# vt-asaplab/vPIN

Hardware: AMD Instinct MI355X
Metric: R1CS constraints/sec, whole Spartan SNARK (sat proof + SPARK evaluation proof; vPIN point-mult + point-add instances) (higher is better)
Workload: dtype u256 (integers mod q and mod p = 2^255-19, 32-bit limbs); 1 GPU; vPIN LeNet trace (layers L1..L7): 12 SNARKs per step; inputs=resident in HBM, parallelism=one trace per rank x 1 rank(s), no collective; 4 stream(s) per rank, table_slot_bytes=128

## Files before the change

include/vpin_hip.h:

```cpp
#ifndef VPIN_HIP_H
#define VPIN_HIP_H
#include <stddef.h>
#include <stdint.h>

#ifdef __cplusplus
extern "C" {
#endif

#define VPIN_OK 0
#define VPIN_EINVAL (-1)
#define VPIN_ENODEV (-2)
#define VPIN_ENOMEM (-3)
#define VPIN_EHIP (-4)
#define VPIN_ESHAPE (-5)
#define VPIN_EVERIFY (-6)

typedef struct vpin_ctx vpin_ctx;
typedef struct vpin_table vpin_table;

const char* vpin_strerror(int code);
const char* vpin_last_error(void);
int vpin_crash_line_set(const char* line, size_t n);
int vpin_abi_version(void);

int vpin_ctx_create(int device, vpin_ctx** out);
int vpin_ctx_create_prio(int device, int priority, vpin_ctx** out);
int vpin_ctx_create_cumask(int device, const uint32_t* cu_mask, uint32_t n_words, vpin_ctx** out);
int vpin_ctx_set_cumask_after_phase1(vpin_ctx* ctx, const uint32_t* cu_mask, uint32_t n_words);
void vpin_ctx_destroy(vpin_ctx* ctx);
void* vpin_ctx_stream(vpin_ctx* ctx);
int vpin_ctx_set_progress_flag(vpin_ctx* ctx, int* flag);
int vpin_ctx_set_shared_device(vpin_ctx* ctx, int on);
unsigned long long vpin_ctx_strip_rows_taken(vpin_ctx* ctx);
unsigned long long vpin_ctx_pip_row_chunks(vpin_ctx* ctx);
int vpin_ctx_pool_stats(vpin_ctx* ctx, size_t out[3]);
int vpin_driver_alloc_stats(unsigned long long out[2]);
int vpin_ctx_pool_trim(vpin_ctx* ctx);
int vpin_ctx_set_low_memory(vpin_ctx* ctx, int on);
int vpin_ctx_set_expected_proofs(vpin_ctx* ctx, int n);
int vpin_ctx_device_props(vpin_ctx* ctx, int* num_cus, int* clock_khz);
int vpin_ctx_mem_info(vpin_ctx* ctx, size_t* free_bytes, size_t* total_bytes);
int vpin_ctx_sync(vpin_ctx* ctx);

int vpin_host_register(void* p, size_t bytes);
int vpin_host_unregister(void* p);

int vpin_table_upload(vpin_ctx* ctx, const uint8_t* mont32, size_t len, vpin_table** out);
int vpin_table_alloc(vpin_ctx* ctx, size_t len, vpin_table** out);
int vpin_table_wrap(vpin_ctx* ctx, void* device_ptr, size_t len, vpin_table** out);
int vpin_table_clone(vpin_ctx* ctx, const vpin_table* src, vpin_table** out);
void vpin_table_free(vpin_ctx* ctx, vpin_table* t);
size_t vpin_table_len(const vpin_table* t);
void* vpin_table_device_ptr(const vpin_table* t);
int vpin_table_read(vpin_ctx* ctx, const vpin_table* t, size_t off, size_t n, uint8_t* out);
int vpin_table_write(vpin_ctx* ctx, vpin_table* t, size_t off, size_t n, const uint8_t* src);

int vpin_sc_cubic_round(vpin_ctx* ctx, const vpin_table* tau, const vpin_table* Az,
                        const vpin_table* Bz, const vpin_table* Cz, uint8_t out_e0_e2_e3[96]);
int vpin_sc_quad_round(vpin_ctx* ctx, const vpin_table* A, const vpin_table* B,
                       uint8_t out_e0_e2[64]);
int vpin_sc_bind(vpin_ctx* ctx, vpin_table* const* tables, int k, const uint8_t r[32]);
int vpin_sc_cubic_bind_round(vpin_ctx* ctx, vpin_table* tau, vpin_table* Az, vpin_table* Bz,
                             vpin_table* Cz, const uint8_t r[32], uint8_t out_e0_e2_e3[96]);
int vpin_sc_quad_bind_round(vpin_ctx* ctx, vpin_table* A, vpin_table* B, const uint8_t r[32],
                            uint8_t out_e0_e2[64]);

int vpin_eq_table(vpin_ctx* ctx, const uint8_t* r, int ell, vpin_table** out);

int vpin_eq_suffix_tables(vpin_ctx* ctx, const uint8_t* tau, int ell, vpin_table** out);
int vpin_sc_cubic3_round(vpin_ctx* ctx, const vpin_table* pyramid, int ell, int level, vpin_table* Az,
                         vpin_table* Bz, vpin_table* Cz, uint8_t out_S0_S2_S3[96]);
int vpin_sc_cubic3_bind_round(vpin_ctx* ctx, const vpin_table* pyramid, int ell, int level, vpin_table* Az,
                              vpin_table* Bz, vpin_table* Cz, const uint8_t r[32], uint8_t out_S0_S2_S3[96]);
int vpin_sc_cubic3_lead_round(vpin_ctx* ctx, const vpin_table* pyramid, int ell, int level, vpin_table* Az,
                              vpin_table* Bz, vpin_table* Cz, const uint8_t* r, uint8_t out[96]);
int vpin_spark_batched_round(vpin_ctx* ctx, vpin_table* forest, size_t n, int ncirc, int level, size_t len,
                             const vpin_table* E, size_t e_off, const uint8_t* r, int lead, const vpin_table* derefs,
                             const vpin_table* vals, vpin_table* scratch, int first_fold, uint8_t* out);

typedef struct vpin_gens vpin_gens;
int vpin_gens_create(vpin_ctx* ctx, const uint8_t* gens_xyzt, size_t nb, vpin_gens** out);
int vpin_gens_map_stream(vpin_ctx* ctx, const uint8_t* stream64, size_t nb, uint8_t* out_xyzt);
int vpin_gens_shared(vpin_ctx* ctx, const char* label, const uint8_t* gens_xyzt, size_t nb, size_t budget_gb,
                     const vpin_gens** out);
void vpin_gens_shared_clear(void);
size_t vpin_gens_shared_bytes(int device);
void vpin_gens_free(vpin_ctx* ctx, vpin_gens* g);
size_t vpin_gens_count(const vpin_gens* g);
int vpin_gens_layout(const vpin_gens* g, size_t out[6]);
size_t vpin_gens_entry_bytes(void);
int vpin_hyrax_commit(vpin_ctx* ctx, const vpin_gens* g, const vpin_table* Z, const uint8_t* blinds,
                      size_t L, size_t blind_base, uint8_t* out_compressed );
int vpin_hyrax_commit_rows(vpin_ctx* ctx, const vpin_gens* g, const vpin_table* Z, size_t L, size_t row0, size_t nrows,
                           const uint8_t* blinds, size_t blind_base, uint8_t* out_compressed);
int vpin_hyrax_commit_pippenger(vpin_ctx* ctx, const vpin_gens* g, const vpin_table* Z, const uint8_t* blinds, size_t L,
                                size_t blind_base, int c_bits, uint8_t* out_compressed);
int vpin_hyrax_commit_pair(vpin_ctx* ctx, const vpin_gens* g, const vpin_table* Za, const vpin_table* Zb,
                           const uint8_t* blinds_a, const uint8_t* blinds_b, size_t L, size_t blind_base,
                           uint8_t* out_a, uint8_t* out_b, uint8_t* out_sum);
int vpin_gens_msm(vpin_ctx* ctx, const vpin_gens* g, const uint8_t* scalars_mont, size_t rows, size_t ncols,
                  uint8_t* out_compressed , uint8_t* out_xyzt );

int vpin_msm(vpin_ctx* ctx, const uint8_t* scalars_mont, const uint8_t* points_compressed, size_t n, uint8_t* out_compressed,
             uint8_t* out_xyzt);
int vpin_msm_bucket(vpin_ctx* ctx, const uint8_t* scalars_mont, const uint8_t* points_compressed, size_t n, uint8_t* out_compressed,
                    uint8_t* out_xyzt);
int vpin_points_add(vpin_ctx* ctx, const uint8_t* a_compressed, const uint8_t* b_compressed, size_t n, uint8_t* out_compressed);

size_t vpin_gens_msm_parts_count(size_t ncols);
int vpin_gens_msm_parts(vpin_ctx* ctx, const vpin_gens* g, const uint8_t* scalars_mont, size_t rows, size_t ncols,
                        uint8_t* parts_xyzt);

int vpin_poly_bound(vpin_ctx* ctx, const vpin_table* Z, const uint8_t* Lvec, size_t L_size, uint8_t* out_LZ);
int vpin_poly_slices_bound(vpin_ctx* ctx, const vpin_table* Z, int nbits, int used, const uint8_t* r, size_t r_len,
                           const uint8_t* ch, uint8_t* evals_out, uint8_t* LZ_out);
int vpin_poly_slices_bound_u32(vpin_ctx* ctx, const uint32_t* slices_u32, int n32, const vpin_table* Zfq, int nbits, int used,
                               const uint8_t* r, size_t r_len, const uint8_t* ch, uint8_t* evals_out, uint8_t* LZ_out);

typedef struct {
  size_t num_cons, num_vars, num_inputs;
  size_t nnz[3];
  const uint32_t* row[3];
  const uint32_t* col[3];
  const uint8_t* val[3];
} vpin_r1cs;
typedef struct vpin_r1cs_dev vpin_r1cs_dev;
int vpin_r1cs_upload(vpin_ctx* ctx, const vpin_r1cs* inst, vpin_r1cs_dev** out);
void vpin_r1cs_free(vpin_ctx* ctx, vpin_r1cs_dev* d);
void vpin_r1cs_dims(const vpin_r1cs_dev* d, size_t* num_cons, size_t* num_vars, size_t* num_inputs);
int vpin_r1cs_build_z(vpin_ctx* ctx, const vpin_r1cs_dev* d, const vpin_table* vars, const uint8_t* inputs,
                      vpin_table** out_z);
int vpin_r1cs_multiply_vec(vpin_ctx* ctx, const vpin_r1cs_dev* d, const vpin_table* z, vpin_table** Az,
                           vpin_table** Bz, vpin_table** Cz);
int vpin_r1cs_eval_table(vpin_ctx* ctx, const vpin_r1cs_dev* d, const vpin_table* evals_rx, const uint8_t r_abc[96],
                         vpin_table** out);
int vpin_r1cs_evaluate(vpin_ctx* ctx, const vpin_r1cs_dev* d, const vpin_table* evals_rx, const vpin_table* evals_ry,
                       uint8_t out[96]);

int vpin_sat_prove(vpin_ctx* ctx, const vpin_r1cs* inst, const uint8_t* vars_para, const uint8_t* vars_input,
                   const uint8_t* vars, const uint8_t* inputs, const uint8_t seed_commit64[64],
                   const uint8_t seed_proof64[64], uint8_t* proof_out, size_t proof_cap, size_t* proof_len,
                   uint8_t* comm_para_out, uint8_t* comm_input_out, uint8_t inst_evals_out[96],
                   uint8_t* rx_out, uint8_t* ry_out);
int vpin_sat_prove_resident(vpin_ctx* ctx, const vpin_r1cs_dev* inst, const vpin_table* vars_para,
                            const vpin_table* vars_input, const vpin_table* vars, const uint8_t* inputs,
                            const uint8_t seed_commit64[64], const uint8_t seed_proof64[64], uint8_t* proof_out,
                            size_t proof_cap, size_t* proof_len, uint8_t* comm_para_out, uint8_t* comm_input_out,
                            uint8_t inst_evals_out[96], uint8_t* rx_out, uint8_t* ry_out);
size_t vpin_sat_proof_max_bytes(size_t num_cons, size_t num_vars);
int vpin_dense_mlpoly_commit_sum(vpin_ctx* ctx, const vpin_table* vars, const uint8_t seed_commit64[64], uint8_t* out_compressed);
int vpin_sat_prepare(vpin_ctx* ctx, size_t num_vars);
int vpin_spark_prepare(vpin_ctx* ctx, size_t num_cons, size_t num_vars, size_t max_nnz);

void vpin_sat_last_timings(double out[8]);


typedef struct vpin_spark_decomm vpin_spark_decomm;

#define VPIN_ECOMM (-7)
typedef struct vpin_comm vpin_comm;
typedef int (*vpin_allgather_fn)(void* user, const void* send, void* recv, size_t bytes_per_rank);
int vpin_comm_create_shm(const char* name, int rank, int world, size_t slot_bytes, vpin_comm** out);
int vpin_comm_create_local(int world, size_t slot_bytes, vpin_comm** out_handles );
int vpin_comm_create_callbacks(int rank, int world, vpin_allgather_fn fn, void* user, vpin_comm** out);
void vpin_comm_destroy(vpin_comm* cm);
int vpin_comm_rank(const vpin_comm* cm);
int vpin_comm_world(const vpin_comm* cm);
int vpin_comm_allgather(vpin_comm* cm, const void* send, void* recv, size_t bytes);
int vpin_comm_enable_rccl(vpin_comm* cm, vpin_ctx* ctx);
int vpin_comm_allgather_dev(vpin_comm* cm, vpin_ctx* ctx, const void* d_send, void* d_recv, size_t bytes);
int vpin_comm_set_serialize(vpin_comm* cm, int on);
typedef struct {
// ... 234 lines not shown
```

vpin_amd/capi.py:

```python
import ctypes as C
import os
import re

import numpy as np

HERE = os.path.dirname(os.path.abspath(__file__))
ROOT = os.path.dirname(HERE)
HEADER = os.path.join(ROOT, "include", "vpin_hip.h")

KERNEL_CLASSES = {
    0: "sc_cubic", 1: "sc_quad", 2: "sc_bind", 3: "sc_cubic_fused", 4: "sc_quad_fused", 5: "eq", 6: "msm", 7: "sc_tail",
    8: "spark_round", 9: "spark_build", 10: "spark_round_big", 11: "msm_rows", 12: "spark_tail",
}
K_COUNT = 16


class VpinError(RuntimeError):
    def __init__(self, code, where):
        self.code = code
        L = lib()
        msg = L.vpin_strerror(code).decode()
        last = L.vpin_last_error().decode()
        super().__init__(f"{where}: {msg} ({code})" + (f" [{last}]" if last else ""))

# ... 586 lines not shown
            _chk(lib().vpin_ctx_create_cumask(device, words.ctypes.data_as(C.c_void_p), len(words), C.byref(self.h)), "vpin_ctx_create_cumask")
            return
        _chk(lib().vpin_ctx_create_prio(device, priority, C.byref(self.h)), "vpin_ctx_create_prio")

    @staticmethod
    def _mask_words(cu_mask):
        cus = sorted(set(int(x) for x in cu_mask))
        words = np.zeros((cus[-1] // 32) + 1, dtype=np.uint32)
        for x in cus:
            words[x // 32] |= np.uint32(1 << (x % 32))
        return words

    def set_cumask_after_phase1(self, cu_mask):
        if cu_mask is None:
            _chk(lib().vpin_ctx_set_cumask_after_phase1(self.h, None, 0), "vpin_ctx_set_cumask_after_phase1")
            return
        words = self._mask_words(cu_mask)
        _chk(lib().vpin_ctx_set_cumask_after_phase1(self.h, words.ctypes.data_as(C.c_void_p), len(words)), "vpin_ctx_set_cumask_after_phase1")

    def close(self):
        if self.h:
            lib().vpin_ctx_destroy(self.h)
            self.h = None

    def __enter__(self):
        return self

    def __exit__(self, *a):
        self.close()

    @property
    def stream(self):
        return lib().vpin_ctx_stream(self.h)

    def sync(self):
        _chk(lib().vpin_ctx_sync(self.h), "vpin_ctx_sync")

    def device_props(self):
        cus, khz = C.c_int(), C.c_int()
        L = lib()
        L.vpin_ctx_device_props.argtypes = [C.c_void_p, C.POINTER(C.c_int), C.POINTER(C.c_int)]
        _chk(L.vpin_ctx_device_props(self.h, C.byref(cus), C.byref(khz)), "vpin_ctx_device_props")
        return cus.value, khz.value * 1e3

    def device_total_bytes(self):
        f, t = C.c_size_t(), C.c_size_t()
        L = lib()
        L.vpin_ctx_mem_info.argtypes = [C.c_void_p, C.POINTER(C.c_size_t), C.POINTER(C.c_size_t)]
        _chk(L.vpin_ctx_mem_info(self.h, C.byref(f), C.byref(t)), "vpin_ctx_mem_info")
        return t.value

    def pool_stats(self):
        L = lib()
        L.vpin_ctx_pool_stats.argtypes = [C.c_void_p, C.POINTER(C.c_size_t * 3)]
        out = (C.c_size_t * 3)()
        _chk(L.vpin_ctx_pool_stats(self.h, C.byref(out)), "vpin_ctx_pool_stats")
        return int(out[0]), int(out[1]), int(out[2])

    @staticmethod
    def crash_line_set(line_bytes):
        L = lib()
        L.vpin_crash_line_set.argtypes = [C.c_char_p, C.c_size_t]
        _chk(L.vpin_crash_line_set(line_bytes if line_bytes else None, len(line_bytes)), "vpin_crash_line_set")

    @staticmethod
    def driver_alloc_stats():
        L = lib()
        L.vpin_driver_alloc_stats.argtypes = [C.POINTER(C.c_ulonglong * 2)]
        out = (C.c_ulonglong * 2)()
        _chk(L.vpin_driver_alloc_stats(C.byref(out)), "vpin_driver_alloc_stats")
        return int(out[0]), int(out[1])

    def pool_trim(self):
        L = lib()
        L.vpin_ctx_pool_trim.argtypes = [C.c_void_p]
        _chk(L.vpin_ctx_pool_trim(self.h), "vpin_ctx_pool_trim")

    def pip_row_chunks(self):
        L = lib()
        L.vpin_ctx_pip_row_chunks.argtypes = [C.c_void_p]
        L.vpin_ctx_pip_row_chunks.restype = C.c_ulonglong
        return int(L.vpin_ctx_pip_row_chunks(self.h))

    def strip_rows_taken(self):
        L = lib()
        L.vpin_ctx_strip_rows_taken.argtypes = [C.c_void_p]
        L.vpin_ctx_strip_rows_taken.restype = C.c_ulonglong
        return int(L.vpin_ctx_strip_rows_taken(self.h))

    def set_shared_device(self, on=True):
        _chk(lib().vpin_ctx_set_shared_device(self.h, 1 if on else 0), "vpin_ctx_set_shared_device")

    def set_low_memory(self, on=True):
        L = lib()
        L.vpin_ctx_set_low_memory.argtypes = [C.c_void_p, C.c_int]
        _chk(L.vpin_ctx_set_low_memory(self.h, 1 if on else 0), "vpin_ctx_set_low_memory")

    def set_expected_proofs(self, n):
        L = lib()
        L.vpin_ctx_set_expected_proofs.argtypes = [C.c_void_p, C.c_int]
        _chk(L.vpin_ctx_set_expected_proofs(self.h, int(n)), "vpin_ctx_set_expected_proofs")

    def gens_map_stream(self, stream):
        L = lib()
        L.vpin_gens_map_stream.argtypes = [C.c_void_p, C.c_void_p, C.c_size_t, C.c_void_p]
        buf = np.frombuffer(bytes(stream), dtype=np.uint8).copy()
        n = buf.size // 64
        out = np.zeros((n, 128), dtype=np.uint8)
        _chk(L.vpin_gens_map_stream(self.h, buf.ctypes.data_as(C.c_void_p), n, out.ctypes.data_as(C.c_void_p)), "vpin_gens_map_stream")
        return out

    def upload(self, arr):
        a = np.ascontiguousarray(arr)
        n = a.nbytes // 32
        h = C.c_void_p()
        _chk(lib().vpin_table_upload(self.h, a.ctypes.data_as(C.c_void_p), n, C.byref(h)), "vpin_table_upload")
        return Table(self, h)

    def alloc(self, n):
        h = C.c_void_p()
        _chk(lib().vpin_table_alloc(self.h, n, C.byref(h)), "vpin_table_alloc")
        return Table(self, h)

    def wrap(self, device_ptr, n):
        h = C.c_void_p()
        _chk(lib().vpin_table_wrap(self.h, C.c_void_p(device_ptr), n, C.byref(h)), "vpin_table_wrap")
        return Table(self, h)

    def eq_table(self, r):
        r = np.ascontiguousarray(r, dtype=np.uint64).reshape(-1, 4)
        h = C.c_void_p()
        _chk(lib().vpin_eq_table(self.h, r.ctypes.data_as(C.c_void_p), r.shape[0], C.byref(h)), "vpin_eq_table")
        return Table(self, h)

    def sc_cubic_round(self, tau, A, B, Cc):
        out = np.zeros((3, 4), dtype=np.uint64)
        _chk(lib().vpin_sc_cubic_round(self.h, tau.h, A.h, B.h, Cc.h, out.ctypes.data_as(C.c_void_p)),
             "vpin_sc_cubic_round")
        return out

    def sc_quad_round(self, A, B):
        out = np.zeros((2, 4), dtype=np.uint64)
        _chk(lib().vpin_sc_quad_round(self.h, A.h, B.h, out.ctypes.data_as(C.c_void_p)), "vpin_sc_quad_round")
        return out

    def sc_bind(self, tables, r):
        r = np.ascontiguousarray(r, dtype=np.uint64).reshape(4)
        arr = (C.c_void_p * len(tables))(*[t.h for t in tables])
        _chk(lib().vpin_sc_bind(self.h, arr, len(tables), r.ctypes.data_as(C.c_void_p)), "vpin_sc_bind")

    def sc_cubic_bind_round(self, tau, A, B, Cc, r):
        r = np.ascontiguousarray(r, dtype=np.uint64).reshape(4)
        out = np.zeros((3, 4), dtype=np.uint64)
        _chk(lib().vpin_sc_cubic_bind_round(self.h, tau.h, A.h, B.h, Cc.h, r.ctypes.data_as(C.c_void_p),
                                            out.ctypes.data_as(C.c_void_p)), "vpin_sc_cubic_bind_round")
        return out

    def sc_quad_bind_round(self, A, B, r):
        r = np.ascontiguousarray(r, dtype=np.uint64).reshape(4)
        out = np.zeros((2, 4), dtype=np.uint64)
        _chk(lib().vpin_sc_quad_bind_round(self.h, A.h, B.h, r.ctypes.data_as(C.c_void_p),
                                           out.ctypes.data_as(C.c_void_p)), "vpin_sc_quad_bind_round")
        return out

    def gens_create(self, xyzt):
        a = np.ascontiguousarray(xyzt, dtype=np.uint8).reshape(-1, 128)
        h = C.c_void_p()
        _chk(lib().vpin_gens_create(self.h, a.ctypes.data_as(C.c_void_p), a.shape[0], C.byref(h)), "vpin_gens_create")
        return Gens(self, h)

    def gens_shared(self, label, xyzt, budget_gb=0):
        a = np.ascontiguousarray(xyzt, dtype=np.uint8).reshape(-1, 128)
        h = C.c_void_p()
        _chk(lib().vpin_gens_shared(self.h, label.encode(), a.ctypes.data_as(C.c_void_p), a.shape[0], budget_gb, C.byref(h)),
             "vpin_gens_shared")
        g = Gens(self, h)
        g.free = lambda: None
        return g

    def gens_msm_parts(self, gens, scalars, rows, ncols):
        L = lib()
        L.vpin_gens_msm_parts_count.restype = C.c_size_t
        L.vpin_gens_msm_parts_count.argtypes = [C.c_size_t]
        s = np.ascontiguousarray(scalars, dtype=np.uint64).reshape(rows * ncols, 4)
        np_ = L.vpin_gens_msm_parts_count(ncols)
        out = np.zeros((rows, np_, 128), dtype=np.uint8)
        L.vpin_gens_msm_parts.argtypes = [C.c_void_p, C.c_void_p, C.c_void_p, C.c_size_t, C.c_size_t, C.c_void_p]
        _chk(L.vpin_gens_msm_parts(self.h, gens.h, s.ctypes.data_as(C.c_void_p), rows, ncols, out.ctypes.data_as(C.c_void_p)),
             "vpin_gens_msm_parts")
        return out

    def hyrax_commit(self, gens, Z, blinds, blind_base):
        b = np.ascontiguousarray(blinds, dtype=np.uint64).reshape(-1, 4)
        Ls = b.shape[0]
        out = np.zeros((Ls, 32), dtype=np.uint8)
        _chk(lib().vpin_hyrax_commit(self.h, gens.h, Z.h, b.ctypes.data_as(C.c_void_p), Ls, blind_base,
                                     out.ctypes.data_as(C.c_void_p)), "vpin_hyrax_commit")
        return out

    def hyrax_commit_pippenger(self, gens, Z, blinds, blind_base, Ls=None, c_bits=0):
        b = None if blinds is None else np.ascontiguousarray(blinds, dtype=np.uint64).reshape(-1, 4)
        Ls = b.shape[0] if b is not None else int(Ls)
        out = np.zeros((Ls, 32), dtype=np.uint8)
        _chk(lib().vpin_hyrax_commit_pippenger(self.h, gens.h, Z.h, b.ctypes.data_as(C.c_void_p) if b is not None else None, Ls,
                                               blind_base, c_bits, out.ctypes.data_as(C.c_void_p)), "vpin_hyrax_commit_pippenger")
        return out

    def hyrax_commit_pair(self, gens, Za, Zb, blinds_a, blinds_b, blind_base):
        ba = np.ascontiguousarray(blinds_a, dtype=np.uint64).reshape(-1, 4)
        bb = np.ascontiguousarray(blinds_b, dtype=np.uint64).reshape(-1, 4)
        Ls = ba.shape[0]
        outs = [np.zeros((Ls, 32), dtype=np.uint8) for _ in range(3)]
        _chk(lib().vpin_hyrax_commit_pair(self.h, gens.h, Za.h, Zb.h, ba.ctypes.data_as(C.c_void_p),
                                          bb.ctypes.data_as(C.c_void_p), Ls, blind_base,
                                          *[o.ctypes.data_as(C.c_void_p) for o in outs]), "vpin_hyrax_commit_pair")
        return outs

    def gens_msm(self, gens, scalars, rows, ncols, want_xyzt=False):
        s = np.ascontiguousarray(scalars, dtype=np.uint64).reshape(rows * ncols, 4)
        out = np.zeros((rows, 32), dtype=np.uint8)
        ox = np.zeros((rows, 128), dtype=np.uint8) if want_xyzt else None
        _chk(lib().vpin_gens_msm(self.h, gens.h, s.ctypes.data_as(C.c_void_p), rows, ncols,
                                 out.ctypes.data_as(C.c_void_p),
                                 ox.ctypes.data_as(C.c_void_p) if want_xyzt else None), "vpin_gens_msm")
        return (out, ox) if want_xyzt else out

    def msm(self, scalars, points_compressed, want_xyzt=False):
        s = np.ascontiguousarray(scalars, dtype=np.uint64).reshape(-1, 4)
        pts = np.ascontiguousarray(points_compressed, dtype=np.uint8).reshape(-1, 32)
        assert s.shape[0] == pts.shape[0]
        out, xyzt = np.zeros(32, np.uint8), np.zeros(128, np.uint8)
        L = lib()
        L.vpin_msm.argtypes = [C.c_void_p, C.c_void_p, C.c_void_p, C.c_size_t, C.c_void_p, C.c_void_p]
        p = lambda a: a.ctypes.data_as(C.c_void_p)
        _chk(L.vpin_msm(self.h, p(s), p(pts), s.shape[0], p(out), p(xyzt) if want_xyzt else None), "vpin_msm")
        return (out, xyzt) if want_xyzt else out

    def msm_bucket(self, scalars, points_compressed, want_xyzt=False):
        s = np.ascontiguousarray(scalars, dtype=np.uint64).reshape(-1, 4)
        pts = np.ascontiguousarray(points_compressed, dtype=np.uint8).reshape(-1, 32)
        assert s.shape[0] == pts.shape[0]
        out, xyzt = np.zeros(32, np.uint8), np.zeros(128, np.uint8)
        L = lib()
        L.vpin_msm_bucket.argtypes = [C.c_void_p, C.c_void_p, C.c_void_p, C.c_size_t, C.c_void_p, C.c_void_p]
        p = lambda a: a.ctypes.data_as(C.c_void_p)
        _chk(L.vpin_msm_bucket(self.h, p(s), p(pts), s.shape[0], p(out), p(xyzt) if want_xyzt else None), "vpin_msm_bucket")
        return (out, xyzt) if want_xyzt else out

    def dense_mlpoly_commit_sum(self, t_vars, seed_commit):
        L = lib()
        L.vpin_dense_mlpoly_commit_sum.argtypes = [C.c_void_p, C.c_void_p, C.c_void_p, C.c_void_p]
        nv = len(t_vars)
        Ls = 1 << ((nv.bit_length() - 1) // 2)
        out = np.zeros((Ls, 32), dtype=np.uint8)
        sc = np.frombuffer(bytes(seed_commit), dtype=np.uint8).copy()
        _chk(L.vpin_dense_mlpoly_commit_sum(self.h, t_vars.h, sc.ctypes.data_as(C.c_void_p), out.ctypes.data_as(C.c_void_p)),
             "vpin_dense_mlpoly_commit_sum")
        return out

    def points_add(self, a, b):
        a = np.ascontiguousarray(a, dtype=np.uint8).reshape(-1, 32)
        b = np.ascontiguousarray(b, dtype=np.uint8).reshape(-1, 32)
        out = np.zeros_like(a)
        L = lib()
        L.vpin_points_add.argtypes = [C.c_void_p, C.c_void_p, C.c_void_p, C.c_size_t, C.c_void_p]
        p = lambda x: x.ctypes.data_as(C.c_void_p)
        _chk(L.vpin_points_add(self.h, p(a), p(b), a.shape[0], p(out)), "vpin_points_add")
        return out

    def poly_bound(self, Z, Lvec):
        lv = np.ascontiguousarray(Lvec, dtype=np.uint64).reshape(-1, 4)
        out = np.zeros((len(Z) // lv.shape[0], 4), dtype=np.uint64)
        _chk(lib().vpin_poly_bound(self.h, Z.h, lv.ctypes.data_as(C.c_void_p), lv.shape[0],
                                   out.ctypes.data_as(C.c_void_p)), "vpin_poly_bound")
        return out

    def poly_slices_bound(self, Z, nbits, used, r, ch=None):
        rr = np.ascontiguousarray(r, dtype=np.uint64).reshape(-1, 4)
        ell = rr.shape[0] + nbits
        ev = np.zeros((used, 4), dtype=np.uint64)
# ... 442 lines not shown
```

vpin_amd/csrc/capi.hip:

```cpp
#include <chrono>
#include <csignal>
#include <execinfo.h>
#include <fcntl.h>
#include <unistd.h>
#include <cstdio>
#include <cstdlib>
#include <cstring>
#include <thread>

#include "ctx.h"

namespace vpin {

static thread_local std::string g_last_error;

void set_last_error(const char* what, hipError_t e) {
  g_last_error = std::string(what) + ": " + hipGetErrorString(e);
}

void set_last_error_text(const char* text) { g_last_error = text; }

static hipEvent_t get_event(vpin_ctx* c) {
  if (!c->free_events.empty()) {
    hipEvent_t e = c->free_events.back();
// ... 273 lines not shown
    c->cu_masked = true;
  } else {
    e = hipStreamCreateWithPriority(&c->stream, hipStreamNonBlocking, prio);
  }
  if (e != hipSuccess) { set_last_error("hipStreamCreate", e); delete c; return VPIN_EHIP; }
  c->stream_main = c->stream;
  c->cus_main = c->num_cus;
  c->partials_cap = (size_t)18 * 4096 * 3;
  if (hipMalloc(&c->d_partials, c->partials_cap * sizeof(fq)) != hipSuccess ||
      hipMalloc(&c->d_out, 8 * sizeof(fq)) != hipSuccess ||
      hipHostMalloc(&c->h_out, 8 * sizeof(fq), hipHostMallocDefault) != hipSuccess) {
    vpin_ctx_destroy(c);
    return VPIN_ENOMEM;
  }
  ctx_register(c);
  *out = c;
  return VPIN_OK;
}

void vpin_ctx_destroy(vpin_ctx* c) {
  if (!c) return;
  (void)hipSetDevice(c->device);
  if (c->stream) (void)hipStreamSynchronize(c->stream);
  ctx_leave_alt(c);
  if (c->prover_cache_free) c->prover_cache_free(c);
  if (c->spark_cache_free) c->spark_cache_free(c);
  if (c->verify_cache_free) c->verify_cache_free(c);
  if (c->h_spark) (void)hipHostFree(c->h_spark);
  if (c->d_spark_cnt) (void)hipFree(c->d_spark_cnt);
  if (c->d_add_count) (void)hipFree(c->d_add_count);
  ctx_unregister(c);
  ctx_wait_unpinned(c);
  dev_pool_release(c);
  if (!c->pool_sizes.empty()) {
    fprintf(stderr, "vpin_ctx_destroy: %zu device block(s) still referenced by live handles are released with the context; "
                    "free tables / instances / decommitments before the context\n", c->pool_sizes.size());
    for (auto& kv : c->pool_sizes) (void)hipFree(kv.first);
    c->pool_sizes.clear();
  }
  for (auto& r : c->recs) { (void)hipEventDestroy(r.start); (void)hipEventDestroy(r.stop); }
  for (auto e : c->free_events) (void)hipEventDestroy(e);
  if (c->d_partials) (void)hipFree(c->d_partials);
  if (c->d_out) (void)hipFree(c->d_out);
  if (c->h_out) (void)hipHostFree(c->h_out);
  if (c->h_bullet) (void)hipHostFree(c->h_bullet);
  if (c->stream_alt) { (void)hipStreamSynchronize(c->stream_alt); (void)hipStreamDestroy(c->stream_alt); }
  if (c->stream_switch_ev) (void)hipEventDestroy(c->stream_switch_ev);
  if (c->stream_main) (void)hipStreamDestroy(c->stream_main);
  delete c;
}

void* vpin_ctx_stream(vpin_ctx* c) { return c ? (void*)c->stream : nullptr; }

int vpin_ctx_set_cumask_after_phase1(vpin_ctx* c, const uint32_t* cu_mask, uint32_t n_words) {
  if (!c || c->cu_masked || c->stream != c->stream_main) return VPIN_EINVAL;
  (void)hipSetDevice(c->device);
  if (c->stream_alt) {
    VPIN_HIP_TRY(hipStreamSynchronize(c->stream_alt));
    (void)hipStreamDestroy(c->stream_alt);
    c->stream_alt = nullptr;
    c->cus_alt = 0;
  }
  if (!cu_mask || n_words == 0) return VPIN_OK;
  int enabled = 0;
  for (uint32_t w = 0; w < n_words; w++) {
    uint32_t bits = cu_mask[w];
    if ((w + 1) * 32 > (uint32_t)c->cus_main) bits &= (w * 32 >= (uint32_t)c->cus_main) ? 0u : ((1u << (c->cus_main - w * 32)) - 1u);
    enabled += __builtin_popcount(bits);
  }
  if (enabled == 0) return VPIN_EINVAL;
  if (!c->stream_switch_ev) VPIN_HIP_TRY(hipEventCreateWithFlags(&c->stream_switch_ev, hipEventDisableTiming));
  VPIN_HIP_TRY(hipExtStreamCreateWithCUMask(&c->stream_alt, n_words, cu_mask));
  c->cus_alt = enabled;
  return VPIN_OK;
}

int vpin_ctx_set_progress_flag(vpin_ctx* c, int* flag) {
  if (!c) return VPIN_EINVAL;
  c->progress_flag = flag;
  return VPIN_OK;
}

unsigned long long vpin_ctx_strip_rows_taken(vpin_ctx* c) { return c ? c->strip_rows_taken : 0ull; }
unsigned long long vpin_ctx_pip_row_chunks(vpin_ctx* c) { return c ? c->pip_row_chunks : 0ull; }

int vpin_host_register(void* p, size_t bytes) {
  if (!p || !bytes) return VPIN_EINVAL;
  VPIN_HIP_TRY(hipHostRegister(p, bytes, hipHostRegisterDefault));
  return VPIN_OK;
}
int vpin_host_unregister(void* p) {
  if (!p) return VPIN_EINVAL;
  VPIN_HIP_TRY(hipHostUnregister(p));
  return VPIN_OK;
}

int vpin_ctx_pool_trim(vpin_ctx* c) {
  if (!c) return VPIN_EINVAL;
  (void)hipSetDevice(c->device);
  dev_pool_release(c);
  return VPIN_OK;
}

int vpin_ctx_pool_stats(vpin_ctx* c, size_t out[3]) {
  if (!c || !out) return VPIN_EINVAL;
  std::lock_guard<std::mutex> g(c->pool_mu);
  size_t total = 0, cached = 0;
  for (auto& kv : c->pool_sizes) total += kv.second;
  for (auto& kv : c->pool_free_lists) cached += kv.first * kv.second.size();
  out[0] = total; out[1] = cached; out[2] = c->pool_sizes.size();
  return VPIN_OK;
}

namespace {
char g_crash_buf[8192];
volatile size_t g_crash_len = 0;
struct sigaction g_crash_old[5];
const int g_crash_sigs[5] = {SIGSEGV, SIGBUS, SIGABRT, SIGFPE, SIGTERM};
void crash_handler(int) {
  const size_t n = g_crash_len;
  size_t off = 0;
  while (off < n) {
    const ssize_t w = write(1, g_crash_buf + off, n - off);
    if (w <= 0) break;
    off += (size_t)w;
  }
  _exit(0);
}
}

namespace {
int g_segv_fd = 2;
void segv_trace_handler(int sig) {
  void* frames[64];
  const int n = backtrace(frames, 64);
  const char msg[] = "[vpin] fatal signal, call stack of the faulting thread:\n";
  (void)!write(g_segv_fd, msg, sizeof msg - 1);
  backtrace_symbols_fd(frames, n, g_segv_fd);
  signal(sig, SIG_DFL);
  raise(sig);
}
struct SegvTraceInit {
  SegvTraceInit() {
    const char* e = getenv("VPIN_SEGV_TRACE");
    if (!e) return;
    if (e[0] == '/' || e[0] == '.' || strchr(e, '/')) {
      const int fd = open(e, O_WRONLY | O_CREAT | O_APPEND, 0644);
      if (fd >= 0) g_segv_fd = fd;
    }
    struct sigaction sa;
    memset(&sa, 0, sizeof sa);
    sa.sa_handler = segv_trace_handler;
    sigemptyset(&sa.sa_mask);
    for (int sg : {SIGSEGV, SIGBUS, SIGABRT}) (void)sigaction(sg, &sa, nullptr);
  }
} g_segv_trace_init;
}

int vpin_crash_line_set(const char* line, size_t n) {
  if (n > sizeof g_crash_buf || (n && !line)) return VPIN_EINVAL;
  const bool was_armed = g_crash_len != 0;
  if (n == 0) {
    if (was_armed)
      for (int i = 0; i < 5; i++) (void)sigaction(g_crash_sigs[i], &g_crash_old[i], nullptr);
    g_crash_len = 0;
    return VPIN_OK;
// ... 232 lines not shown
```

vpin_amd/csrc/ctx.h:

```cpp
#pragma once
#include <hip/hip_runtime.h>

#include <atomic>
#include <chrono>
#include <cstdio>
#include <cstdlib>
#include <map>
#include <mutex>
#include <string>
#include <unordered_map>
#include <vector>

#include "../../include/vpin_hip.h"
#include "fq_dev.h"

namespace vpin {

void set_last_error(const char* what, hipError_t e);

#define VPIN_HIP_TRY(expr)                         \
  do {                                             \
    hipError_t e_ = (expr);                        \
    if (e_ != hipSuccess) {                        \
      ::vpin::set_last_error(#expr, e_);           \
      return VPIN_EHIP;                            \
    }                                              \
  } while (0)

struct ProfRec {
  int kclass;
  double bytes;
  hipEvent_t start, stop;
  int also = -1;
  double units = 0.0;
};

}

struct vpin_ctx;

struct vpin_table {
  vpin::fq* d = nullptr;
  size_t len = 0;
  size_t cap = 0;
  bool owned = true;
  vpin_ctx* owner = nullptr;
};

struct vpin_gens;

struct vpin_ctx {
  int device = 0;
  hipStream_t stream = nullptr;
  int num_cus = 256;
  bool cu_masked = false;
  hipStream_t stream_main = nullptr, stream_alt = nullptr;
  hipEvent_t stream_switch_ev = nullptr;
  int cus_main = 256, cus_alt = 0;
  vpin::fq* d_partials = nullptr;
  size_t partials_cap = 0;
  vpin::fq* d_out = nullptr;
  vpin::fq* h_out = nullptr;
  bool prof = false;
  bool prof_count_adds = false;
  unsigned long long* d_add_count = nullptr;
  std::vector<vpin::ProfRec> recs;
  std::vector<hipEvent_t> free_events;
  vpin_kstat stats[VPIN_K_COUNT] = {};
  std::mutex pool_mu;
  std::atomic<int> pins{0};
  std::map<size_t, std::vector<void*>> pool_free_lists;
  std::unordered_map<void*, size_t> pool_sizes;
  void* prover_cache = nullptr;
  void (*prover_cache_free)(vpin_ctx*) = nullptr;
  void* spark_cache = nullptr;
  void (*spark_cache_free)(vpin_ctx*) = nullptr;
  void* verify_cache = nullptr;
  void (*verify_cache_free)(vpin_ctx*) = nullptr;
  vpin::fq* h_spark = nullptr;
  uint32_t* d_spark_cnt = nullptr;
  uint32_t spark_seq = 0;
  int round_split = 0, round_split_grid = 0, round_split_ncirc = 0;
  int round_group_ndotp = 0;
  uint32_t tail_seq = 0;
  std::atomic<int> tail_rounds{0};
  vpin::fq tail_sums[3 * 18];
  vpin::fq tail_final[6 * 18];
  unsigned long long pip_row_chunks = 0;
  unsigned long long strip_rows_taken = 0;
  bool low_memory = false;
  bool shared_device = false;
  int expected_proofs = 0;
  double gens_scalars_per_proof = 0.0;
  void* h_bullet = nullptr;
  uint32_t bullet_seq = 0;
  std::atomic<vpin_comm*> comm_pub{nullptr};
  vpin_comm* comm = nullptr;
  volatile int* progress_flag = nullptr;
};

namespace vpin {

struct ProfScope {
  vpin_ctx* ctx;
  int rec = -1;
  ProfScope(vpin_ctx* c, int kclass, double bytes, int also = -1, double units = 0.0);
  ~ProfScope();
};

void ctx_enter_alt(vpin_ctx* c);
void ctx_leave_alt(vpin_ctx* c);
struct AltStreamGuard {
  vpin_ctx* c;
  explicit AltStreamGuard(vpin_ctx* ctx) : c(ctx) {}
  ~AltStreamGuard() { ctx_leave_alt(c); }
};

int dev_alloc(vpin_ctx* c, size_t bytes, void** out);
hipError_t driver_malloc(void** p, size_t bytes);
void note_driver_alloc(size_t bytes);
void dev_free(vpin_ctx* c, void* p);
int live_ctx_count();
double host_cpu_quota();
void dev_free_owned(vpin_ctx* owner, vpin_ctx* fallback, void* p);
void dev_pool_release(vpin_ctx* c);
void dev_release_block(vpin_ctx* c, void* p);

struct DevBuf {
  vpin_ctx* c;
  void* p = nullptr;
  explicit DevBuf(vpin_ctx* ctx) : c(ctx) {}
  ~DevBuf() { if (p) dev_free(c, p); }
  int alloc(size_t bytes) { return dev_alloc(c, bytes, &p); }
  void release() { if (p) { dev_free(c, p); p = nullptr; } }
};

int table_alloc_uninit(vpin_ctx* c, size_t len, vpin_table** out);

struct CommitPairState;
int commit_pair_begin(vpin_ctx* c, const vpin_gens* g, const vpin_table* Za, const vpin_table* Zb, size_t L,
                      CommitPairState** out, size_t row0 = 0, size_t nrows = (size_t)-1, size_t row_step = 1);
int commit_pair_finish(vpin_ctx* c, const vpin_gens* g, CommitPairState* st, const uint8_t* blinds_a, const uint8_t* blinds_b,
                       size_t blind_base, uint8_t* out_a, uint8_t* out_b, uint8_t* out_sum);

int sc_round_launch(vpin_ctx* c, int K, vpin_table* const* tabs, const uint8_t* r);
int sc_round_wait(vpin_ctx* c, int K, uint8_t* out);
int sc_final_claims(vpin_ctx* c, vpin_table* const* tables, int k, const uint8_t r[32], uint8_t* out);
int sc_cubic3_launch(vpin_ctx* c, vpin_table* const* t, const vpin_table* pyramid, int ell, int level, const uint8_t* r,
                     bool lead = false);

int r1cs_multiply_vec_strided(vpin_ctx* c, const vpin_r1cs_dev* d, const vpin_table* z, size_t r0, size_t step, vpin_table** Az,
                              vpin_table** Bz, vpin_table** Cz);
int table_take_strided(vpin_ctx* c, const vpin_table* src, size_t r0, size_t step, vpin_table** out);
int r1cs_eval_table_strided(vpin_ctx* c, const vpin_r1cs_dev* d, const vpin_table* evals_rx, const uint8_t r_abc[96], size_t r0,
                            size_t step, vpin_table** out);

int poly_bound_dist(vpin_ctx* c, const vpin_table* Z, const uint8_t* Lvec, size_t L_size, uint8_t* out_LZ, const fq* z_rows = nullptr);

int slices_bound(vpin_ctx* c, const uint32_t* Z32, int n32, const fq* Z, size_t N, int S, size_t Rs, const uint8_t* Ltop, size_t T,
                 const uint8_t* Rv, fq* d_LZs, uint8_t* ev_out);
int slices_combine(vpin_ctx* c, const fq* d_LZs, int S, size_t Rs, const uint8_t* coef, uint8_t* out_LZ);

inline bool is_pow2(size_t x) { return x && !(x & (x - 1)); }

int gens_msm_parts_dev(vpin_ctx* c, const vpin_gens* g, const fq* d_scalars, size_t rows, size_t ncols, uint8_t* parts_xyzt);
int hyrax_commit_derefs_hot(vpin_ctx* c, const vpin_gens* g, const vpin_table* Z, size_t L, size_t N, const uint32_t* const col_idx[3],
                            const uint32_t hot[3], const fq* e_ry, uint8_t* out_compressed, size_t row0 = 0, size_t nrows = (size_t)-1,
                            size_t row_step = 1, const fq* z_rows = nullptr);
int hyrax_commit_rows_strided(vpin_ctx* c, const vpin_gens* g, const vpin_table* Z, size_t L, size_t row0, size_t nrows, size_t row_step,
                              uint8_t* out_compressed, const fq* z_rows = nullptr);
size_t gens_msm_parts_scratch_bytes(size_t rows, size_t ncols);
int gens_msm_parts_launch(vpin_ctx* c, const vpin_gens* g, const fq* d_scalars, size_t rows, size_t ncols, void* scratch,
                          uint8_t* parts_xyzt, bool host_mapped = false);

struct ge_niels;
struct ge_ext;
int pip_rows(vpin_ctx* c, const ge_niels* d_gn, const fq* dZ, size_t rows, size_t stride, size_t ncols, const fq* d_extra, int n_extra,
             int cbits, ge_ext* d_points, unsigned long long* d_adds);
int pip_default_bits(size_t n);

struct BulletState;
int bullet_begin(vpin_ctx* c, const uint8_t* x_mont, const uint8_t* a_mont, size_t R, BulletState** out);
int bullet_round_begin(vpin_ctx* c, const vpin_gens* g, BulletState* st, size_t n, uint8_t* parts_xyzt, uint8_t cLR[64]);
int bullet_round_end(vpin_ctx* c);
uint8_t* bullet_pinned(vpin_ctx* c);
int bullet_fold(vpin_ctx* c, BulletState* st, size_t n, const uint8_t u[32], const uint8_t u_inv[32]);
int bullet_finish(vpin_ctx* c, const vpin_gens* g, BulletState* st, uint8_t xhat_ahat[64], uint8_t* parts_xyzt);
void bullet_free(vpin_ctx* c, BulletState* st);
bool bullet_fused(const BulletState* st);
int bullet_step(vpin_ctx* c, const vpin_gens* g, BulletState* st, size_t n, const uint8_t* u_prev, const uint8_t* u_inv_prev,
                uint8_t cLR[64]);
size_t bullet_part_ptrs(vpin_ctx* c, const BulletState* st, size_t n, int row, const uint8_t** out);
int bullet_finish_fused(vpin_ctx* c, const vpin_gens* g, BulletState* st, const uint8_t u[32], const uint8_t u_inv[32],
                        uint8_t xhat_ahat[64]);
int bullet_step_launch(vpin_ctx* c, const vpin_gens* g, const fq* a_prev, const fq* b_prev, fq* a_next, fq* b_next, fq* sj, size_t n,
                       size_t R, bool fold, bool finish, const uint8_t* u, const uint8_t* u_inv, uint8_t* parts_pinned,
                       uint32_t* up_pinned, uint32_t seq, void* dev_parts);

struct TraceLap {
  vpin_ctx* c;
  const char* who;
  bool on;
  std::chrono::steady_clock::time_point t;
  TraceLap(vpin_ctx* ctx, const char* w) : c(ctx), who(w), on(getenv("VPIN_CLI_TRACE") != nullptr), t(std::chrono::steady_clock::now()) {}
  void operator()(const char* what) {
    if (!on) return;
    if (c) (void)hipStreamSynchronize(c->stream);
    auto n = std::chrono::steady_clock::now();
    fprintf(stderr, "[%s] %-22s %9.1f ms\n", who, what, std::chrono::duration<double, std::milli>(n - t).count());
    t = n;
  }
};

}
```

vpin_amd/csrc/ge_tree_dev.h:

```cpp
#pragma once
#include "fp10_dev.h"

namespace vpin {

__device__ __forceinline__ ge_ext ge_load(const ge_ext* p) {
  ge_ext e;
  e.X = fp_load(&p->X); e.Y = fp_load(&p->Y); e.Z = fp_load(&p->Z); e.T = fp_load(&p->T);
  return e;
}
__device__ __forceinline__ void ge_store(ge_ext* o, const ge_ext& a) {
  fp_store(&o->X, a.X); fp_store(&o->Y, a.Y); fp_store(&o->Z, a.Z); fp_store(&o->T, a.T);
}
__device__ __forceinline__ void ge_store_identity(ge_ext* o) { ge_store(o, ge_identity()); }
__device__ __forceinline__ ge_niels ge_load(const ge_niels* p) {
  ge_niels e;
  e.ypx = fp_load(&p->ypx); e.ymx = fp_load(&p->ymx); e.xy2d = fp_load(&p->xy2d);
  return e;
}
__device__ __forceinline__ void ge_store(ge_niels* o, const ge_niels& a) {
  fp_store(&o->ypx, a.ypx); fp_store(&o->ymx, a.ymx); fp_store(&o->xy2d, a.xy2d);
}
__device__ __forceinline__ ge_cached ge_load(const ge_cached* p) {
  ge_cached e;
  e.YpX = fp_load(&p->YpX); e.YmX = fp_load(&p->YmX); e.Z = fp_load(&p->Z); e.T2d = fp_load(&p->T2d);
  return e;
}
__device__ __forceinline__ void ge_store(ge_cached* o, const ge_cached& a) {
  fp_store(&o->YpX, a.YpX); fp_store(&o->YmX, a.YmX); fp_store(&o->Z, a.Z); fp_store(&o->T2d, a.T2d);
}
__device__ __forceinline__ ge_ext ge_load(const fp* xyzt) { return ge_load(reinterpret_cast<const ge_ext*>(xyzt)); }
__device__ __forceinline__ void ge_store(fp* xyzt, const ge_ext& a) { ge_store(reinterpret_cast<ge_ext*>(xyzt), a); }
__device__ __forceinline__ void ge_store_frozen(fp* xyzt, const ge_ext& a) {
  fp_store(xyzt, fp_freeze(a.X)); fp_store(xyzt + 1, fp_freeze(a.Y)); fp_store(xyzt + 2, fp_freeze(a.Z)); fp_store(xyzt + 3, fp_freeze(a.T));
}
__device__ __forceinline__ void ge_store_result(fp* out32, fp* out_xyzt, const ge_ext& r) {
  fp_store(out32, ge_compress(r));
  ge_store_frozen(out_xyzt, r);
}

__device__ __forceinline__ void ge10_store_strided(uint32_t* __restrict__ p, size_t stride, const ge10& a) {
#pragma unroll
  for (int l = 0; l < 10; l++) {
    p[(size_t)l * stride] = a.X.v[l]; p[(size_t)(10 + l) * stride] = a.Y.v[l];
    p[(size_t)(20 + l) * stride] = a.Z.v[l]; p[(size_t)(30 + l) * stride] = a.T.v[l];
  }
}
__device__ __forceinline__ ge10 ge10_load_strided(const uint32_t* __restrict__ p, size_t stride) {
  ge10 a;
#pragma unroll
  for (int l = 0; l < 10; l++) {
    a.X.v[l] = p[(size_t)l * stride]; a.Y.v[l] = p[(size_t)(10 + l) * stride];
    a.Z.v[l] = p[(size_t)(20 + l) * stride]; a.T.v[l] = p[(size_t)(30 + l) * stride];
  }
  return a;
}

__device__ __forceinline__ uint16_t fq_signed_window(fq& s, uint32_t& carry, uint32_t cw, bool top) {
  const uint32_t mask = (1u << cw) - 1u, half = 1u << (cw - 1);
  uint32_t v = (s.v[0] & mask) + carry;
#pragma unroll
  for (int i = 0; i < 7; i++) s.v[i] = __builtin_amdgcn_alignbit(s.v[i + 1], s.v[i], cw);
  s.v[7] >>= cw;
  const bool neg = !top && v > half;
  if (neg) v = (mask + 1u) - v;
  carry = neg ? 1u : 0u;
  return (uint16_t)(v | (neg && v ? 0x8000u : 0u));
}
template <class Width>
__device__ __forceinline__ ge10 ge10_horner_windows(const ge_ext* wsum, int W, Width width) {
  ge10 acc = ge10_from_ext(ge_load(wsum + W - 1));
#pragma unroll 1
  for (int w = W - 2; w >= 0; w--) {
#pragma unroll 1
    for (int k = 0, cw = width(w); k < cw; k++) acc = ge10_double(acc);
    acc = ge10_add_ge10(acc, ge10_from_ext(ge_load(wsum + w)));
  }
  return acc;
}

__device__ __forceinline__ fp fp_shfl_from(const fp& a, int src) {
  fp r;
#pragma unroll
  for (int i = 0; i < 8; i++) r.v[i] = __shfl(a.v[i], src, 64);
  return r;
}
__device__ __forceinline__ fp fp_pick(bool c, const fp& a, const fp& b) {
  fp r;
#pragma unroll
  for (int i = 0; i < 8; i++) r.v[i] = c ? a.v[i] : b.v[i];
  return r;
}
__device__ __forceinline__ void ge_tree_quad(ge_ext* sh, int n, int split = 0) {
  const int role = threadIdx.x & 3, qbase = (threadIdx.x & 63) & ~3;
  const fp* shf = reinterpret_cast<const fp*>(sh);
  fp* shw = reinterpret_cast<fp*>(sh);
  for (int s = n / 2; s >= 1; s >>= 1) {
    if (s == split) continue;
    const int items = s < split ? 2 * s : s;
    for (int w = threadIdx.x >> 2; w < items; w += (int)(blockDim.x >> 2)) {
      const int i = w < s ? w : split + (w - s);
      const int f0 = role < 2 ? 1 : (role == 2 ? 3 : 2);
      const fp p0 = shf[4 * i + f0], q0 = shf[4 * (i + s) + f0];
      fp u = p0, v = q0;
      if (role < 2) {
        const fp p1 = shf[4 * i], q1 = shf[4 * (i + s)];
        u = fp_pick(role == 0, fp_sub(p0, p1), fp_add(p0, p1));
        v = fp_pick(role == 0, fp_sub(q0, q1), fp_add(q0, q1));
      }
      fp m = fp_mul(u, v);
      m = fp_mul(m, fp_pick(role == 2, FP_D2(), fp_one()));
      m = fp_pick(role == 3, fp_add(m, m), m);
      const fp a = fp_shfl_from(m, qbase), b = fp_shfl_from(m, qbase + 1), c = fp_shfl_from(m, qbase + 2),
               d = fp_shfl_from(m, qbase + 3);
      const fp E = fp_sub(b, a), H = fp_add(b, a), F = fp_sub(d, c), G = fp_add(d, c);
      u = fp_pick(role == 0 || role == 3, E, fp_pick(role == 1, G, F));
      v = fp_pick(role == 0, F, fp_pick(role == 2, G, H));
      shw[4 * i + role] = fp_mul(u, v);
    }
    __syncthreads();
  }
}

}
```

vpin_amd/csrc/msm.hip:

```cpp
#include <algorithm>
#include <atomic>
#include <cstdlib>
#include <condition_variable>
#include <cstring>
#include <memory>
#include <mutex>
#include <string>
#include <vector>

#include "ctx.h"
#include "fp_dev.h"
#include "fp10_dev.h"
#include "ge_tree_dev.h"
#include "mailbox_dev.h"

#ifndef VPIN_NIELS_SLOT
#define VPIN_NIELS_SLOT 96
#endif
static_assert(VPIN_NIELS_SLOT == 96 || VPIN_NIELS_SLOT == 128, "table entry size");

struct vpin_gens {
  vpin::fp* table = nullptr;
  vpin::fp* table_hi = nullptr;
  int s32 = VPIN_NIELS_SLOT / 32;
  size_t nb = 0;
  size_t nbt = 0;
  size_t split = 0;
  int c = 12, W = 22, E = 2048;
  int c_hi = 8, W_hi = 32, E_hi = 128;
};

namespace vpin {

struct TableView {
  const fp* t;
  const fp* t_hi;
  size_t split, nbt;
  int c, W, E, c_hi, W_hi, E_hi;
  size_t sum0;
  int s32;
};

struct TableSeg {
  const fp* t;
  size_t j, nb;
  int c, W, E, s32;
  __device__ __forceinline__ const ge_niels* entry(int w, uint32_t d) const {
    return reinterpret_cast<const ge_niels*>(t + (((size_t)w * nb + j) * (size_t)E + d) * (size_t)s32);
  }
};
__device__ __forceinline__ TableSeg table_seg(const TableView& tv, size_t j) {
  if (j < tv.split) return TableSeg{tv.t, j, tv.split, tv.c, tv.W, tv.E, tv.s32};
  return TableSeg{tv.t_hi, j - tv.split, tv.nbt - tv.split, tv.c_hi, tv.W_hi, tv.E_hi, tv.s32};
}


__global__ __launch_bounds__(256) void gens_sum_kernel(fp* __restrict__ xyzt, size_t nb) {
  const int k = blockIdx.x;
  const size_t lo = k ? ((size_t)1 << (k - 1)) : 0, hi = (size_t)1 << k;
  ge_ext acc = ge_identity();
  for (size_t j = lo + threadIdx.x; j < hi && j < nb; j += 256) {
    acc = ge_add(acc, ge_load(xyzt + 4 * j));
  }
  __shared__ ge_ext sh[256];
  sh[threadIdx.x] = acc;
  __syncthreads();
  for (int st = 128; st >= 1; st >>= 1) {
    if ((int)threadIdx.x < st) {
      acc = ge_add(acc, sh[threadIdx.x + st]);
      sh[threadIdx.x] = acc;
    }
    __syncthreads();
  }
  if (threadIdx.x == 0) ge_store(xyzt + 4 * (nb + k), acc);
}
__global__ void gens_sum_scan_kernel(fp* __restrict__ xyzt, size_t nb, int nsum) {
  if (threadIdx.x || blockIdx.x) return;
  ge_ext acc = ge_load(xyzt + 4 * nb);
  for (int k = 1; k < nsum; k++) {
    fp* q = xyzt + 4 * (nb + k);
    acc = ge_add(acc, ge_load(q));
    ge_store(q, acc);
  }
}

__global__ __launch_bounds__(64) void gens_shift_kernel(const fp* __restrict__ xyzt, size_t nb, int W, int c,
                                                        ge_ext* __restrict__ shifts) {
  size_t j = (size_t)blockIdx.x * blockDim.x + threadIdx.x;
  if (j >= nb) return;
  ge_ext p = ge_load(xyzt + 4 * j);
  for (int w = 0; w < W; w++) {
    ge_store(shifts + j * W + w, p);
    for (int k = 0; k < c; k++) p = ge_double(p);
  }
}

__global__ __launch_bounds__(64) void gens_table_kernel(const ge_ext* __restrict__ shifts, size_t nb, int W, int E,
                                                        fp* __restrict__ table, int s32, fp* __restrict__ prefix) {
  size_t idx = (size_t)blockIdx.x * blockDim.x + threadIdx.x;
  if (idx >= nb * (size_t)W) return;
  size_t j = idx / W;
  int w = (int)(idx % W);
  const ge_ext p = ge_load(shifts + j * W + w);
  ge_cached pc = ge_to_cached(p);
  fp* out = table + (((size_t)w * nb + j) * E) * (size_t)s32;
  fp* pre = prefix + ((size_t)w * nb + j) * E;
  ge_ext q = p;
  fp run = fp_one();
  for (int k = 0; k < E; k++) {
    fp_store(out + (size_t)k * s32, q.X); fp_store(out + (size_t)k * s32 + 1, q.Y); fp_store(out + (size_t)k * s32 + 2, q.Z);
    run = fp_mul(run, q.Z);
    fp_store(pre + k, run);
    if (k + 1 < E) q = ge_add_cached(q, pc);
  }
  fp acc = fp_invert(run);
  const fp d2 = FP_D2();
  for (int k = E - 1; k >= 0; k--) {
    fp X = fp_load(out + (size_t)k * s32), Y = fp_load(out + (size_t)k * s32 + 1), Z = fp_load(out + (size_t)k * s32 + 2);
    fp zinv = (k > 0) ? fp_mul(acc, fp_load(pre + k - 1)) : acc;
    acc = fp_mul(acc, Z);
    fp x = fp_mul(X, zinv), y = fp_mul(Y, zinv);
    fp_store(out + (size_t)k * s32, fp_add(y, x));
    fp_store(out + (size_t)k * s32 + 1, fp_sub(y, x));
    fp_store(out + (size_t)k * s32 + 2, fp_mul(fp_mul(x, y), d2));
  }
}


__device__ __forceinline__ bool fq_fold_sign(fq& s) {
  if (s.v[7] < 0x08000000u) return false;
  fq d;
  unsigned bw = 0;
#pragma unroll
  for (int i = 0; i < 8; i++) d.v[i] = __builtin_subc(fq_modulus_limb(i), s.v[i], bw, &bw);
  s = d;
  return true;
}
// ... 290 lines not shown
  for (size_t r = r0; r < r1; r++) n += flag[r] ? 1u : 0u;
  base[threadIdx.x] = n;
  __syncthreads();
  if (threadIdx.x == 0) {
    uint32_t run = 0;
    for (int t = 0; t < 1024; t++) { const uint32_t v = base[t]; base[t] = run; run += v; }
    *count = run;
  }
  __syncthreads();
  uint32_t o = base[threadIdx.x];
  for (size_t r = r0; r < r1; r++)
    if (flag[r]) list[o++] = (uint32_t)r;
}

__global__ __launch_bounds__(256) void strip_trim_kernel(const uint32_t* __restrict__ list, uint32_t* __restrict__ count, uint32_t n_use,
                                                          uint32_t n_all, uint8_t* __restrict__ flag) {
  const uint32_t li = n_use + blockIdx.x * 256 + threadIdx.x;
  if (li < n_all) flag[list[li]] = 0;
  if (blockIdx.x == 0 && threadIdx.x == 0) *count = n_use;
}

__global__ __launch_bounds__(kMsmBlock, 3) void msm_strip_kernel(const fq* __restrict__ Z, size_t stride, size_t ncols, TableView tv, HotRows hr,
                                                                  const uint32_t* __restrict__ list, const uint32_t* __restrict__ list_count,
                                                                  int S, size_t row_base, size_t row_step, int z_compact,
                                                                  ge_ext* __restrict__ parts, uint32_t* __restrict__ sync, int lag) {
  const uint32_t n = *list_count;
  const uint32_t s = blockIdx.x % (uint32_t)S, grp = blockIdx.x / (uint32_t)S;
  if (grp * kMsmBlock >= n) return;
  const uint32_t li = grp * kMsmBlock + threadIdx.x;
  const bool live = li < n;
  const uint32_t i = list[live ? li : n - 1];
  const size_t row = row_base + (size_t)i * row_step;
  const fq* zr = Z + (z_compact ? (size_t)i : row) * stride;
  const uint32_t* idx = nullptr;
  uint32_t hot = 0xffffffffu;
  if (hr.rows_per_vec && row >= hr.row0 && row < hr.row0 + 3 * hr.rows_per_vec) {
    const size_t m = (row - hr.row0) / hr.rows_per_vec;
    if (hr.hot[m] != 0xffffffffu) { hot = hr.hot[m]; idx = hr.idx[m] + (row - hr.row0 - m * hr.rows_per_vec) * ncols; }
  }
  const size_t per = (ncols + (size_t)S - 1) / (size_t)S, j0 = (size_t)s * per, j1 = j0 + per < ncols ? j0 + per : ncols;
  ge10 acc = ge10_identity();
  const uint32_t groups = (n + kMsmBlock - 1) / kMsmBlock;
  uint32_t* my_sync = sync ? sync + (size_t)s * (per + 1) : nullptr;
  __shared__ int sh_nosync;
  if (threadIdx.x == 0) sh_nosync = 0;
  __syncthreads();
  for (size_t j = j0; j < j1; j++) {
    if (my_sync && j - j0 >= (size_t)lag) {
      if (threadIdx.x == 0 && !sh_nosync) {
        long spin = 0;
        while (__hip_atomic_load(my_sync + (j - j0 - (size_t)lag), __ATOMIC_RELAXED, __HIP_MEMORY_SCOPE_AGENT) < groups)
          if (++spin > (1L << 16)) { sh_nosync = 1; break; }
      }
      __syncthreads();
    }
    fq v = fq_load(zr + j);
    const bool act = live && !fq_is_zero(v) && !(idx && idx[j] == hot);
    if (__builtin_amdgcn_ballot_w64(act) != 0) {
      fq sc = fq_from_mont(v);
      if (!act) sc = fq_zero();
      table_mul_acc10(acc, sc, tv, j);
    }
    if (my_sync) {
      __syncthreads();
      if (threadIdx.x == 0) __hip_atomic_fetch_add(my_sync + (j - j0), 1u, __ATOMIC_RELAXED, __HIP_MEMORY_SCOPE_AGENT);
    }
  }
  if (live) {
    const ge_ext av = ge10_to_ext(acc);
    ge_store(parts + (size_t)li * (size_t)S + s, av);
  }
}

__global__ __launch_bounds__(64) void strip_combine_kernel(const ge_ext* __restrict__ parts, const uint32_t* __restrict__ list,
                                                            const uint32_t* __restrict__ list_count, int S, ge_ext* __restrict__ out) {
  const uint32_t li = blockIdx.x * 64 + threadIdx.x;
  if (li >= *list_count) return;
  ge_ext* o = out + list[li];
  ge_ext a = ge_load(o);
  for (int s = 0; s < S; s++) a = ge_add(a, ge_load(parts + (size_t)li * (size_t)S + s));
  ge_store(o, a);
}

__device__ __forceinline__ uint32_t count_digits(fq s, const TableView& tv, size_t j) {
  (void)fq_fold_sign(s);
  const TableSeg sg = table_seg(tv, j);
  uint32_t carry = 0, n = 0;
  const uint32_t full = 1u << sg.c, half = 1u << (sg.c - 1);
  for (int w = 0; w < sg.W; w++) {
    uint32_t v = scalar_digit(s, w, sg.c) + carry;
    const bool neg = v > half;
    const uint32_t mag = neg ? full - v : v;
    carry = neg ? 1u : 0u;
    n += mag != 0;
  }
  return n;
}
__global__ __launch_bounds__(kMsmBlock) void msm_count_adds_kernel(const fq* __restrict__ Z, size_t stride, size_t ncols,
                                                                   const fq* __restrict__ extra, int n_extra, size_t extra_base0,
                                                                   TableView tv, unsigned long long* __restrict__ count,
                                                                   HotRows hr = HotRows{}, size_t row_base = 0, size_t row_step = 1,
                                                                   int z_compact = 0) {
  const size_t row = row_base + (size_t)blockIdx.x * row_step;
  const fq* zr = Z + (z_compact ? (size_t)blockIdx.x : row) * stride;
  const uint32_t* hidx = nullptr;
  uint32_t hot = 0xffffffffu;
  if (hr.rows_per_vec && row >= hr.row0 && row < hr.row0 + 3 * hr.rows_per_vec) {
    const size_t m = (row - hr.row0) / hr.rows_per_vec;
    if (hr.hot[m] != 0xffffffffu) { hot = hr.hot[m]; hidx = hr.idx[m] + (row - hr.row0 - m * hr.rows_per_vec) * ncols; }
  }
  uint32_t n = 0;
  bool constant = false;
  if (ncols >= 256 && (ncols & (ncols - 1)) == 0 && ((size_t)1 << (tv.nbt - tv.sum0 - 1)) >= ncols) {
    const fq first = fq_load(zr);
    int same = 1;
    for (size_t j = threadIdx.x; j < ncols; j += kMsmBlock) same &= fq_eq(first, fq_load(zr + j)) ? 1 : 0;
    constant = __syncthreads_and(same) != 0;
    if (constant && threadIdx.x == 0 && !fq_is_zero(first))
      n += count_digits(fq_from_mont(first), tv, tv.sum0 + (size_t)(63 - __builtin_clzll((unsigned long long)ncols)));
  }
  if (!constant)
    for (size_t j = threadIdx.x; j < ncols; j += kMsmBlock) {
      const fq s = fq_load(zr + j);
      if (!fq_is_zero(s) && !(hidx && hidx[j] == hot)) n += count_digits(fq_from_mont(s), tv, j);
    }
  for (int e = threadIdx.x; e < n_extra; e += kMsmBlock) {
    const fq x = fq_load(extra + row * (size_t)n_extra + e);
    if (!fq_is_zero(x)) n += count_digits(fq_from_mont(x), tv, extra_base0 + e);
  }
  __shared__ uint32_t sh[kMsmBlock];
  sh[threadIdx.x] = n;
  __syncthreads();
  for (int st = kMsmBlock / 2; st >= 1; st >>= 1) {
    if ((int)threadIdx.x < st) sh[threadIdx.x] += sh[threadIdx.x + st];
    __syncthreads();
  }
  if (threadIdx.x == 0 && sh[0]) atomicAdd(count, (unsigned long long)sh[0]);
}

constexpr int kWideScalars = 32;
template <int Q>
__global__ __launch_bounds__(kMsmBlock) void msm_wide_kernel(const fq* __restrict__ S, size_t ncols, TableView tv,
                                                             fp* __restrict__ parts_xyzt) {
  const size_t row = blockIdx.y;
  const int grp = threadIdx.x & 7;
  ge_ext acc = ge_identity();
#pragma unroll 1
  for (int q = 0; q < Q; q++) {
    const size_t j = ((size_t)blockIdx.x * Q + q) * kWideScalars + (threadIdx.x >> 3);
    if (j < ncols) {
      fq s = fq_load(S + row * ncols + j);
      if (!fq_is_zero(s)) {
        const TableSeg sg = table_seg(tv, j);
        const int wpg = (sg.W + 7) / 8;
        int w0 = grp * wpg, w1 = (w0 + wpg < sg.W) ? w0 + wpg : sg.W;
        if (w0 < w1) table_mul_acc_range(acc, fq_from_mont(s), sg, w0, w1);
      }
    }
  }
  __shared__ ge_ext sh[kMsmBlock];
  sh[threadIdx.x] = acc;
  __syncthreads();
  ge_tree_quad(sh, kMsmBlock);
  if (threadIdx.x == 0) {
    acc = sh[0];
    ge_store_frozen(parts_xyzt + 4 * (row * gridDim.x + blockIdx.x), acc);
  }
}


struct BulletStep {
  const fq* a_prev; const fq* b_prev;
  fq* a_next; fq* b_next;
  fq* sj;
  size_t n, R;
  int fold, finish, nmsm;
  fq u, u_inv;
  fp* parts;
  uint32_t* up;
  uint32_t seq;
};

__global__ __launch_bounds__(kMsmBlock) void bullet_step_kernel(BulletStep a, TableView tv) {
  const size_t n = a.n;
  const int nip = (int)gridDim.x - a.nmsm;
  if ((int)blockIdx.x < nip) {
    const int ib = (int)blockIdx.x;
    const size_t i = (size_t)ib * kMsmBlock + threadIdx.x;
    fq pl = fq_zero(), pr = fq_zero();
    if (a.finish) {
      if (ib == 0 && threadIdx.x == 0) {
        pl = fq_add(fq_mul(fq_load(a.a_prev), a.u), fq_mul(a.u_inv, fq_load(a.a_prev + 1)));
        pr = fq_add(fq_mul(fq_load(a.b_prev), a.u_inv), fq_mul(a.u, fq_load(a.b_prev + 1)));
      }
    } else if (i < n) {
      fq a0, a1, b0, b1;
      if (a.fold) {
        a0 = fq_add(fq_mul(fq_load(a.a_prev + i), a.u), fq_mul(a.u_inv, fq_load(a.a_prev + 2 * n + i)));
        a1 = fq_add(fq_mul(fq_load(a.a_prev + n + i), a.u), fq_mul(a.u_inv, fq_load(a.a_prev + 3 * n + i)));
        b0 = fq_add(fq_mul(fq_load(a.b_prev + i), a.u_inv), fq_mul(a.u, fq_load(a.b_prev + 2 * n + i)));
        b1 = fq_add(fq_mul(fq_load(a.b_prev + n + i), a.u_inv), fq_mul(a.u, fq_load(a.b_prev + 3 * n + i)));
      } else {
        a0 = fq_load(a.a_prev + i); a1 = fq_load(a.a_prev + n + i);
        b0 = fq_load(a.b_prev + i); b1 = fq_load(a.b_prev + n + i);
      }
      fq_store(a.a_next + i, a0); fq_store(a.a_next + n + i, a1);
      fq_store(a.b_next + i, b0); fq_store(a.b_next + n + i, b1);
      pl = fq_mul(a0, b1);
      pr = fq_mul(a1, b0);
    }
    __shared__ fq shp[kMsmBlock / 64][2];
// ... 113 lines not shown
  ge_ext acc = ge_load(p);
  for (int k = 1; k < chunks; k++) acc = ge_add(acc, ge_load(p + k));
  ge_store(out + i, acc);
}

__global__ __launch_bounds__(64) void ge_add_rows_kernel(const ge_ext* __restrict__ a, const ge_ext* __restrict__ b, size_t n,
                                                         ge_ext* __restrict__ out) {
  size_t i = (size_t)blockIdx.x * blockDim.x + threadIdx.x;
  if (i >= n) return;
  ge_store(out + i, ge_add(ge_load(a + i), ge_load(b + i)));
}

__global__ __launch_bounds__(256) void pip_gens_kernel(TableView tv, size_t n, size_t blind_base, int n_extra, ge_niels* __restrict__ out) {
  const size_t i = (size_t)blockIdx.x * 256 + threadIdx.x;
  if (i >= n + (size_t)n_extra) return;
  const TableSeg sg = table_seg(tv, i < n ? i : blind_base);
  ge_store(out + i, ge_load(sg.entry(0, 0)));
}

__global__ __launch_bounds__(64) void ge_compress_kernel(const ge_ext* __restrict__ pts, size_t n, fp* __restrict__ out32,
                                                         fp* __restrict__ out_xyzt) {
  size_t i = (size_t)blockIdx.x * blockDim.x + threadIdx.x;
  if (i >= n) return;
  const ge_ext p = ge_load(pts + i);
  if (out32) fp_store(out32 + i, ge_compress(p));
  if (out_xyzt) ge_store_frozen(out_xyzt + 4 * i, p);
}

}

namespace vpin {

__device__ __forceinline__ fp FP_ONE_MINUS_D_SQ() { return fp_const(0x945fc176u, 0xe27c09c1u, 0xcd5e350fu, 0x2c81a138u, 0xbe70dfe4u, 0x9994abddu, 0xb2b3e0d7u, 0x029072a8u); }
__device__ __forceinline__ fp FP_D_MINUS_ONE_SQ() { return fp_const(0x44ed4d20u, 0x31ad5aaau, 0xb01e1999u, 0xd29e4a2cu, 0x529b4eebu, 0x4cdcd32fu, 0xf66c2241u, 0x5968b37au); }
__device__ __forceinline__ fp FP_SQRT_AD_MINUS_ONE() { return fp_const(0x497b2e1bu, 0x7e97f6a0u, 0x1b7854bdu, 0xaf9d8e0cu, 0x31f5d1fdu, 0x0f3cfcc9u, 0x2b8348acu, 0x376931bfu); }

__device__ __forceinline__ fp fp_sqrt_ratio_m1(const fp& u, const fp& v, bool* was_square) {
  const fp v3 = fp_mul(fp_sqr(v), v), v7 = fp_mul(fp_sqr(v3), v);
  fp r = fp_mul(fp_mul(u, v3), fp_pow_p58(fp_mul(u, v7)));
  const fp check = fp_mul(v, fp_sqr(r));
  const fp nu = fp_neg(u), nu_i = fp_mul(nu, FP_SQRT_M1());
  const bool correct = fp_eq(check, u), flipped = fp_eq(check, nu), flipped_i = fp_eq(check, nu_i);
  r = fp_select(flipped || flipped_i, fp_mul(r, FP_SQRT_M1()), r);
  *was_square = correct || flipped;
  return fp_abs(r);
}

__device__ __noinline__ ge_ext ge_elligator(const fp& t) {
  const fp one = fp_one(), m1 = fp_neg(one), d = FP_D();
  const fp r = fp_mul(FP_SQRT_M1(), fp_sqr(t));
  const fp u = fp_mul(fp_add(r, one), FP_ONE_MINUS_D_SQ());
  const fp v = fp_mul(fp_sub(m1, fp_mul(r, d)), fp_add(r, d));
  bool sq;
  fp s = fp_sqrt_ratio_m1(u, v, &sq);
  const fp sp = fp_neg(fp_abs(fp_mul(s, t)));
  s = fp_select(sq, s, sp);
  const fp c = fp_select(sq, m1, r);
  const fp N = fp_sub(fp_mul(fp_mul(c, fp_sub(r, one)), FP_D_MINUS_ONE_SQ()), v);
  const fp ss = fp_sqr(s);
  const fp w0 = fp_mul(fp_add(s, s), v), w1 = fp_mul(N, FP_SQRT_AD_MINUS_ONE()), w2 = fp_sub(one, ss), w3 = fp_add(one, ss);
  ge_ext p;
  p.X = fp_mul(w0, w3); p.Y = fp_mul(w2, w1); p.Z = fp_mul(w1, w3); p.T = fp_mul(w0, w2);
  return p;
}

__global__ __launch_bounds__(64) void gens_derive_kernel(const uint32_t* __restrict__ stream, size_t nb, fp* __restrict__ xyzt) {
  const size_t i = (size_t)blockIdx.x * 64 + threadIdx.x;
  if (i >= nb) return;
  fp t0, t1;
#pragma unroll
  for (int k = 0; k < 8; k++) { t0.v[k] = stream[16 * i + k]; t1.v[k] = stream[16 * i + 8 + k]; }
  t0.v[7] &= 0x7fffffffu;
  t1.v[7] &= 0x7fffffffu;
  const ge_ext p = ge_add(ge_elligator(t0), ge_elligator(t1));
  ge_store_frozen(xyzt + 4 * i, p);
}

}

using namespace vpin;

extern "C" {

static int gens_build_once(vpin_ctx* c, const uint8_t* gens_xyzt, size_t nb, size_t budget, int cmax, vpin_gens** out);

static int gens_build(vpin_ctx* c, const uint8_t* gens_xyzt, size_t nb, size_t budget, vpin_gens** out) {
  (void)hipSetDevice(c->device);
  size_t free_b = 0, total_b = 0;
  const hipError_t e_info = c->expected_proofs > 0 ? hipErrorUnknown : hipMemGetInfo(&free_b, &total_b);
  if (e_info == hipSuccess && free_b) {
    static const double frac = [] { const char* e = getenv("VPIN_GENS_FREE_FRACTION"); double v = e ? atof(e) : 0.0; return v > 0.0 && v < 1.0 ? v : 1.0 / 3.0; }();
    const size_t cap = (size_t)((double)free_b * frac);
    if (budget > cap) budget = cap;
  }
  const size_t floor_b = (size_t)1 << 28;
  if (budget < floor_b) budget = floor_b;
  static const int env_cmax = [] { const char* e = getenv("VPIN_GENS_CMAX"); int v = e ? atoi(e) : 12; return v < 8 ? 8 : v > 14 ? 14 : v; }();
  int cmax = env_cmax;
  if (c->expected_proofs > 0 && c->gens_scalars_per_proof > 0.0) {
    const double S = c->gens_scalars_per_proof * (double)c->expected_proofs, n_lo = (double)std::min<size_t>(nb, 16386);
    double best = 0.0;
    for (int cc = 8; cc <= 12; cc++) {
      const double W = (double)((254 + cc - 1) / cc), cost = n_lo * W * (double)(1u << (cc - 1)) * 4.0 + S * W;
      if (cc == 8 || cost < best) { best = cost; cmax = cc; }
    }
  }
  for (;;) {
    int rc = gens_build_once(c, gens_xyzt, nb, budget, cmax, out);
    if (rc != VPIN_ENOMEM || budget <= floor_b) return rc;
    (void)hipGetLastError();
    budget /= 2;
    if (budget < floor_b) budget = floor_b;
  }
}

static size_t table_slot_bytes() {
  const char* e = getenv("VPIN_TABLE_SLOT");
  const int v = e ? atoi(e) : VPIN_NIELS_SLOT;
  return v == 128 ? 128 : v == 96 ? 96 : (size_t)VPIN_NIELS_SLOT;
}

static int gens_build_once(vpin_ctx* c, const uint8_t* gens_xyzt, size_t nb, size_t budget, int cmax, vpin_gens** out) {
  if (!c || !gens_xyzt || !out || nb == 0) return VPIN_EINVAL;
  const size_t slot = table_slot_bytes();
  (void)hipSetDevice(c->device);
  vpin_gens* g = new (std::nothrow) vpin_gens();
  if (!g) return VPIN_ENOMEM;
  g->nb = nb;
  g->s32 = (int)(slot / 32);
  int nsum = 1;
  while (((size_t)2 << (nsum - 1)) <= nb) nsum++;
  const size_t nbt = nb + (size_t)nsum;
  g->nbt = nbt;
  constexpr size_t kSplitBases = 16386;
  auto fit = [&](size_t n, size_t bud, int cmax, int* c_, int* W_, int* E_) {
    int cc = cmax;
    for (; cc > 6; cc--)
      if (n * (size_t)((254 + cc - 1) / cc) * ((size_t)1 << (cc - 1)) * slot <= bud) break;
    *c_ = cc;
    *W_ = (254 + cc - 1) / cc;
    *E_ = 1 << (cc - 1);
  };
  g->split = nbt;
  fit(nb, budget, cmax, &g->c, &g->W, &g->E);
  if (nb > kSplitBases) {
    int c2, W2, E2;
    fit(kSplitBases, budget, cmax, &c2, &W2, &E2);
    const size_t lo_bytes = kSplitBases * (size_t)W2 * E2 * slot;
    if (c2 > g->c && lo_bytes < budget) {
      g->split = kSplitBases;
      g->c = c2; g->W = W2; g->E = E2;
      fit(nbt - kSplitBases, budget - lo_bytes, g->c, &g->c_hi, &g->W_hi, &g->E_hi);
    }
  }
  const size_t n_hi = nbt - g->split;
  const size_t entries = g->split * (size_t)g->W * g->E, entries_hi = n_hi * (size_t)g->W_hi * g->E_hi;
  const size_t max_entries = entries > entries_hi ? entries : entries_hi;
  const size_t max_shifts = std::max(g->split * (size_t)g->W, n_hi * (size_t)g->W_hi);
  TraceLap lap(c, "gens_build");
  DevBuf raw(c), b_shifts(c), b_prefix(c);
  if (raw.alloc(nbt * 128) != VPIN_OK || b_shifts.alloc(max_shifts * sizeof(ge_ext)) != VPIN_OK ||
      b_prefix.alloc(max_entries * sizeof(fp)) != VPIN_OK || driver_malloc((void**)&g->table, entries * slot) != hipSuccess ||
      (n_hi && driver_malloc((void**)&g->table_hi, entries_hi * slot) != hipSuccess)) {
    if (g->table) (void)hipFree(g->table);
    if (g->table_hi) (void)hipFree(g->table_hi);
    delete g;
    return VPIN_ENOMEM;
  }
  ge_ext* shifts = (ge_ext*)b_shifts.p;
  fp* prefix = (fp*)b_prefix.p;
  lap("hipMalloc");
  hipError_t e = hipMemcpyAsync(raw.p, gens_xyzt, nb * 128, hipMemcpyHostToDevice, c->stream);
  if (e == hipSuccess) {
    hipLaunchKernelGGL(gens_sum_kernel, dim3((unsigned)nsum), dim3(256), 0, c->stream, (fp*)raw.p, nb);
    hipLaunchKernelGGL(gens_sum_scan_kernel, dim3(1), dim3(64), 0, c->stream, (fp*)raw.p, nb, nsum);
    hipLaunchKernelGGL(gens_shift_kernel, dim3((unsigned)((g->split + 63) / 64)), dim3(64), 0, c->stream, (const fp*)raw.p, g->split,
                       g->W, g->c, shifts);
    hipLaunchKernelGGL(gens_table_kernel, dim3((unsigned)((g->split * g->W + 63) / 64)), dim3(64), 0, c->stream, shifts, g->split, g->W,
                       g->E, g->table, g->s32, prefix);
    if (n_hi) {
      hipLaunchKernelGGL(gens_shift_kernel, dim3((unsigned)((n_hi + 63) / 64)), dim3(64), 0, c->stream,
                         (const fp*)raw.p + 4 * g->split, n_hi, g->W_hi, g->c_hi, shifts);
      hipLaunchKernelGGL(gens_table_kernel, dim3((unsigned)((n_hi * g->W_hi + 63) / 64)), dim3(64), 0, c->stream, shifts, n_hi,
                         g->W_hi, g->E_hi, g->table_hi, g->s32, prefix);
    }
    e = hipGetLastError();
  }
  if (e == hipSuccess) e = hipStreamSynchronize(c->stream);
  lap("table kernels");
  if (e == hipSuccess && c->expected_proofs == 0 && !getenv("VPIN_GENS_TMP_KEEP") && b_prefix.p) {
    void* pp = b_prefix.p;
    b_prefix.p = nullptr;
    dev_release_block(c, pp);
  }
  if (e != hipSuccess) {
    set_last_error("vpin_gens_create", e);
    (void)hipFree(g->table);
    if (g->table_hi) (void)hipFree(g->table_hi);
    delete g;
    return VPIN_EHIP;
  }
  *out = g;
  return VPIN_OK;
}

static size_t default_budget() {
  static const size_t budget = [] {
    const char* e = getenv("VPIN_GENS_BUDGET_GB");
    size_t gb = e ? (size_t)atoi(e) : 24;
    return (gb ? gb : 24) << 30;
  }();
  return budget;
}

int vpin_gens_create(vpin_ctx* c, const uint8_t* gens_xyzt, size_t nb, vpin_gens** out) {
  return gens_build(c, gens_xyzt, nb, default_budget(), out);
}

int vpin_gens_map_stream(vpin_ctx* c, const uint8_t* stream64, size_t nb, uint8_t* out_xyzt) {
  if (!c || !stream64 || !out_xyzt || nb == 0) return VPIN_EINVAL;
  (void)hipSetDevice(c->device);
  DevBuf bs(c), bo(c);
  if (bs.alloc(nb * 64) || bo.alloc(nb * 128)) return VPIN_ENOMEM;
  VPIN_HIP_TRY(hipMemcpyAsync(bs.p, stream64, nb * 64, hipMemcpyHostToDevice, c->stream));
  hipLaunchKernelGGL(gens_derive_kernel, dim3((unsigned)((nb + 63) / 64)), dim3(64), 0, c->stream, (const uint32_t*)bs.p, nb, (fp*)bo.p);
  VPIN_HIP_TRY(hipGetLastError());
  VPIN_HIP_TRY(hipMemcpyAsync(out_xyzt, bo.p, nb * 128, hipMemcpyDeviceToHost, c->stream));
  VPIN_HIP_TRY(hipStreamSynchronize(c->stream));
  return VPIN_OK;
}

namespace {
struct RegEntry { int device; std::string label; vpin_gens* g; };
struct Building { int device; std::string label; size_t nb; };
std::mutex g_reg_mu;
std::condition_variable g_reg_cv;
std::vector<RegEntry> g_reg;
std::vector<Building> g_building;
}

int vpin_gens_shared(vpin_ctx* c, const char* label, const uint8_t* gens_xyzt, size_t nb, size_t budget_gb,
                     const vpin_gens** out) {
  if (!c || !label || !out || nb == 0) return VPIN_EINVAL;
  auto lookup = [&]() -> const vpin_gens* {
    const vpin_gens* best = nullptr;
    for (auto& e : g_reg)
      if (e.device == c->device && e.label == label && e.g->nb >= nb && (!best || e.g->nb < best->nb)) best = e.g;
    return best;
  };
  {
    std::unique_lock<std::mutex> lock(g_reg_mu);
    for (;;) {
      if (const vpin_gens* best = lookup()) { *out = best; return VPIN_OK; }
      bool covered = false;
      for (auto& b : g_building) covered = covered || (b.device == c->device && b.label == label && b.nb >= nb);
      if (!covered) break;
      g_reg_cv.wait(lock);
    }
    if (!gens_xyzt) return VPIN_EINVAL;
    static std::atomic<bool> said{false};
    for (auto& e : g_reg)
      if (e.device == c->device && e.label == label && !said.exchange(true))
        fprintf(stderr, "vpin_gens_shared: a table of \"%s\" for %zu generators is built beside the one for %zu (both stay allocated): "
                        "call vpin_spark_prepare / vpin_sat_prepare with the largest shape first\n", label, nb, e.g->nb);
    g_building.push_back(Building{c->device, label, nb});
  }
  vpin_gens* g = nullptr;
  const int rc = gens_build(c, gens_xyzt, nb, budget_gb ? (budget_gb << 30) : default_budget(), &g);
  std::lock_guard<std::mutex> lock(g_reg_mu);
  for (size_t i = 0; i < g_building.size(); i++)
    if (g_building[i].device == c->device && g_building[i].label == label && g_building[i].nb == nb) { g_building.erase(g_building.begin() + (long)i); break; }
  if (!rc) {
    g_reg.push_back(RegEntry{c->device, label, g});
    *out = g;
  }
  g_reg_cv.notify_all();
  return rc;
}

size_t vpin_gens_shared_bytes(int device) {
  std::lock_guard<std::mutex> lock(g_reg_mu);
  size_t total = 0;
  for (auto& e : g_reg)
    if (e.device == device)
      total += (size_t)32 * (size_t)e.g->s32 * ((size_t)e.g->W * e.g->split * (size_t)e.g->E +
                                     (e.g->split < e.g->nbt ? (size_t)e.g->W_hi * (e.g->nbt - e.g->split) * (size_t)e.g->E_hi : 0));
  return total;
}

void vpin_gens_shared_clear(void) {
  std::lock_guard<std::mutex> lock(g_reg_mu);
  for (auto& e : g_reg) {
    (void)hipSetDevice(e.device);
    (void)hipDeviceSynchronize();
    if (e.g->table) (void)hipFree(e.g->table);
    if (e.g->table_hi) (void)hipFree(e.g->table_hi);
    delete e.g;
  }
  g_reg.clear();
}

void vpin_gens_free(vpin_ctx* c, vpin_gens* g) {
  if (!g) return;
  if (c) { (void)hipSetDevice(c->device); (void)hipStreamSynchronize(c->stream); }
  if (g->table) (void)hipFree(g->table);
  if (g->table_hi) (void)hipFree(g->table_hi);
  delete g;
}

size_t vpin_gens_count(const vpin_gens* g) { return g ? g->nb : 0; }
int vpin_gens_layout(const vpin_gens* g, size_t out[6]) {
  if (!g || !out) return VPIN_EINVAL;
  out[0] = (size_t)g->c; out[1] = (size_t)g->W; out[2] = g->split;
  out[3] = g->split < g->nbt ? (size_t)g->c_hi : 0; out[4] = g->split < g->nbt ? (size_t)g->W_hi : 0; out[5] = g->nbt;
  return VPIN_OK;
}
size_t vpin_gens_entry_bytes(void) { return table_slot_bytes(); }

static inline TableView view(const vpin_gens* g) {
  return TableView{g->table, g->table_hi, g->split, g->nbt, g->c, g->W, g->E, g->c_hi, g->W_hi, g->E_hi, g->nb, g->s32};
}

static int pip_mode() {
  const char* e = getenv("VPIN_MSM_PIPPENGER");
  const int v = e ? atoi(e) : 0;
  return v <= 0 ? 0 : (v >= 9 && v <= 12 ? v : -1);
}

static int msm_rows_pip(vpin_ctx* c, const vpin_gens* g, const fq* dZ, size_t rows, size_t stride, size_t ncols, const fq* d_extra,
                        int n_extra, size_t extra_base0, int cbits, ge_ext* d_points) {
  DevBuf dgn(c);
  if (dgn.alloc((ncols + 1) * sizeof(ge_niels))) return VPIN_ENOMEM;
  hipLaunchKernelGGL(pip_gens_kernel, dim3((unsigned)((ncols + 1 + 255) / 256)), dim3(256), 0, c->stream, view(g), ncols, extra_base0,
                     n_extra, (ge_niels*)dgn.p);
  return pip_rows(c, (const ge_niels*)dgn.p, dZ, rows, stride, ncols, d_extra, n_extra, cbits, d_points,
                  c->prof_count_adds ? c->d_add_count : nullptr);
}

static unsigned msm_lds_pad(const vpin_ctx* c) {
  static const int env_pad = [] { const char* e = getenv("VPIN_MSM_LDS_PAD"); return e ? atoi(e) : -1; }();
  return env_pad >= 0 ? (unsigned)env_pad : (c->shared_device ? kSharedPad : 0u);
}

static int msm_rows(vpin_ctx* c, const vpin_gens* g, const fq* dZ, size_t rows, size_t stride, size_t ncols,
                    const fq* d_extra, int n_extra, size_t extra_base0, ge_ext* d_points) {
  if (const int pm = pip_mode())
    if (n_extra <= 1 && ncols + (size_t)n_extra <= 32768)
      return msm_rows_pip(c, g, dZ, rows, stride, ncols, d_extra, n_extra, extra_base0, pm < 0 ? 0 : pm, d_points);
  double nz_est = (double)rows * ((double)ncols + n_extra);
  size_t total = ncols + (size_t)n_extra;
  int chunks = 1;
  if (rows < 128) {
    size_t want = (total + kMsmBlock - 1) / kMsmBlock * 4;
    chunks = (int)(want < 1 ? 1 : want > 64 ? 64 : want);
  } else if (rows >= 768 && total > (size_t)kSeg) {
    static const int env_chunks = [] { const char* e = getenv("VPIN_MSM_ROW_CHUNKS"); return e ? atoi(e) : 0; }();
    chunks = env_chunks > 0 ? env_chunks : (int)std::min<size_t>(8, (total + kSeg - 1) / kSeg);
  } else if (rows < 768 && total >= 2 * (size_t)kMsmBlock) {
    size_t want = (768 + rows - 1) / rows, most = total / kMsmBlock;
    chunks = (int)(want < most ? want : most);
    if (chunks < 1) chunks = 1;
  }
  DevBuf parts(c);
  ge_ext* dst = d_points;
  if (chunks > 1) {
    if (parts.alloc(rows * (size_t)chunks * sizeof(ge_ext))) return VPIN_ENOMEM;
    dst = (ge_ext*)parts.p;
  }
  if (c->prof_count_adds && c->d_add_count && rows >= 128)
    hipLaunchKernelGGL(msm_count_adds_kernel, dim3((unsigned)rows), dim3(kMsmBlock), 0, c->stream, dZ, stride, ncols, d_extra,
                       n_extra, extra_base0, view(g), c->d_add_count);
  {
    ProfScope ps(c, VPIN_K_MSM, 32.0 * nz_est, rows >= 128 ? VPIN_K_MSM_ROWS : -1);
    hipLaunchKernelGGL(msm_rows_kernel, dim3((unsigned)rows, (unsigned)chunks), dim3(kMsmBlock), msm_lds_pad(c), c->stream, dZ, stride, ncols,
                       d_extra, n_extra, extra_base0, view(g), dst);
  }
  if (chunks > 1)
    hipLaunchKernelGGL(ge_sum_chunks_kernel, dim3((unsigned)((rows + 63) / 64)), dim3(64), 0, c->stream, (const ge_ext*)dst,
                       rows, chunks, d_points);
  VPIN_HIP_TRY(hipGetLastError());
  return VPIN_OK;
}

static int compress_to_host(vpin_ctx* c, const ge_ext* d_pts, size_t n, uint8_t* out0, uint8_t* out1 = nullptr, uint8_t* out2 = nullptr) {
  uint8_t* const outs[3] = {out0, out1, out2};
  const size_t k = out2 ? 3 : out1 ? 2 : 1, per = n / k * 32;
  DevBuf dout(c);
  if (dout.alloc(n * 32)) return VPIN_ENOMEM;
  hipLaunchKernelGGL(ge_compress_kernel, dim3((unsigned)((n + 63) / 64)), dim3(64), 0, c->stream, d_pts, n, (fp*)dout.p, (fp*)nullptr);
  VPIN_HIP_TRY(hipGetLastError());
  for (size_t i = 0; i < k; i++) VPIN_HIP_TRY(hipMemcpyAsync(outs[i], (uint8_t*)dout.p + i * per, per, hipMemcpyDeviceToHost, c->stream));
  VPIN_HIP_TRY(hipStreamSynchronize(c->stream));
  return VPIN_OK;
}

static int commit_rows(vpin_ctx* c, const vpin_gens* g, const fq* z, size_t rows, size_t stride, size_t R, const uint8_t* blinds,
                       size_t blind_base, bool buckets, int c_bits, uint8_t* out_compressed) {
  (void)hipSetDevice(c->device);
  const int n_extra = blinds ? 1 : 0;
  DevBuf dbl(c), dpts(c);
  if ((blinds && dbl.alloc(rows * 32)) || dpts.alloc(rows * sizeof(ge_ext))) return VPIN_ENOMEM;
  if (blinds) VPIN_HIP_TRY(hipMemcpyAsync(dbl.p, blinds, rows * 32, hipMemcpyHostToDevice, c->stream));
  const int rc = buckets ? msm_rows_pip(c, g, z, rows, stride, R, (const fq*)dbl.p, n_extra, blind_base, c_bits, (ge_ext*)dpts.p)
                         : msm_rows(c, g, z, rows, stride, R, (const fq*)dbl.p, n_extra, blind_base, (ge_ext*)dpts.p);
  if (rc) return rc;
  return compress_to_host(c, (const ge_ext*)dpts.p, rows, out_compressed);
}

int vpin_hyrax_commit(vpin_ctx* c, const vpin_gens* g, const vpin_table* Z, const uint8_t* blinds, size_t L,
                      size_t blind_base, uint8_t* out_compressed) {
  if (!c || !g || !Z || !Z->d || !blinds || !out_compressed || L == 0) return VPIN_EINVAL;
  if (Z->len % L != 0) return VPIN_ESHAPE;
  const size_t R = Z->len / L;
  if (R > g->nb || blind_base >= g->nb) return VPIN_ESHAPE;
  return commit_rows(c, g, Z->d, L, R, R, blinds, blind_base, false, 0, out_compressed);
}

int vpin_hyrax_commit_pippenger(vpin_ctx* c, const vpin_gens* g, const vpin_table* Z, const uint8_t* blinds, size_t L,
                                size_t blind_base, int c_bits, uint8_t* out_compressed) {
  if (!c || !g || !Z || !Z->d || !out_compressed || L == 0) return VPIN_EINVAL;
  if (Z->len % L != 0) return VPIN_ESHAPE;
  const size_t R = Z->len / L;
  if (R > g->nb || (blinds && blind_base >= g->nb)) return VPIN_ESHAPE;
  return commit_rows(c, g, Z->d, L, R, R, blinds, blind_base, true, c_bits, out_compressed);
}

int vpin_hyrax_commit_rows(vpin_ctx* c, const vpin_gens* g, const vpin_table* Z, size_t L, size_t row0, size_t nrows,
                           const uint8_t* blinds, size_t blind_base, uint8_t* out_compressed) {
  if (!c || !g || !Z || !Z->d || !out_compressed || L == 0 || nrows == 0) return VPIN_EINVAL;
  if (Z->len % L != 0 || row0 + nrows > L) return VPIN_ESHAPE;
  const size_t R = Z->len / L;
  if (R > g->nb || (blinds && blind_base >= g->nb)) return VPIN_ESHAPE;
  return commit_rows(c, g, Z->d + row0 * R, nrows, R, R, blinds, blind_base, false, 0, out_compressed);
}

}

namespace vpin {

struct StripShape { size_t groups; int strips; uint32_t rows_used; };
static StripShape strip_shape(size_t R, uint32_t eligible, size_t slots, bool cu_masked, size_t min_list) {
  const size_t G = ((size_t)eligible + kMsmBlock - 1) / kMsmBlock;
  size_t bestG = 0;
  int bestS = 0;
  for (int cand = 8; cand <= 64 && (size_t)cand * 128 <= R; cand += 8)
    if (G * (size_t)cand <= slots) { bestG = G; bestS = cand; }
  if (cu_masked)
    for (int cand = 8; cand <= 64 && (size_t)cand * 128 <= R; cand += 8) {
      const size_t g2 = std::min(G, slots / (size_t)cand);
      if (g2 * kMsmBlock >= min_list && g2 * (size_t)cand > bestG * (size_t)bestS) { bestG = g2; bestS = cand; }
    }
  if (const char* eshape = getenv("VPIN_MSM_STRIP_SHAPE")) {
    int eg = 0, esn = 0;
    if (sscanf(eshape, "%d,%d", &eg, &esn) == 2 && eg > 0 && esn > 0 && esn % 8 == 0 && (size_t)esn <= R / 8) {
      if (std::min(G, (size_t)eg) * (size_t)esn <= slots) { bestG = std::min(G, (size_t)eg); bestS = esn; }
      else if (getenv("VPIN_MSM_STRIP_TRACE")) fprintf(stderr, "[strip] VPIN_MSM_STRIP_SHAPE=%d,%d refused: %zu workgroups on %zu slots\n", eg, esn, std::min(G, (size_t)eg) * (size_t)esn, slots);
    }
  }
  return StripShape{bestG, bestS, bestG ? (uint32_t)std::min<size_t>(eligible, bestG * kMsmBlock) : 0u};
}

int hyrax_commit_derefs_hot(vpin_ctx* c, const vpin_gens* g, const vpin_table* Z, size_t L, size_t N, const uint32_t* const col_idx[3],
                            const uint32_t hot[3], const fq* e_ry, uint8_t* out_compressed, size_t row0, size_t nrows, size_t row_step,
                            const fq* z_rows) {
  if (!c || !g || !Z || (!Z->d && !z_rows) || !col_idx || !hot || !e_ry || !out_compressed || L == 0 || Z->len % L) return VPIN_EINVAL;
  const size_t R = Z->len / L;
  if (R > g->nb || N % R || Z->len < 6 * N) return VPIN_ESHAPE;
  const fq* zbase = z_rows ? z_rows : (const fq*)Z->d;
  const int z_compact = z_rows ? 1 : 0;
  if (nrows == (size_t)-1) { row0 = 0; nrows = L; row_step = 1; }
  if (row_step == 0 || (nrows && row0 + (nrows - 1) * row_step >= L)) return VPIN_ESHAPE;
  if (nrows == 0) return VPIN_OK;
  if (pip_mode()) return hyrax_commit_rows_strided(c, g, Z, L, row0, nrows, row_step, out_compressed, z_rows);
  (void)hipSetDevice(c->device);
  DevBuf dpts(c), dT(c);
  if (dpts.alloc(nrows * sizeof(ge_ext))) return VPIN_ENOMEM;
  HotRows hr{};
  hr.row0 = 3 * (N / R);
  hr.rows_per_vec = N / R;
  uint32_t distinct[3];
  int nd = 0;
  for (int m = 0; m < 3; m++) {
    hr.idx[m] = col_idx[m];
    hr.hot[m] = hot[m];
    if (hot[m] == 0xffffffffu) continue;
    bool seen = false;
    for (int k = 0; k < nd; k++) seen = seen || distinct[k] == hot[m];
    if (!seen) distinct[nd++] = hot[m];
  }
  if (nd && dT.alloc((size_t)nd * R * sizeof(ge_cached))) return VPIN_ENOMEM;
  for (int k = 0; k < nd; k++) {
    ge_cached* Tk = (ge_cached*)dT.p + (size_t)k * R;
    hipLaunchKernelGGL(scalar_times_bases_kernel, dim3((unsigned)((R + 63) / 64)), dim3(64), 0, c->stream, e_ry + distinct[k], R, view(g), Tk);
    for (int m = 0; m < 3; m++)
      if (hot[m] == distinct[k]) hr.T[m] = Tk;
  }
  if (c->prof_count_adds && c->d_add_count)
    hipLaunchKernelGGL(msm_count_adds_kernel, dim3((unsigned)nrows), dim3(kMsmBlock), 0, c->stream, zbase, R, R, (const fq*)nullptr, 0,
                       (size_t)0, view(g), c->d_add_count, hr, row0, row_step, z_compact);
  static const int env_chunks = [] { const char* e = getenv("VPIN_MSM_HOT_CHUNKS"); return e ? atoi(e) : 0; }();
  const int chunks = env_chunks > 0 ? env_chunks : (int)std::max<size_t>(1, std::min<size_t>(8, R / kSeg));
  DevBuf dparts(c);
  if (chunks > 1 && dparts.alloc(nrows * (size_t)chunks * sizeof(ge_ext))) return VPIN_ENOMEM;
  const char* es = getenv("VPIN_MSM_STRIP");
  const char* em = getenv("VPIN_MSM_STRIP_MIN");
  const int env_strip = es ? atoi(es) : -1;
  const size_t min_rows = em ? (size_t)atol(em) : 8192, min_list = em ? (size_t)1 : 4096, min_R = em ? (size_t)64 : 4096;
  int S = env_strip > 0 ? env_strip : 16;
  DevBuf dflag(c), dlist(c), dsparts(c), dsync(c);
  uint32_t n_strip = 0;
  bool uniform_shape = false;
  if (env_strip != 0 && (env_strip > 0 || (!c->shared_device && c->comm == nullptr)) && nrows >= min_rows && R >= min_R && R <= g->split &&
      S % 8 == 0 && (size_t)S <= R / 8) {
    if (dflag.alloc(nrows) || dlist.alloc((nrows + 1) * sizeof(uint32_t))) return VPIN_ENOMEM;
    uint32_t* d_list = (uint32_t*)dlist.p;
    uint32_t* d_count = d_list + nrows;
    hipLaunchKernelGGL(strip_classify_kernel, dim3((unsigned)nrows), dim3(kMsmBlock), 0, c->stream, zbase, R, R, hr, row0, row_step, z_compact,
                       (uint8_t*)dflag.p);
    hipLaunchKernelGGL(strip_list_kernel, dim3(1), dim3(1024), 0, c->stream, (const uint8_t*)dflag.p, nrows, d_list, d_count);
    VPIN_HIP_TRY(hipMemcpyAsync(&n_strip, d_count, sizeof n_strip, hipMemcpyDeviceToHost, c->stream));
    VPIN_HIP_TRY(hipStreamSynchronize(c->stream));
    if (n_strip < min_list) n_strip = 0;
    if (n_strip && env_strip < 0) {
      const size_t slots = (size_t)c->num_cus * (c->shared_device ? 1 : 3);
      const StripShape shape = strip_shape(R, n_strip, slots, c->cu_masked, min_list);
      if (shape.rows_used && shape.rows_used < n_strip)
        hipLaunchKernelGGL(strip_trim_kernel, dim3((n_strip - shape.rows_used + 255) / 256), dim3(256), 0, c->stream, (const uint32_t*)d_list,
                           d_count, shape.rows_used, n_strip, (uint8_t*)dflag.p);
      if (getenv("VPIN_MSM_STRIP_TRACE")) fprintf(stderr, "[strip] %zu rows: %u eligible, %u taken as %zu groups x %d strips on %zu slots\n", nrows, n_strip, shape.rows_used, shape.groups, shape.strips, slots);
      n_strip = shape.rows_used;
      if (n_strip) {
        S = shape.strips;
        uniform_shape = true;
      }
    }
    if (n_strip && dsparts.alloc((size_t)n_strip * (size_t)S * sizeof(ge_ext))) return VPIN_ENOMEM;
  }
  const uint8_t* d_flag = n_strip ? (const uint8_t*)dflag.p : nullptr;
  {
    ProfScope ps(c, VPIN_K_MSM, 32.0 * (double)(nrows * R), VPIN_K_MSM_ROWS);
    const unsigned pad = msm_lds_pad(c);
    if (n_strip) {
      c->strip_rows_taken += n_strip;
      const unsigned groups = (unsigned)((n_strip + kMsmBlock - 1) / kMsmBlock);
      const size_t per = (R + (size_t)S - 1) / (size_t)S;
      const char* el = getenv("VPIN_MSM_STRIP_LAG");
      const int lag = el ? atoi(el) : 1;
      uint32_t* d_sync = nullptr;
      if (lag > 0 && uniform_shape) {
        if (dsync.alloc((size_t)S * (per + 1) * sizeof(uint32_t))) return VPIN_ENOMEM;
        d_sync = (uint32_t*)dsync.p;
        VPIN_HIP_TRY(hipMemsetAsync(d_sync, 0, (size_t)S * (per + 1) * sizeof(uint32_t), c->stream));
      }
      hipLaunchKernelGGL(msm_strip_kernel, dim3(groups * (unsigned)S), dim3(kMsmBlock), pad, c->stream, zbase, R, R, view(g), hr,
                         (const uint32_t*)dlist.p, (const uint32_t*)dlist.p + nrows, S, row0, row_step, z_compact, (ge_ext*)dsparts.p,
                         d_sync, lag);
    }
    hipLaunchKernelGGL(msm_rows_hot_kernel, dim3((unsigned)nrows, (unsigned)chunks), dim3(kMsmBlock), pad, c->stream, zbase, R, R,
                       view(g), hr, chunks > 1 ? (ge_ext*)dparts.p : (ge_ext*)dpts.p, row0, row_step, z_compact, d_flag);
    if (chunks > 1)
      hipLaunchKernelGGL(ge_sum_chunks_kernel, dim3((unsigned)((nrows + 63) / 64)), dim3(64), 0, c->stream, (const ge_ext*)dparts.p, nrows,
                         chunks, (ge_ext*)dpts.p);
    if (n_strip)
      hipLaunchKernelGGL(strip_combine_kernel, dim3((n_strip + 63) / 64), dim3(64), 0, c->stream, (const ge_ext*)dsparts.p,
                         (const uint32_t*)dlist.p, (const uint32_t*)dlist.p + nrows, S, (ge_ext*)dpts.p);
  }
  return compress_to_host(c, (const ge_ext*)dpts.p, nrows, out_compressed);
}

int hyrax_commit_rows_strided(vpin_ctx* c, const vpin_gens* g, const vpin_table* Z, size_t L, size_t row0, size_t nrows, size_t row_step,
                              uint8_t* out_compressed, const fq* z_rows) {
  if (!c || !g || !Z || (!Z->d && !z_rows) || !out_compressed || L == 0 || row_step == 0) return VPIN_EINVAL;
  if (nrows == 0) return VPIN_OK;
  if (Z->len % L != 0 || row0 + (nrows - 1) * row_step >= L) return VPIN_ESHAPE;
  const size_t R = Z->len / L;
  if (R > g->nb) return VPIN_ESHAPE;
  if (z_rows) return commit_rows(c, g, z_rows, nrows, R, R, nullptr, 0, false, 0, out_compressed);
  return commit_rows(c, g, Z->d + row0 * R, nrows, row_step * R, R, nullptr, 0, false, 0, out_compressed);
}

}

extern "C" {

int vpin_hyrax_commit_pair(vpin_ctx* c, const vpin_gens* g, const vpin_table* Za, const vpin_table* Zb,
                           const uint8_t* blinds_a, const uint8_t* blinds_b, size_t L, size_t blind_base,
                           uint8_t* out_a, uint8_t* out_b, uint8_t* out_sum) {
  if (!c || !g || !Za || !Zb || !blinds_a || !blinds_b || !out_a || !out_b || !out_sum || L == 0) return VPIN_EINVAL;
  if (Za->len != Zb->len || Za->len % L != 0) return VPIN_ESHAPE;
  size_t R = Za->len / L;
  if (R > g->nb || blind_base >= g->nb) return VPIN_ESHAPE;
  (void)hipSetDevice(c->device);
  DevBuf dbl(c), dpts(c);
  if (dbl.alloc(2 * L * 32) || dpts.alloc(3 * L * sizeof(ge_ext))) return VPIN_ENOMEM;
  VPIN_HIP_TRY(hipMemcpyAsync(dbl.p, blinds_a, L * 32, hipMemcpyHostToDevice, c->stream));
  VPIN_HIP_TRY(hipMemcpyAsync((uint8_t*)dbl.p + L * 32, blinds_b, L * 32, hipMemcpyHostToDevice, c->stream));
  ge_ext* pts = (ge_ext*)dpts.p;
  int rc = msm_rows(c, g, Za->d, L, R, R, (const fq*)dbl.p, 1, blind_base, pts);
  if (rc) return rc;
  rc = msm_rows(c, g, Zb->d, L, R, R, (const fq*)dbl.p + L, 1, blind_base, pts + L);
  if (rc) return rc;
  hipLaunchKernelGGL(ge_add_rows_kernel, dim3((unsigned)((L + 63) / 64)), dim3(64), 0, c->stream, pts, pts + L, L, pts + 2 * L);
  return compress_to_host(c, pts, 3 * L, out_a, out_b, out_sum);
}

constexpr size_t kMaxParts = 128;
static inline int wide_q(size_t ncols) { return ncols >= 8192 ? 4 : 1; }
static inline size_t raw_parts(size_t ncols) { const size_t per = (size_t)kWideScalars * wide_q(ncols); return (ncols + per - 1) / per; }
size_t vpin_gens_msm_parts_count(size_t ncols) { size_t n = raw_parts(ncols); return n < kMaxParts ? n : kMaxParts; }

int vpin_gens_msm_parts(vpin_ctx* c, const vpin_gens* g, const uint8_t* scalars_mont, size_t rows, size_t ncols,
                        uint8_t* parts_xyzt) {
  if (!c || !g || !scalars_mont || !parts_xyzt || rows == 0 || ncols == 0) return VPIN_EINVAL;
  if (ncols > g->nb) return VPIN_ESHAPE;
  (void)hipSetDevice(c->device);
  DevBuf ds(c);
  if (ds.alloc(rows * ncols * 32)) return VPIN_ENOMEM;
  VPIN_HIP_TRY(hipMemcpyAsync(ds.p, scalars_mont, rows * ncols * 32, hipMemcpyHostToDevice, c->stream));
  return vpin::gens_msm_parts_dev(c, g, (const fq*)ds.p, rows, ncols, parts_xyzt);
}

}

namespace vpin {
struct CommitPairState {
  DevBuf pts;
  size_t L = 0;
  explicit CommitPairState(vpin_ctx* c) : pts(c) {}
};

int commit_pair_begin(vpin_ctx* c, const vpin_gens* g, const vpin_table* Za, const vpin_table* Zb, size_t L_all,
                      CommitPairState** out, size_t row0, size_t nrows, size_t row_step) {
  if (!c || !g || !Za || !Zb || !out || L_all == 0) return VPIN_EINVAL;
  if (Za->len != Zb->len || Za->len % L_all != 0) return VPIN_ESHAPE;
  size_t R = Za->len / L_all;
  if (R > g->nb) return VPIN_ESHAPE;
  if (nrows == (size_t)-1) { row0 = 0; nrows = L_all; row_step = 1; }
  if (nrows == 0 || row_step == 0 || row0 + (nrows - 1) * row_step >= L_all) return VPIN_ESHAPE;
  const size_t L = nrows;
  (void)hipSetDevice(c->device);
  CommitPairState* st = new (std::nothrow) CommitPairState(c);
  if (!st) return VPIN_ENOMEM;
  st->L = L;
  if (st->pts.alloc(5 * L * sizeof(ge_ext))) { delete st; return VPIN_ENOMEM; }
  ge_ext* pts = (ge_ext*)st->pts.p;
  int rc = msm_rows(c, g, Za->d + row0 * R, L, row_step * R, R, nullptr, 0, 0, pts);
  if (!rc) rc = msm_rows(c, g, Zb->d + row0 * R, L, row_step * R, R, nullptr, 0, 0, pts + L);
  if (rc) { delete st; return rc; }
  *out = st;
  return VPIN_OK;
}

int commit_pair_finish(vpin_ctx* c, const vpin_gens* g, CommitPairState* st, const uint8_t* blinds_a, const uint8_t* blinds_b,
                       size_t blind_base, uint8_t* out_a, uint8_t* out_b, uint8_t* out_sum) {
  if (!st) return VPIN_EINVAL;
  std::unique_ptr<CommitPairState> guard(st);
  if (!c || !g || !blinds_a || !blinds_b || !out_a || !out_b || !out_sum) return VPIN_EINVAL;
  if (blind_base >= g->nb) return VPIN_ESHAPE;
  const size_t L = st->L;
  DevBuf dbl(c);
  if (dbl.alloc(2 * L * 32)) return VPIN_ENOMEM;
  VPIN_HIP_TRY(hipMemcpyAsync(dbl.p, blinds_a, L * 32, hipMemcpyHostToDevice, c->stream));
  VPIN_HIP_TRY(hipMemcpyAsync((uint8_t*)dbl.p + L * 32, blinds_b, L * 32, hipMemcpyHostToDevice, c->stream));
  ge_ext* pts = (ge_ext*)st->pts.p;
  hipLaunchKernelGGL(single_base_mul_kernel, dim3((unsigned)((2 * L + 7) / 8)), dim3(64), 0, c->stream, (const fq*)dbl.p, 2 * L,
                     view(g), blind_base, pts + 2 * L);
// ... 106 lines not shown
```

vpin_amd/csrc/prover.cpp:

```cpp
#include "host/prover_common.h"

namespace {

using namespace vpin_host;
using namespace vpin_prover;


struct SatGens {
  size_t ell = 0, L = 0, R = 0, nb = 0;
  std::vector<Point> g;
  FixedBase fb[5];
  const vpin_gens* dev = nullptr;
  PcGens pc;
  Mcg gens_1, gens_3, gens_4;
};

struct ProverCache {
  std::map<size_t, std::unique_ptr<SatGens>> by_nv;
};

static void cache_free(vpin_ctx* c) {
  auto* pc = static_cast<ProverCache*>(c->prover_cache);
  if (!pc) return;
  delete pc;
  c->prover_cache = nullptr;
}

static int get_gens(vpin_ctx* c, size_t num_vars, SatGens** out) {
  if (!c->prover_cache) { c->prover_cache = new ProverCache(); c->prover_cache_free = cache_free; }
  auto* pc = static_cast<ProverCache*>(c->prover_cache);
  auto it = pc->by_nv.find(num_vars);
  if (it != pc->by_nv.end()) { *out = it->second.get(); return VPIN_OK; }
  std::unique_ptr<SatGens> sg(new SatGens());
  sg->ell = log2z(num_vars);
  size_t left = sg->ell / 2;
  sg->L = (size_t)1 << left;
  sg->R = (size_t)1 << (sg->ell - left);
  sg->nb = sg->R + 2 < 5 ? 5 : sg->R + 2;
  vpin::TraceLap lap(nullptr, "sat gens");
  derive_gens(sg->g, sg->nb, "gens_r1cs_sat", c);
  lap("derive_gens (host)");
#pragma omp parallel for schedule(dynamic, 1) num_threads(host_threads())
  for (int i = 0; i < 7; i++) {
    if (i < 5) sg->fb[i] = FixedBase(sg->g[i]);
    else if (i == 5) sg->pc.fb_gR = FixedBase(sg->g[sg->R]);
    else sg->pc.fb_h = FixedBase(sg->g[sg->R + 1]);
  }
  sg->pc.ell = sg->ell; sg->pc.L = sg->L; sg->pc.R = sg->R;
  sg->pc.bind_views();
  sg->gens_1 = sg->pc.gens_1;
  sg->gens_3 = Mcg{3, {&sg->fb[0], &sg->fb[1], &sg->fb[2], nullptr}, &sg->fb[3]};
  sg->gens_4 = Mcg{4, {&sg->fb[0], &sg->fb[1], &sg->fb[2], &sg->fb[3]}, &sg->fb[4]};
  int rc = vpin_gens_shared(c, "gens_r1cs_sat", nullptr, sg->nb, 0, &sg->dev);
  if (rc == VPIN_EINVAL) {
    std::vector<uint8_t> xyzt(128 * sg->nb);
    for (size_t i = 0; i < sg->nb; i++) sg->g[i].to_xyzt(xyzt.data() + 128 * i);
    c->gens_scalars_per_proof = (double)num_vars;
    rc = vpin_gens_shared(c, "gens_r1cs_sat", xyzt.data(), sg->nb, 0, &sg->dev);
  }
  if (rc) return rc;
  lap("fixed bases + table");
  sg->pc.dev = sg->dev;
  *out = sg.get();
  pc->by_nv[num_vars] = std::move(sg);
  return VPIN_OK;
}


struct ZkSc { std::vector<CG> comm_polys, comm_evals; std::vector<DotProof> proofs; };

static void write_zksc(Writer& w, const ZkSc& p) {
  w.u64(p.comm_polys.size()); for (auto& c : p.comm_polys) w.point(c);
  w.u64(p.comm_evals.size()); for (auto& c : p.comm_evals) w.point(c);
  w.u64(p.proofs.size());
  for (auto& d : p.proofs) {
    w.point(d.delta); w.point(d.beta);
    w.u64(d.z.size()); for (auto& s : d.z) w.scalar(s);
    w.scalar(d.z_delta); w.scalar(d.z_beta);
  }
}

static int zk_sumcheck(vpin_ctx* c, int K, vpin_table** tabs, const Fq& claim, const Fq& blind_claim, int rounds,
                       const Mcg& g1, const Mcg& gn, Transcript& tr, Transcript& tape, ZkSc& pf, std::vector<Fq>& r_out,
                       Fq* final_claims, Fq& blind_last, const std::vector<Fq>* tau = nullptr,
                       const vpin_table* pyramid = nullptr, int lw = 0) {
  const int nc = (K == 4) ? 4 : 3;
  const bool factored = (K == 4 && tau != nullptr && pyramid != nullptr);
  const int ntab = factored ? 3 : K;
  vpin_comm* cm = lw > 0 ? c->comm : nullptr;
  const int world = cm ? cm->world : 1;
  const int loc_rounds = rounds - lw;
  if (lw > 0 && (!cm || (1 << lw) != world || loc_rounds < 1)) return VPIN_EINVAL;
  Fq c_rank = Fq::one();
  std::vector<Fq> eq_lo;
  if (cm && factored) {
    eq_lo.resize(world);
    host_eq(tau->data() + loc_rounds, (size_t)lw, eq_lo.data());
    c_rank = eq_lo[cm->rank];
  }
  std::vector<std::vector<Fq>> htab;
  Fq s_eq = Fq::one();
  const Fq f_one = Fq::one(), f_two = Fq::from_u64(2), f_three = Fq::from_u64(3), f_five = Fq::from_u64(5);
  std::vector<Fq> blinds_poly = tape.challenge_vector("blinds_poly", rounds);
  std::vector<Fq> blinds_evals = tape.challenge_vector("blinds_evals", rounds);
  struct RoundRand { Fq d[4], r_delta, r_beta; };
  std::vector<RoundRand> rr(rounds);
  for (int j = 0; j < rounds; j++) {
    for (int i = 0; i < nc; i++) rr[j].d[i] = tape.challenge_scalar("d_vec");
    rr[j].r_delta = tape.challenge_scalar("r_delta");
    rr[j].r_beta = tape.challenge_scalar("r_beta");
  }
  std::vector<CG> delta(rounds);
  std::vector<Point> P_bp(rounds), P_be(rounds), P_rb(rounds);
#pragma omp parallel for schedule(dynamic, 1) num_threads(host_threads())
  for (int j = 0; j < rounds; j++) {
    delta[j] = compress(commit(rr[j].d, nc, rr[j].r_delta, gn));
    P_bp[j] = gn.h->mul(blinds_poly[j]);
    P_be[j] = g1.h->mul(blinds_evals[j]);
    P_rb[j] = g1.h->mul(rr[j].r_beta);
  }
  Fq claim_pr = claim;
  CG comm_claim = compress(commit1(claim_pr, blind_claim, g1));
  r_out.clear();
  bool lead = factored;
  std::vector<Fq> tau_inv;
  if (factored) {
    tau_inv.assign(tau->begin(), tau->begin() + rounds);
    for (auto& x : tau_inv) lead = lead && !x.is_zero();
    if (lead) fq_batch_invert(tau_inv.data(), tau_inv.size());
  }
  Fq cn = claim;
  int rc = factored ? vpin::sc_cubic3_launch(c, tabs, pyramid, loc_rounds, 1, nullptr, lead) : vpin::sc_round_launch(c, K, tabs, nullptr);
  if (rc) return rc;
  auto host_round = [&](int j, bool lead_now, Fq e[3]) {
    const size_t len = htab[0].size(), half = len / 2;
    e[0] = e[1] = e[2] = Fq::zero();
    if (factored) {
      std::vector<Fq> E(half);
      host_eq(tau->data() + j + 1, (size_t)(rounds - j - 1), E.data());
      for (size_t i = 0; i < half; i++) {
        const Fq a0 = htab[0][i], a1 = htab[0][i + half], b0 = htab[1][i], b1 = htab[1][i + half], c0 = htab[2][i], c1 = htab[2][i + half];
// ... 630 lines not shown
```

vpin_amd/csrc/spark.cpp:

```cpp
#include <cstdio>

#include "host/prover_common.h"
#include "gadget_dev.h"
#include "spark_dev.h"

namespace {

using namespace vpin_host;
using namespace vpin_prover;

static bool spark_trace() { static const bool on = getenv("VPIN_SPARK_TRACE") != nullptr; return on; }
struct TraceSpan {
  const char* name; Clock::time_point t0;
  explicit TraceSpan(const char* n) : name(n), t0(Clock::now()) {}
  ~TraceSpan() { if (spark_trace()) fprintf(stderr, "[spark] %-28s %8.3f ms\n", name, secs(t0, Clock::now()) * 1e3); }
};


struct SparkGens {
  std::vector<Point> g;
  std::map<size_t, std::unique_ptr<PcGens>> views;
};

static void spark_cache_free(vpin_ctx* c) {
  auto* sg = static_cast<SparkGens*>(c->spark_cache);
  if (!sg) return;
  delete sg;
  c->spark_cache = nullptr;
}

static size_t spark_budget_gb(vpin_ctx* c) {
  if (c->expected_proofs > 0) return (size_t)24;
  static const size_t gb = [c] {
    const char* e = getenv("VPIN_SPARK_GENS_BUDGET_GB");
    if (e && atoi(e) > 0) return (size_t)atoi(e);
    size_t free_b = 0, total_b = 0;
    (void)hipSetDevice(c->device);
    if (hipMemGetInfo(&free_b, &total_b) != hipSuccess) return (size_t)24;
    return free_b >= ((size_t)200 << 30) ? (size_t)80 : (size_t)24;
  }();
  return gb;
}

static int get_view(vpin_ctx* c, size_t ell, const PcGens** out) {
  if (!c->spark_cache) { c->spark_cache = new SparkGens(); c->spark_cache_free = spark_cache_free; }
  auto* sg = static_cast<SparkGens*>(c->spark_cache);
  auto it = sg->views.find(ell);
  if (it == sg->views.end()) {
    const size_t left = ell / 2, R = (size_t)1 << (ell - left), nb = R + 2;
    vpin::TraceLap lap(nullptr, "spark get_view");
    if (sg->g.size() < nb) derive_gens(sg->g, nb, "gens_r1cs_eval", c);
    lap("derive_gens (host)");
    std::unique_ptr<PcGens> v(new PcGens());
    v->ell = ell; v->L = (size_t)1 << left; v->R = R;
    int rc = vpin_gens_shared(c, "gens_r1cs_eval", nullptr, nb, 0, &v->dev);
    if (rc == VPIN_EINVAL) {
      std::vector<uint8_t> xyzt(128 * nb);
#pragma omp parallel for schedule(static) num_threads(host_threads())
      for (long i = 0; i < (long)nb; i++) sg->g[i].to_xyzt(xyzt.data() + 128 * (size_t)i);
      c->gens_scalars_per_proof = (double)((size_t)1 << ell) * 0.375;
      rc = vpin_gens_shared(c, "gens_r1cs_eval", xyzt.data(), nb, spark_budget_gb(c), &v->dev);
    }
    if (rc) return rc;
    lap("device table");
#pragma omp parallel for schedule(static, 1) num_threads(2)
    for (int k = 0; k < 2; k++) {
      if (k == 0) v->fb_gR = FixedBase(sg->g[R]);
      else v->fb_h = FixedBase(sg->g[R + 1]);
    }
    lap("fixed bases (host)");
    v->bind_views();
    it = sg->views.emplace(ell, std::move(v)).first;
  }
  *out = it->second.get();
  return VPIN_OK;
}

struct Shape { size_t nx, ny, N, M, v_ops, v_mem, v_derefs; };

static size_t next_pow2(size_t n) { size_t p = 1; while (p < n) p <<= 1; return p; }

static Shape shape_of(size_t num_cons, size_t num_vars, const size_t nnz[3]) {
  Shape s;
  s.nx = log2z(num_cons);
  s.ny = log2z(2 * num_vars);
  s.N = 1;
  for (int m = 0; m < 3; m++) s.N = std::max(s.N, next_pow2(nnz[m]));
  s.M = (size_t)1 << std::max(s.nx, s.ny);
  s.v_ops = log2z(s.N) + 4;
  s.v_mem = std::max(s.nx, s.ny) + 1;
  s.v_derefs = log2z(s.N) + 3;
  return s;
}

static int commit_noblind(vpin_ctx* c, const PcGens* pc, const vpin_table* Z, std::vector<CG>& out) {
  std::vector<uint8_t> zeros(pc->L * 32, 0);
  out.resize(pc->L);
  return vpin_hyrax_commit(c, pc->dev, Z, zeros.data(), pc->L, pc->R + 1, out[0].b);
}

static void append_polycomm(Transcript& tr, const char* label, const std::vector<CG>& C) {
  tr.append_message(label, "poly_commitment_begin");
  for (auto& p : C) tr.append_point("poly_commitment_share", p.b);
  tr.append_message(label, "poly_commitment_end");
}

static void w_scalars(Writer& w, const Fq* v, size_t n) { w.u64(n); for (size_t i = 0; i < n; i++) w.scalar(v[i]); }

static int polyeval_prove_plain(vpin_ctx* c, const PcGens& pc, const vpin_table* Z, const std::vector<Fq>& r, const Fq& Zr,
                                Transcript& tr, Transcript& tape, DpLog& out, const vpin::fq* z_rows = nullptr,
                                const std::vector<Fq>* lz_pre = nullptr, const std::vector<Fq>* rv_pre = nullptr) {
  if (r.size() != pc.ell || (!(lz_pre && rv_pre) && (!Z || Z->len != ((size_t)1 << pc.ell)))) return VPIN_ESHAPE;
  tr.append_protocol_name("polynomial evaluation proof");
  const size_t left = pc.ell / 2, right = pc.ell - left;
  if (lz_pre && rv_pre) {
    if (lz_pre->size() != pc.R || rv_pre->size() != pc.R) return VPIN_ESHAPE;
    TraceSpan ts("  dplog");
    return dplog_prove(c, pc, tr, tape, *lz_pre, Fq::zero(), *rv_pre, Zr, Fq::zero(), out);
  }
  std::vector<Fq> Lv(pc.L), Rv(pc.R), LZ(pc.R);
  host_eq(r.data(), left, Lv.data());
  host_eq(r.data() + left, right, Rv.data());
  int rc;
  {
    TraceSpan ts("  poly_bound");
    if (c->comm && c->comm->world > 1) rc = vpin::poly_bound_dist(c, Z, B(Lv.data()), pc.L, B(LZ.data()), z_rows);
    else rc = vpin_poly_bound(c, Z, B(Lv.data()), pc.L, B(LZ.data()));
  }
  if (rc) return rc;
  if ((rc = vpin::comm_mark(c, "hash_poly_bound"))) return rc;
  TraceSpan ts("  dplog");
  return dplog_prove(c, pc, tr, tape, LZ, Fq::zero(), Rv, Zr, Fq::zero(), out);
}

struct SlicePass {
  vpin::DevBuf lzs;
  std::vector<Fq> Rv;
  int used = 0, nbits = 0;
  bool on = false;
  explicit SlicePass(vpin_ctx* c) : lzs(c) {}
  static bool fits(const PcGens& pc, int nbits, const std::vector<Fq>& rand) {
    const bool off = getenv("VPIN_HASH_TWO_PASS") != nullptr;
    return !off && pc.ell / 2 >= (size_t)nbits && rand.size() + (size_t)nbits == pc.ell;
  }
  int run(vpin_ctx* c, const PcGens& pc, const uint32_t* table32, int n32, const vpin::fq* table, int nbits_, int used_,
          const std::vector<Fq>& rand, Fq* ev) {
    nbits = nbits_; used = used_;
    const size_t left = pc.ell / 2, T = pc.L >> nbits, N = (size_t)1 << rand.size();
    std::vector<Fq> Ltop(T);
    host_eq(rand.data(), left - (size_t)nbits, Ltop.data());
    Rv.resize(pc.R);
    host_eq(rand.data() + (left - (size_t)nbits), pc.ell - left, Rv.data());
    if (lzs.alloc((size_t)used * pc.R * 32)) return VPIN_ENOMEM;
    int rc = vpin::slices_bound(c, table32, n32, table, N, used, pc.R, B(Ltop.data()), T, B(Rv.data()), (vpin::fq*)lzs.p, B(ev));
    on = rc == VPIN_OK;
    return rc;
  }
  int combine(vpin_ctx* c, const PcGens& pc, const std::vector<Fq>& ch, std::vector<Fq>& LZ) {
    std::vector<Fq> coef((size_t)1 << nbits);
    host_eq(ch.data(), (size_t)nbits, coef.data());
    LZ.resize(pc.R);
    return vpin::slices_combine(c, (const vpin::fq*)lzs.p, used, pc.R, B(coef.data()), B(LZ.data()));
  }
};

struct DistPlan {
  vpin_comm* cm = nullptr;
  int rank = 0, world = 1;
  int owner_ops[12], owner_dotp[6], owner_mem[4];
  std::vector<std::vector<int>> ops_of, dotp_of, mem_of;
  int max_ops_inst = 0, max_mem_inst = 0;
  int lw = 0;
};

static void make_plan(int world, int owner_ops[12], int owner_dotp[6], int owner_mem[4]) {
  std::vector<long> load(world, 0);
  auto least = [&](const std::vector<long>& key2) {
    int best = 0;
    for (int r = 1; r < world; r++)
      if (load[r] < load[best] || (load[r] == load[best] && key2[r] < key2[best])) best = r;
// ... 848 lines not shown
  return 8 * 6 + 8 + 32 * ((size_t)1 << (s.v_ops / 2)) + 8 + 32 * ((size_t)1 << (s.v_mem / 2));
}

size_t vpin_snark_proof_max_bytes(const vpin_r1cs* inst) {
  if (!inst) return 0;
  Shape s = shape_of(inst->num_cons, inst->num_vars, inst->nnz);
  const size_t lgN = log2z(s.N), lgM = log2z(s.M);
  size_t b = vpin_sat_proof_max_bytes(inst->num_cons, inst->num_vars) + 96;
  b += 8 + 32 * ((size_t)1 << (s.v_derefs / 2)) + 64 * 32;
  b += lgN * (lgN * 104 + 64 + 24 * 32 + 64) + 18 * 32 + 64;
  b += lgM * (lgM * 104 + 64 + 8 * 32 + 64) + 64;
  b += 3 * (16 + 64 * 40 + 128 + 64) + 40 * 32 + 1024;
  return b;
}

int vpin_spark_prepare(vpin_ctx* c, size_t num_cons, size_t num_vars, size_t max_nnz) {
  if (!c || !vpin::is_pow2(num_cons) || !vpin::is_pow2(num_vars) || max_nnz == 0) return VPIN_EINVAL;
  (void)hipSetDevice(c->device);
  const size_t nnz[3] = {max_nnz, max_nnz, max_nnz};
  const Shape s = shape_of(num_cons, num_vars, nnz);
  const PcGens* g = nullptr;
  int rc = get_view(c, std::max(s.v_ops, s.v_mem), &g);
  if (!rc) {
    auto* sg = static_cast<SparkGens*>(c->spark_cache);
    std::vector<size_t> idx;
    for (size_t ell : {s.v_ops, s.v_mem, s.v_derefs}) {
      const size_t R = (size_t)1 << (ell - ell / 2);
      if (R + 1 < sg->g.size()) { idx.push_back(R); idx.push_back(R + 1); }
    }
#pragma omp parallel for schedule(dynamic, 1) num_threads(host_threads())
    for (long k = 0; k < (long)idx.size(); k++) { FixedBase warm(sg->g[idx[(size_t)k]]); (void)warm; }
  }
  if (!rc) rc = get_view(c, s.v_ops, &g);
  if (!rc) rc = get_view(c, s.v_mem, &g);
  if (!rc) rc = get_view(c, s.v_derefs, &g);
  return rc;
}

int vpin_spark_gens_view(vpin_ctx* c, size_t ell, const vpin_gens** out, size_t* L, size_t* R) {
  if (!c || !out || !L || !R || ell < 2 || ell > 40) return VPIN_EINVAL;
  (void)hipSetDevice(c->device);
  const PcGens* g = nullptr;
  int rc = get_view(c, ell, &g);
  if (rc) return rc;
  *out = g->dev; *L = g->L; *R = g->R;
  return VPIN_OK;
}

int vpin_dist_plan(int world, int owner_ops[12], int owner_dotp[6], int owner_mem[4]) {
  if (world < 1 || world > 12 || !owner_ops || !owner_dotp || !owner_mem) return VPIN_EINVAL;
  make_plan(world, owner_ops, owner_dotp, owner_mem);
  return VPIN_OK;
}

void vpin_spark_decomm_hot_cols(const vpin_spark_decomm* d, uint32_t out[3]) {
  for (int m = 0; m < 3; m++) out[m] = d ? d->hot_col[m] : 0xffffffffu;
}

void vpin_spark_decomm_free(vpin_ctx* c, vpin_spark_decomm* d) {
  if (!d) return;
  if (c) {
    (void)hipSetDevice(c->device);
    if (d->idx) vpin::dev_free(c, d->idx);
    if (d->vals) vpin::dev_free(c, d->vals);
    if (d->comb_ops) vpin_table_free(c, d->comb_ops);
    if (d->comb_mem) vpin_table_free(c, d->comb_mem);
  }
  delete d;
}

static int encode_commit(vpin_ctx* c, const Shape& s, std::unique_ptr<vpin_spark_decomm>& d, vpin::TraceLap& lap, size_t num_cons,
                         size_t num_vars, size_t num_inputs, vpin_spark_decomm** out, uint8_t* comm_out, size_t comm_cap,
                         size_t* comm_len, Clock::time_point t0) {
  auto fail = [&](int rc) { vpin_spark_decomm_free(c, d.release()); return rc; };
  int rc;
  const PcGens *g_ops = nullptr, *g_mem = nullptr;
  if ((rc = get_view(c, std::max(s.v_ops, s.v_mem), &g_ops)) || (rc = get_view(c, s.v_ops, &g_ops)) ||
      (rc = get_view(c, s.v_mem, &g_mem)))
    return fail(rc);
  lap("generators (views)");
  std::vector<CG> c_ops, c_mem;
  if ((rc = vpin::spark_comb_tables(c, d.get()))) return fail(rc);
  lap("comb tables");
  if ((rc = commit_noblind(c, g_ops, d->comb_ops, c_ops))) return fail(rc);
  lap("commit ops");
  if ((rc = commit_noblind(c, g_mem, d->comb_mem, c_mem))) return fail(rc);
  lap("commit mem");
  vpin::spark_comb_release(c, d.get(), false);
  lap("comb release");
  if ((rc = vpin::spark_find_hot_cols(c, d.get()))) return fail(rc);
  lap("hot columns");
  Writer w;
  w.u64(num_cons); w.u64(num_vars); w.u64(num_inputs);
  w.u64(3); w.u64(s.N); w.u64(s.M);
  w.u64(c_ops.size()); for (auto& p : c_ops) w.point(p);
  w.u64(c_mem.size()); for (auto& p : c_mem) w.point(p);
  if (w.buf.size() > comm_cap) return fail(VPIN_ESHAPE);
  memcpy(comm_out, w.buf.data(), w.buf.size());
  *comm_len = w.buf.size();
  *out = d.release();
  g_spark_timings[0] = secs(t0, Clock::now());
  return VPIN_OK;
}

int vpin_spark_encode(vpin_ctx* c, const vpin_r1cs* inst, vpin_spark_decomm** out, uint8_t* comm_out, size_t comm_cap,
                      size_t* comm_len) {
  if (!c || !inst || !out || !comm_out || !comm_len) return VPIN_EINVAL;
  if (!vpin::is_pow2(inst->num_cons) || !vpin::is_pow2(inst->num_vars) || inst->num_inputs >= inst->num_vars) return VPIN_ESHAPE;
  auto t0 = Clock::now();
  (void)hipSetDevice(c->device);
  const Shape s = shape_of(inst->num_cons, inst->num_vars, inst->nnz);
  const size_t N = s.N, M = s.M;
  if (N < 4 || M < 4 || M > ((size_t)1 << 32) || N > ((size_t)1 << 31)) return VPIN_ESHAPE;
  if (comm_cap < vpin_spark_comm_bytes(inst)) return VPIN_ESHAPE;
  for (int m = 0; m < 3; m++)
    if (inst->nnz[m] && (!inst->row[m] || !inst->col[m] || !inst->val[m])) return VPIN_EINVAL;
  std::unique_ptr<vpin_spark_decomm> d(new vpin_spark_decomm());
  d->num_cons = inst->num_cons; d->num_vars = inst->num_vars; d->num_inputs = inst->num_inputs;
  d->nx = s.nx; d->ny = s.ny; d->N = N; d->M = M;
  auto fail = [&](int rc) { vpin_spark_decomm_free(c, d.release()); return rc; };

  vpin::TraceLap lap(c, "spark_encode");
  int rc;
  if ((rc = vpin::dev_alloc(c, (12 * N + 2 * M) * 4, (void**)&d->idx))) return fail(rc);
  vpin::DevBuf b_bad(c);
  if (b_bad.alloc(4)) return fail(VPIN_ENOMEM);
  if (hipMemsetAsync(b_bad.p, 0, 4, c->stream) != hipSuccess) return fail(VPIN_EHIP);
  for (int side = 0; side < 2; side++) {
    uint32_t* addr = d->idx + (size_t)side * 6 * N;
    if (hipMemsetAsync(addr, 0, 3 * N * 4, c->stream) != hipSuccess) return fail(VPIN_EHIP);
    for (int m = 0; m < 3; m++) {
      const uint32_t* src = side ? inst->col[m] : inst->row[m];
      if (inst->nnz[m] && hipMemcpyAsync(addr + (size_t)m * N, src, inst->nnz[m] * 4, hipMemcpyHostToDevice, c->stream) != hipSuccess)
        return fail(VPIN_EHIP);
      if ((rc = vpin::spark_check_bounds(c, addr + (size_t)m * N, inst->nnz[m], (uint32_t)(side ? 2 * inst->num_vars : inst->num_cons),
                                         (uint32_t*)b_bad.p)))
        return fail(rc);
    }
    if ((rc = vpin::spark_trace_timestamps(c, addr, 3 * N, M, addr + 3 * N, d->idx + 12 * N + (size_t)side * M))) return fail(rc);
  }
  uint32_t bad = 0;
  if (hipMemcpyAsync(&bad, b_bad.p, 4, hipMemcpyDeviceToHost, c->stream) != hipSuccess || hipStreamSynchronize(c->stream) != hipSuccess)
    return fail(VPIN_EHIP);
  if (bad) return fail(VPIN_ESHAPE);
  b_bad.release();
  lap("device idx + timestamps");
  if ((rc = vpin::dev_alloc(c, 3 * N * 32, (void**)&d->vals))) return fail(rc);
  if (hipMemsetAsync(d->vals, 0, 3 * N * 32, c->stream) != hipSuccess) return fail(VPIN_EHIP);
  for (int m = 0; m < 3; m++)
    if (inst->nnz[m] && hipMemcpyAsync(d->vals + (size_t)m * N, inst->val[m], inst->nnz[m] * 32, hipMemcpyHostToDevice,
                                       c->stream) != hipSuccess)
      return fail(VPIN_EHIP);
  if (hipStreamSynchronize(c->stream) != hipSuccess) return fail(VPIN_EHIP);
  lap("upload + comb tables");

  return encode_commit(c, s, d, lap, inst->num_cons, inst->num_vars, inst->num_inputs, out, comm_out, comm_cap, comm_len, t0);
}

int vpin_spark_encode_dev(vpin_ctx* c, const vpin_dev_instance* g, vpin_spark_decomm** out, uint8_t* comm_out, size_t comm_cap,
                          size_t* comm_len) {
  if (!c || !g || !g->r1cs || !out || !comm_out || !comm_len) return VPIN_EINVAL;
  auto t0 = Clock::now();
  (void)hipSetDevice(c->device);
  const size_t num_cons = g->r1cs->num_cons, num_vars = g->r1cs->num_vars;
  const Shape s = shape_of(num_cons, num_vars, g->nnz);
  const size_t N = s.N, M = s.M;
  if (N < 4 || M < 4 || M > ((size_t)1 << 32) || N > ((size_t)1 << 31)) return VPIN_ESHAPE;
  if (comm_cap < vpin_dev_instance_comm_bytes(g)) return VPIN_ESHAPE;
  std::unique_ptr<vpin_spark_decomm> d(new vpin_spark_decomm());
// ... 173 lines not shown
```

vpin_amd/csrc/verify.cpp:

```cpp
#include <sys/random.h>

#include <functional>

#include "host/prover_common.h"

namespace {

using namespace vpin_host;
using namespace vpin_prover;

struct VSpan {
  const char* name;
  std::chrono::steady_clock::time_point t0;
  static bool on() { static const bool v = getenv("VPIN_VERIFY_TRACE") != nullptr; return v; }
  explicit VSpan(const char* n) : name(n), t0(std::chrono::steady_clock::now()) {}
  ~VSpan() {
    if (on()) fprintf(stderr, "[verify] %-28s %8.3f ms\n", name, std::chrono::duration<double, std::milli>(std::chrono::steady_clock::now() - t0).count());
  }
};

struct Deferred {
  std::vector<std::function<bool()>> jobs;
  void add(std::function<bool()> f) { jobs.push_back(std::move(f)); }
  bool run() {
// ... 295 lines not shown
    const Fq mz = (pf.z1 * sk->w).neg();
    s.resize(n);
    for (size_t i = 0; i < n; i++) s[i] = s[i] * mz;
    sk->tab.push_back(Sink::Tab{&pc, std::move(s)});
    return true;
  }
  Point G_hat;
  if (msm_rows_host_sum(c, pc.dev, s.data(), 1, n + 2, &G_hat)) return false;
  Fq a_hat = Fq::zero();
  for (size_t i = 0; i < n; i++) a_hat = a_hat + a[i] * s[i];
  Point Gamma_hat = Gamma;
  {
    std::vector<Point> term(lg);
    bool dec_ok = true;
#pragma omp parallel for schedule(dynamic, 1) num_threads(host_threads()) reduction(&& : dec_ok)
    for (long i = 0; i < (long)lg; i++) {
      Point pl, pr;
      const bool ok_i = decompress(pl, pf.Lv[(size_t)i]) && decompress(pr, pf.Rv[(size_t)i]);
      if (ok_i) term[(size_t)i] = Point::mul2(usq[(size_t)i], pl, uisq[(size_t)i], pr);
      dec_ok = dec_ok && ok_i;
    }
    if (!dec_ok) return false;
    for (size_t i = 0; i < lg; i++) Gamma_hat = Gamma_hat + term[i];
  }
  tr.append_point("delta", pf.delta.b);
  tr.append_point("beta", pf.beta.b);
  Fq cc = tr.challenge_scalar("c");
  Point pb, pd;
  if (!decompress(pb, pf.beta) || !decompress(pd, pf.delta)) return false;
  Point lhs = (Gamma_hat.mul(cc) + pb).mul(a_hat) + pd;
  Point rhs = (G_hat + Gs.mul(a_hat)).mul(pf.z1) + pc.fb_h.mul(pf.z2);
  return lhs.equals(rhs);
}

static bool polyeval_verify(vpin_ctx* c, const DpLogP& pf, const PcGens& pc, Transcript& tr, const Fq* r, const CG& C_Zr,
                            const std::vector<CG>& comm, Sink* sk) {
  if (comm.size() != pc.L) return false;
  VSpan vs(" polyeval");
  tr.append_protocol_name("polynomial evaluation proof");
  const size_t left = pc.ell / 2, right = pc.ell - left;
  std::vector<Fq> Lv(pc.L), Rv(pc.R);
  host_eq(r, left, Lv.data());
  host_eq(r + left, right, Rv.data());
  CG C_LZ;
  static const bool host_only = getenv("VPIN_VERIFY_HOST_MSM") != nullptr;
  bool on_device = false;
  if (pc.L >= 128 && !host_only) {
    int rc;
    {
      DevLock lock(sk);
      rc = vpin_msm(c, B(Lv.data()), comm[0].b, pc.L, C_LZ.b, nullptr);
    }
    if (rc == VPIN_EVERIFY) return false;
    on_device = rc == VPIN_OK;
  }
  if (!on_device) {
    std::vector<Point> Cd(pc.L);
    bool ok = true;
#pragma omp parallel for schedule(static) num_threads(!sk && pc.L >= 64 ? host_threads() : 1) reduction(&& : ok)
    for (long i = 0; i < (long)pc.L; i++) ok = ok && decompress(Cd[i], comm[i]);
    if (!ok) return false;
    C_LZ = compress(msm_var(Lv.data(), Cd.data(), pc.L, !sk));
  }
  return dplog_verify(c, pf, pc, tr, Rv, C_LZ, C_Zr, sk);
}
static bool polyeval_verify_plain(vpin_ctx* c, const DpLogP& pf, const PcGens& pc, Transcript& tr, const Fq* r, const Fq& Zr,
                                  const std::vector<CG>& comm, Sink* sk) {
  CG C_Zr = compress(commit1(Zr, Fq::zero(), pc.gens_1));
  return polyeval_verify(c, pf, pc, tr, r, C_Zr, comm, sk);
}


struct SatGensV {
  size_t ell, L, R;
  std::vector<Point> g;
  FixedBase fb[5];
  PcGens pc;
  Mcg gens_1, gens_3, gens_4;
};

static int make_pc(vpin_ctx* c, const char* label, const std::vector<Point>& g, size_t ell, size_t budget_gb, PcGens& pc) {
  const size_t left = ell / 2, R = (size_t)1 << (ell - left), nb = R + 2;
  pc.ell = ell; pc.L = (size_t)1 << left; pc.R = R;
  int rc = vpin_gens_shared(c, label, nullptr, nb, 0, &pc.dev);
  if (rc == VPIN_EINVAL) {
    std::vector<uint8_t> xyzt(128 * nb);
    for (size_t i = 0; i < nb; i++) g[i].to_xyzt(xyzt.data() + 128 * i);
    rc = vpin_gens_shared(c, label, xyzt.data(), nb, budget_gb, &pc.dev);
  }
  if (rc) return rc;
  pc.fb_gR = FixedBase(g[R]);
  pc.fb_h = FixedBase(g[R + 1]);
  pc.bind_views();
  return VPIN_OK;
}

struct VCache {
  std::map<size_t, std::unique_ptr<SatGensV>> sat;
  std::vector<Point> g_eval;
  std::map<size_t, std::unique_ptr<PcGens>> eval_views;
};
static void vcache_free(vpin_ctx* c) {
  delete static_cast<VCache*>(c->verify_cache);
  c->verify_cache = nullptr;
}
static VCache* vcache(vpin_ctx* c) {
  if (!c->verify_cache) { c->verify_cache = new VCache(); c->verify_cache_free = vcache_free; }
  return static_cast<VCache*>(c->verify_cache);
}

static int sat_gens_v(vpin_ctx* c, size_t num_vars, SatGensV** out) {
  VCache* vc = vcache(c);
  auto it = vc->sat.find(num_vars);
  if (it != vc->sat.end()) { *out = it->second.get(); return VPIN_OK; }
  VSpan vs("setup: sat generators");
  std::unique_ptr<SatGensV> sgp(new SatGensV());
  SatGensV& sg = *sgp;
  sg.ell = log2z(num_vars);
  const size_t left = sg.ell / 2;
  sg.L = (size_t)1 << left;
  sg.R = (size_t)1 << (sg.ell - left);
  const size_t nb = sg.R + 2 < 5 ? 5 : sg.R + 2;
  derive_gens(sg.g, nb, "gens_r1cs_sat", c);
  for (int i = 0; i < 5; i++) sg.fb[i] = FixedBase(sg.g[i]);
  int rc = make_pc(c, "gens_r1cs_sat", sg.g, sg.ell, 0, sg.pc);
  if (rc) return rc;
  sg.gens_1 = sg.pc.gens_1;
  sg.gens_3 = Mcg{3, {&sg.fb[0], &sg.fb[1], &sg.fb[2], nullptr}, &sg.fb[3]};
  sg.gens_4 = Mcg{4, {&sg.fb[0], &sg.fb[1], &sg.fb[2], &sg.fb[3]}, &sg.fb[4]};
  *out = sgp.get();
  vc->sat[num_vars] = std::move(sgp);
  return VPIN_OK;
}

static int eval_view_v(vpin_ctx* c, size_t ell, const PcGens** out) {
  VCache* vc = vcache(c);
  auto it = vc->eval_views.find(ell);
  if (it != vc->eval_views.end()) { *out = it->second.get(); return VPIN_OK; }
  VSpan vs("setup: eval generators");
  const size_t nb = ((size_t)1 << (ell - ell / 2)) + 2;
  if (vc->g_eval.size() < nb) derive_gens(vc->g_eval, nb, "gens_r1cs_eval", c);
  std::unique_ptr<PcGens> v(new PcGens());
  int rc = make_pc(c, "gens_r1cs_eval", vc->g_eval, ell, 0, *v);
  if (rc) return rc;
  *out = v.get();
  vc->eval_views[ell] = std::move(v);
  return VPIN_OK;
}

static bool sat_verify(vpin_ctx* c, Reader& r, size_t num_cons, size_t num_vars, const Fq* inputs, size_t num_inputs,
                       const Fq* inst_evals_in, Fq inst_evals[3], const uint8_t* comm_para, const uint8_t* comm_input,
                       Transcript& tr, std::vector<Fq>& rx, std::vector<Fq>& ry, int* err, Sink* sk = nullptr) {
  SatGensV* sgp = nullptr;
  if ((*err = sat_gens_v(c, num_vars, &sgp))) return false;
  SatGensV& sg = *sgp;
  const size_t L = sg.L;
  const int nrx = (int)log2z(num_cons), nry = (int)log2z(2 * num_vars);
  std::vector<CG> comm_vars;
  if (!r.points(comm_vars, L)) return false;
  ZkScP sc1, sc2;
  if (!read_zksc(r, sc1, nrx, 3)) return false;
  CG comm_Az = r.point(), comm_Bz = r.point(), comm_Cz = r.point(), comm_prod = r.point();
  KnowP pok; pok.alpha = r.point(); pok.z1 = r.scalar(); pok.z2 = r.scalar();
  ProdP pp; pp.alpha = r.point(); pp.beta = r.point(); pp.delta = r.point();
  for (int i = 0; i < 5; i++) pp.z[i] = r.scalar();
  EqP eq1; eq1.alpha = r.point(); eq1.z = r.scalar();
  if (!read_zksc(r, sc2, nry, 2)) return false;
// ... 579 lines not shown
```

Before: 71.63 million constraints/s.

## Add windowed row-table MSM kernel with signed digits for Hyrax row commits

Adds a per-generator row table (fixed window size per row, signed-digit recoding) and a new msm_rows_win kernel. The kernel stages digits in LDS, walks table entries per window with prefetching, then tree-reduces per window and finishes with a Horner combine. Sat and SPARK generator tables are now built with the row-table variant, and the SPARK ops/mem commits use a walk-only path. The aim is to replace the bucket/strip MSM path with fixed-base precomputation so fewer point additions are needed per row, at the cost of more table memory and build time.

```diff
diff --git a/include/vpin_hip.h b/include/vpin_hip.h
--- a/include/vpin_hip.h
+++ b/include/vpin_hip.h
@@ -32,6 +32,7 @@
 int vpin_ctx_set_progress_flag(vpin_ctx* ctx, int* flag);
 int vpin_ctx_set_shared_device(vpin_ctx* ctx, int on);
 unsigned long long vpin_ctx_strip_rows_taken(vpin_ctx* ctx);
+unsigned long long vpin_ctx_row_table_rows(vpin_ctx* ctx);
 unsigned long long vpin_ctx_pip_row_chunks(vpin_ctx* ctx);
 int vpin_ctx_pool_stats(vpin_ctx* ctx, size_t out[3]);
 int vpin_driver_alloc_stats(unsigned long long out[2]);
@@ -88,6 +89,9 @@
 void vpin_gens_free(vpin_ctx* ctx, vpin_gens* g);
 size_t vpin_gens_count(const vpin_gens* g);
 int vpin_gens_layout(const vpin_gens* g, size_t out[6]);
+int vpin_gens_row_layout(const vpin_gens* g, size_t out[4]);
+int vpin_hyrax_commit_derefs(vpin_ctx* ctx, const vpin_gens* g, const vpin_table* Z, size_t L, size_t N, const uint32_t* col_idx,
+                             const uint32_t hot[3], const vpin_table* e_ry, uint8_t* out_compressed);
 size_t vpin_gens_entry_bytes(void);
 int vpin_hyrax_commit(vpin_ctx* ctx, const vpin_gens* g, const vpin_table* Z, const uint8_t* blinds,
                       size_t L, size_t blind_base, uint8_t* out_compressed );
diff --git a/vpin_amd/capi.py b/vpin_amd/capi.py
--- a/vpin_amd/capi.py
+++ b/vpin_amd/capi.py
@@ -692,6 +692,12 @@
         L.vpin_ctx_pip_row_chunks.restype = C.c_ulonglong
         return int(L.vpin_ctx_pip_row_chunks(self.h))
 
+    def row_table_rows(self):
+        L = lib()
+        L.vpin_ctx_row_table_rows.argtypes = [C.c_void_p]
+        L.vpin_ctx_row_table_rows.restype = C.c_ulonglong
+        return int(L.vpin_ctx_row_table_rows(self.h))
+
     def strip_rows_taken(self):
         L = lib()
         L.vpin_ctx_strip_rows_taken.argtypes = [C.c_void_p]
@@ -806,6 +812,17 @@
         out = np.zeros((Ls, 32), dtype=np.uint8)
         _chk(lib().vpin_hyrax_commit(self.h, gens.h, Z.h, b.ctypes.data_as(C.c_void_p), Ls, blind_base,
                                      out.ctypes.data_as(C.c_void_p)), "vpin_hyrax_commit")
+        return out
+
+    def hyrax_commit_derefs(self, gens, Z, Ls, N, col_idx, hot, e_ry):
+        idx = np.ascontiguousarray(col_idx, dtype=np.uint32).reshape(3 * N)
+        h = (C.c_uint32 * 3)(*[0xFFFFFFFF if x is None else int(x) for x in hot])
+        out = np.zeros((Ls, 32), dtype=np.uint8)
+        L = lib()
+        L.vpin_hyrax_commit_derefs.argtypes = [C.c_void_p, C.c_void_p, C.c_void_p, C.c_size_t, C.c_size_t, C.c_void_p, C.c_void_p,
+                                               C.c_void_p, C.c_void_p]
+        _chk(L.vpin_hyrax_commit_derefs(self.h, gens.h, Z.h, Ls, N, idx.ctypes.data_as(C.c_void_p), h, e_ry.h,
+                                        out.ctypes.data_as(C.c_void_p)), "vpin_hyrax_commit_derefs")
         return out
 
     def hyrax_commit_pippenger(self, gens, Z, blinds, blind_base, Ls=None, c_bits=0):
diff --git a/vpin_amd/csrc/capi.hip b/vpin_amd/csrc/capi.hip
--- a/vpin_amd/csrc/capi.hip
+++ b/vpin_amd/csrc/capi.hip
@@ -379,6 +379,7 @@
 }
 
 unsigned long long vpin_ctx_strip_rows_taken(vpin_ctx* c) { return c ? c->strip_rows_taken : 0ull; }
+unsigned long long vpin_ctx_row_table_rows(vpin_ctx* c) { return c ? c->row_table_rows : 0ull; }
 unsigned long long vpin_ctx_pip_row_chunks(vpin_ctx* c) { return c ? c->pip_row_chunks : 0ull; }
 
 int vpin_host_register(void* p, size_t bytes) {
diff --git a/vpin_amd/csrc/ctx.h b/vpin_amd/csrc/ctx.h
--- a/vpin_amd/csrc/ctx.h
+++ b/vpin_amd/csrc/ctx.h
@@ -87,6 +87,7 @@
   vpin::fq tail_sums[3 * 18];
   vpin::fq tail_final[6 * 18];
   unsigned long long pip_row_chunks = 0;
+  unsigned long long row_table_rows = 0;
   unsigned long long strip_rows_taken = 0;
   bool low_memory = false;
   bool shared_device = false;
@@ -163,6 +164,9 @@
 
 inline bool is_pow2(size_t x) { return x && !(x & (x - 1)); }
 
+int hyrax_commit_walk(vpin_ctx* c, const vpin_gens* g, const vpin_table* Z, const uint8_t* blinds, size_t L, size_t blind_base,
+                      uint8_t* out_compressed);
+int gens_shared_rows(vpin_ctx* c, const char* label, const uint8_t* gens_xyzt, size_t nb, size_t budget_gb, const vpin_gens** out);
 int gens_msm_parts_dev(vpin_ctx* c, const vpin_gens* g, const fq* d_scalars, size_t rows, size_t ncols, uint8_t* parts_xyzt);
 int hyrax_commit_derefs_hot(vpin_ctx* c, const vpin_gens* g, const vpin_table* Z, size_t L, size_t N, const uint32_t* const col_idx[3],
                             const uint32_t hot[3], const fq* e_ry, uint8_t* out_compressed, size_t row0 = 0, size_t nrows = (size_t)-1,
diff --git a/vpin_amd/csrc/ge_tree_dev.h b/vpin_amd/csrc/ge_tree_dev.h
--- a/vpin_amd/csrc/ge_tree_dev.h
+++ b/vpin_amd/csrc/ge_tree_dev.h
@@ -90,33 +90,47 @@
   for (int i = 0; i < 8; i++) r.v[i] = c ? a.v[i] : b.v[i];
   return r;
 }
+__device__ __forceinline__ void ge_quad_add_into(ge_ext* sh, int i, int j, int role, int qbase) {
+  const fp* shf = reinterpret_cast<const fp*>(sh);
+  fp* shw = reinterpret_cast<fp*>(sh);
+  const int f0 = role < 2 ? 1 : (role == 2 ? 3 : 2);
+  const fp p0 = shf[4 * i + f0], q0 = shf[4 * j + f0];
+  fp u = p0, v = q0;
+  if (role < 2) {
+    const fp p1 = shf[4 * i], q1 = shf[4 * j];
+    u = fp_pick(role == 0, fp_sub(p0, p1), fp_add(p0, p1));
+    v = fp_pick(role == 0, fp_sub(q0, q1), fp_add(q0, q1));
+  }
+  fp m = fp_mul(u, v);
+  m = fp_mul(m, fp_pick(role == 2, FP_D2(), fp_one()));
+  m = fp_pick(role == 3, fp_add(m, m), m);
+  const fp a = fp_shfl_from(m, qbase), b = fp_shfl_from(m, qbase + 1), c = fp_shfl_from(m, qbase + 2),
+           d = fp_shfl_from(m, qbase + 3);
+  const fp E = fp_sub(b, a), H = fp_add(b, a), F = fp_sub(d, c), G = fp_add(d, c);
+  u = fp_pick(role == 0 || role == 3, E, fp_pick(role == 1, G, F));
+  v = fp_pick(role == 0, F, fp_pick(role == 2, G, H));
+  shw[4 * i + role] = fp_mul(u, v);
+}
 __device__ __forceinline__ void ge_tree_quad(ge_ext* sh, int n, int split = 0) {
   const int role = threadIdx.x & 3, qbase = (threadIdx.x & 63) & ~3;
-  const fp* shf = reinterpret_cast<const fp*>(sh);
-  fp* shw = reinterpret_cast<fp*>(sh);
   for (int s = n / 2; s >= 1; s >>= 1) {
     if (s == split) continue;
     const int items = s < split ? 2 * s : s;
     for (int w = threadIdx.x >> 2; w < items; w += (int)(blockDim.x >> 2)) {
       const int i = w < s ? w : split + (w - s);
-      const int f0 = role < 2 ? 1 : (role == 2 ? 3 : 2);
-      const fp p0 = shf[4 * i + f0], q0 = shf[4 * (i + s) + f0];
-      fp u = p0, v = q0;
-      if (role < 2) {
-        const fp p1 = shf[4 * i], q1 = shf[4 * (i + s)];
-        u = fp_pick(role == 0, fp_sub(p0, p1), fp_add(p0, p1));
-        v = fp_pick(role == 0, fp_sub(q0, q1), fp_add(q0, q1));
-      }
-      fp m = fp_mul(u, v);
-      m = fp_mul(m, fp_pick(role == 2, FP_D2(), fp_one()));
-      m = fp_pick(role == 3, fp_add(m, m), m);
-      const fp a = fp_shfl_from(m, qbase), b = fp_shfl_from(m, qbase + 1), c = fp_shfl_from(m, qbase + 2),
-               d = fp_shfl_from(m, qbase + 3);
-      const fp E = fp_sub(b, a), H = fp_add(b, a), F = fp_sub(d, c), G = fp_add(d, c);
-      u = fp_pick(role == 0 || role == 3, E, fp_pick(role == 1, G, F));
-      v = fp_pick(role == 0, F, fp_pick(role == 2, G, H));
-      shw[4 * i + role] = fp_mul(u, v);
+      ge_quad_add_into(sh, i, i + s, role, qbase);
     }
+    __syncthreads();
+  }
+}
+__device__ __forceinline__ void ge_tree_quad_strided(ge_ext* sh, int n, int W) {
+  const int role = threadIdx.x & 3, qbase = (threadIdx.x & 63) & ~3;
+  int P = 1;
+  while (P * W < n) P <<= 1;
+  for (int s = P / 2; s >= 1; s >>= 1) {
+    const int items = s * W;
+    for (int i = threadIdx.x >> 2; i < items; i += (int)(blockDim.x >> 2))
+      if (i + items < n) ge_quad_add_into(sh, i, i + items, role, qbase);
     __syncthreads();
   }
 }
diff --git a/vpin_amd/csrc/msm.hip b/vpin_amd/csrc/msm.hip
--- a/vpin_amd/csrc/msm.hip
+++ b/vpin_amd/csrc/msm.hip
@@ -28,6 +28,10 @@
   size_t split = 0;
   int c = 12, W = 22, E = 2048;
   int c_hi = 8, W_hi = 32, E_hi = 128;
+  vpin::fp* table_row = nullptr;
+  size_t n_row = 0;
+  int c_row = 0, W_row = 0, E_row = 0;
+  bool narrowed = false;
 };
 
 namespace vpin {
@@ -53,6 +57,16 @@
   if (j < tv.split) return TableSeg{tv.t, j, tv.split, tv.c, tv.W, tv.E, tv.s32};
   return TableSeg{tv.t_hi, j - tv.split, tv.nbt - tv.split, tv.c_hi, tv.W_hi, tv.E_hi, tv.s32};
 }
+
+struct RowTable {
+  const fp* t;
+  size_t n;
+  int c, W, E, s32;
+  __device__ __forceinline__ const ge_niels* entry(size_t j, uint32_t d) const {
+    return reinterpret_cast<const ge_niels*>(t + (j * (size_t)E + d) * (size_t)s32);
+  }
+};
+constexpr int row_windows(int c) { return (253 + c - 1) / c; }
 
 
 __global__ __launch_bounds__(256) void gens_sum_kernel(fp* __restrict__ xyzt, size_t nb) {
@@ -509,6 +523,172 @@
   ge_store(o, a);
 }
 
+constexpr int kRowLdsBytes = 48 * 1024;
+constexpr uint16_t kNoDigit = 0xffffu;
+static inline int row_segment(int W) { return ((kRowLdsBytes / 2) / W) & ~3; }
+
+__device__ __forceinline__ uint16_t row_digit(fq& s, uint32_t& carry, int c, bool flip, bool top) {
+  const uint32_t mask = (1u << c) - 1u, half = 1u << (c - 1);
+  const uint32_t v = (s.v[0] & mask) + carry;
+#pragma unroll
+  for (int i = 0; i < 7; i++) s.v[i] = __builtin_amdgcn_alignbit(s.v[i + 1], s.v[i], c);
+  s.v[7] >>= c;
+  const bool neg = !top && (flip ? v >= half : v > half);
+  const uint32_t mag = neg ? (mask + 1u) - v : v;
+  carry = neg ? 1u : 0u;
+  return mag ? (uint16_t)((mag - 1u) | ((neg != flip) ? 0x8000u : 0u)) : kNoDigit;
+}
+
+__global__ __launch_bounds__(kMsmBlock, 3) void msm_rows_win_kernel(const fq* __restrict__ Z, size_t stride, size_t ncols,
+                                                                     const fq* __restrict__ extra, int n_extra, size_t extra_base0,
+                                                                     TableView tv, RowTable rt, HotRows hr, int segn,
+                                                                     ge_ext* __restrict__ parts, size_t row_base, size_t row_step,
+                                                                     int z_compact) {
+  const size_t row = row_base + (size_t)blockIdx.x * row_step;
+  const fq* zr = Z + (z_compact ? (size_t)blockIdx.x : row) * stride;
+  const fq* xr = extra + (size_t)blockIdx.x * (size_t)n_extra;
+  const int W = rt.W;
+  ge_ext* o = parts + ((size_t)blockIdx.x * gridDim.y + blockIdx.y) * (size_t)W;
+  __shared__ __align__(16) unsigned char lds[kRowLdsBytes];
+  __shared__ uint32_t n_hot;
+  if (ncols >= 256 && (ncols & (ncols - 1)) == 0 && ((size_t)1 << (tv.nbt - tv.sum0 - 1)) >= ncols) {
+    const fq first = fq_load(zr);
+    if (fq_eq(first, fq_load(zr + 1)) && fq_eq(first, fq_load(zr + ncols / 2)) && fq_eq(first, fq_load(zr + ncols - 1))) {
+      int same = 1;
+      for (size_t j = threadIdx.x; j < ncols; j += kMsmBlock) same &= fq_eq(first, fq_load(zr + j)) ? 1 : 0;
+      if (__syncthreads_and(same)) {
+        if (threadIdx.x == 0) {
+          RowAcc acc;
+          if (blockIdx.y == 0) {
+            if (!fq_is_zero(first)) acc.mul_acc(fq_from_mont(first), tv, tv.sum0 + (size_t)(63 - __builtin_clzll((unsigned long long)ncols)));
+            for (int e = 0; e < n_extra; e++) {
+              const fq x = fq_load(xr + e);
+              if (!fq_is_zero(x)) acc.mul_acc(fq_from_mont(x), tv, extra_base0 + e);
+            }
+          }
+          ge_store(o, acc.ext());
+        } else if ((int)threadIdx.x < W) {
+          ge_store_identity(o + threadIdx.x);
+        }
+        return;
+      }
+    }
+  }
+  const uint32_t* idx = nullptr;
+  const ge_cached* T = nullptr;
+  uint32_t hot = 0xffffffffu;
+  if (hr.rows_per_vec && row >= hr.row0 && row < hr.row0 + 3 * hr.rows_per_vec) {
+    const size_t m = (row - hr.row0) / hr.rows_per_vec;
+    if (hr.hot[m] != 0xffffffffu) {
+      hot = hr.hot[m];
+      T = hr.T[m];
+      idx = hr.idx[m] + (row - hr.row0 - m * hr.rows_per_vec) * ncols;
+    }
+  }
+  const size_t total = ncols + (size_t)n_extra;
+  const size_t per = (total + gridDim.y - 1) / gridDim.y;
+  const size_t j0 = (size_t)blockIdx.y * per, j1 = (j0 + per < total) ? j0 + per : total;
+  const int w = (int)threadIdx.x % W, r = (int)threadIdx.x / W, nw = (kMsmBlock - 1 - w + W) / W;
+  uint16_t* dig = reinterpret_cast<uint16_t*>(lds);
+  ge10 acc = ge10_identity();
+  for (size_t seg = j0; seg < j1; seg += (size_t)segn) {
+    const uint32_t n = (uint32_t)((seg + (size_t)segn < j1) ? (size_t)segn : j1 - seg);
+    for (uint32_t jl = threadIdx.x; jl < n; jl += kMsmBlock) {
+      const size_t j = seg + jl;
+      fq s = fq_load(j < ncols ? zr + j : xr + (j - ncols));
+      const bool live = !fq_is_zero(s) && !(idx && j < ncols && idx[j] == hot);
+      bool flip = false;
+      if (live) {
+        s = fq_from_mont(s);
+        flip = fq_fold_sign(s);
+      }
+      uint32_t carry = 0;
+#pragma unroll 1
+      for (int ww = 0; ww < W; ww++) {
+        uint16_t d = kNoDigit;
+        if (live) d = row_digit(s, carry, rt.c, flip, ww == W - 1);
+        dig[(size_t)ww * segn + jl] = d;
+      }
+    }
+    __syncthreads();
+    const uint16_t* dg = dig + (size_t)w * segn;
+    uint32_t k = (uint32_t)r;
+    auto fetch = [&](ge_niels& e, bool& neg) -> bool {
+      while (k < n) {
+        const uint32_t kk = k;
+        k += (uint32_t)nw;
+        const uint16_t d = dg[kk];
+        if (d != kNoDigit) {
+          const size_t j = seg + kk;
+          e = ge_load(rt.entry(j < ncols ? j : extra_base0 + (j - ncols), d & 0x7fffu));
+          neg = (d >> 15) != 0;
+          return true;
+        }
+      }
+      return false;
+    };
+    ge_niels e_cur;
+    bool neg_cur = false;
+    bool have_cur = fetch(e_cur, neg_cur);
+    while (have_cur) {
+      ge_niels e_next;
+      bool neg_next = false;
+      const bool have_next = fetch(e_next, neg_next);
+      acc = ge10_add_niels(acc, e_cur, neg_cur);
+      e_cur = e_next;
+      neg_cur = neg_next;
+      have_cur = have_next;
+    }
+    __syncthreads();
+  }
+  ge_ext* sh = reinterpret_cast<ge_ext*>(lds);
+  sh[threadIdx.x] = ge10_to_ext(acc);
+  __syncthreads();
+  ge_tree_quad_strided(sh, kMsmBlock, W);
+  ge_ext mine = ge_identity();
+  if ((int)threadIdx.x < W) mine = sh[threadIdx.x];
+  __syncthreads();
+  if (idx) {
+    uint16_t* list = reinterpret_cast<uint16_t*>(lds);
+    RowAcc hacc;
+    uint32_t any = 0;
+    const size_t c1 = j1 < ncols ? j1 : ncols;
+    for (size_t seg = j0; seg < c1; seg += kSeg) {
+      const size_t seg_end = (seg + kSeg < c1) ? seg + kSeg : c1;
+      if (threadIdx.x == 0) n_hot = 0;
+      __syncthreads();
+      for (size_t j = seg + threadIdx.x; j < seg_end; j += kMsmBlock)
+        if (idx[j] == hot && !fq_is_zero(fq_load(zr + j))) list[atomicAdd(&n_hot, 1u)] = (uint16_t)(j - seg);
+      __syncthreads();
+      const uint32_t nh = n_hot;
+      any |= nh;
+      for (uint32_t kk = threadIdx.x; kk < nh; kk += kMsmBlock) hacc.add_cached(ge_load(T + seg + list[kk]));
+      __syncthreads();
+    }
+    if (any) {
+      sh[threadIdx.x] = hacc.ext();
+      __syncthreads();
+      ge_tree_quad(sh, kMsmBlock);
+      if (threadIdx.x == 0) mine = ge_add(mine, sh[0]);
+    }
+  }
+  if ((int)threadIdx.x < W) ge_store(o + threadIdx.x, mine);
+}
+
+__global__ __launch_bounds__(64) void msm_rows_finish_kernel(ge_ext* __restrict__ parts, size_t rows, int chunks, int W, int c,
+                                                             ge_ext* __restrict__ out) {
+  const size_t i = (size_t)blockIdx.x * blockDim.x + threadIdx.x;
+  if (i >= rows) return;
+  ge_ext* p = parts + i * (size_t)chunks * (size_t)W;
+  if (chunks > 1)
+    for (int w = 0; w < W; w++) {
+      ge_ext a = ge_load(p + w);
+      for (int k = 1; k < chunks; k++) a = ge_add(a, ge_load(p + (size_t)k * W + w));
+      ge_store(p + w, a);
+    }
+  ge_store(out + i, ge10_to_ext(ge10_horner_windows(p, W, [c](int) { return c; })));
+}
+
 __device__ __forceinline__ uint32_t count_digits(fq s, const TableView& tv, size_t j) {
   (void)fq_fold_sign(s);
   const TableSeg sg = table_seg(tv, j);
@@ -523,11 +703,17 @@
   }
   return n;
 }
+__device__ __forceinline__ uint32_t count_digits_row(fq s, int c, int W) {
+  const bool flip = fq_fold_sign(s);
+  uint32_t carry = 0, n = 0;
+  for (int w = 0; w < W; w++) n += row_digit(s, carry, c, flip, w == W - 1) != kNoDigit;
+  return n;
+}
 __global__ __launch_bounds__(kMsmBlock) void msm_count_adds_kernel(const fq* __restrict__ Z, size_t stride, size_t ncols,
                                                                    const fq* __restrict__ extra, int n_extra, size_t extra_base0,
                                                                    TableView tv, unsigned long long* __restrict__ count,
                                                                    HotRows hr = HotRows{}, size_t row_base = 0, size_t row_step = 1,
-                                                                   int z_compact = 0) {
+                                                                   int z_compact = 0, int c_row = 0, int W_row = 0) {
   const size_t row = row_base + (size_t)blockIdx.x * row_step;
   const fq* zr = Z + (z_compact ? (size_t)blockIdx.x : row) * stride;
   const uint32_t* hidx = nullptr;
@@ -549,11 +735,11 @@
   if (!constant)
     for (size_t j = threadIdx.x; j < ncols; j += kMsmBlock) {
       const fq s = fq_load(zr + j);
-      if (!fq_is_zero(s) && !(hidx && hidx[j] == hot)) n += count_digits(fq_from_mont(s), tv, j);
+      if (!fq_is_zero(s) && !(hidx && hidx[j] == hot)) n += c_row ? count_digits_row(fq_from_mont(s), c_row, W_row) : count_digits(fq_from_mont(s), tv, j);
     }
   for (int e = threadIdx.x; e < n_extra; e += kMsmBlock) {
     const fq x = fq_load(extra + row * (size_t)n_extra + e);
-    if (!fq_is_zero(x)) n += count_digits(fq_from_mont(x), tv, extra_base0 + e);
+    if (!fq_is_zero(x)) n += (c_row && !constant) ? count_digits_row(fq_from_mont(x), c_row, W_row) : count_digits(fq_from_mont(x), tv, extra_base0 + e);
   }
   __shared__ uint32_t sh[kMsmBlock];
   sh[threadIdx.x] = n;
@@ -833,9 +1019,9 @@
 
 extern "C" {
 
-static int gens_build_once(vpin_ctx* c, const uint8_t* gens_xyzt, size_t nb, size_t budget, int cmax, vpin_gens** out);
-
-static int gens_build(vpin_ctx* c, const uint8_t* gens_xyzt, size_t nb, size_t budget, vpin_gens** out) {
+static int gens_build_once(vpin_ctx* c, const uint8_t* gens_xyzt, size_t nb, size_t budget, int cmax, bool row_policy, vpin_gens** out);
+
+static int gens_build(vpin_ctx* c, const uint8_t* gens_xyzt, size_t nb, size_t budget, bool row_policy, vpin_gens** out) {
   (void)hipSetDevice(c->device);
   size_t free_b = 0, total_b = 0;
   const hipError_t e_info = c->expected_proofs > 0 ? hipErrorUnknown : hipMemGetInfo(&free_b, &total_b);
@@ -857,7 +1043,7 @@
     }
   }
   for (;;) {
-    int rc = gens_build_once(c, gens_xyzt, nb, budget, cmax, out);
+    int rc = gens_build_once(c, gens_xyzt, nb, budget, cmax, row_policy, out);
     if (rc != VPIN_ENOMEM || budget <= floor_b) return rc;
     (void)hipGetLastError();
     budget /= 2;
@@ -871,7 +1057,18 @@
   return v == 128 ? 128 : v == 96 ? 96 : (size_t)VPIN_NIELS_SLOT;
 }
 
-static int gens_build_once(vpin_ctx* c, const uint8_t* gens_xyzt, size_t nb, size_t budget, int cmax, vpin_gens** out) {
+static int row_table_forced_bits() {
+  const char* e = getenv("VPIN_ROW_TABLE_C");
+  const int v = e ? atoi(e) : 0;
+  return v >= 4 && v <= 16 ? v : 0;
+}
+static bool row_table_off() {
+  const char* e = getenv("VPIN_ROW_TABLE");
+  return e && atoi(e) == 0;
+}
+constexpr size_t kRowTableMinBases = 4096;
+
+static int gens_build_once(vpin_ctx* c, const uint8_t* gens_xyzt, size_t nb, size_t budget, int cmax, bool row_policy, vpin_gens** out) {
   if (!c || !gens_xyzt || !out || nb == 0) return VPIN_EINVAL;
   const size_t slot = table_slot_bytes();
   (void)hipSetDevice(c->device);
@@ -904,17 +1101,36 @@
       fit(nbt - kSplitBases, budget - lo_bytes, g->c, &g->c_hi, &g->W_hi, &g->E_hi);
     }
   }
+  const size_t n_row = std::min(nb, kSplitBases);
+  int c_row = row_table_forced_bits();
+  if (!c_row && row_policy && !row_table_off() && c->expected_proofs == 0 && nb >= kRowTableMinBases) {
+    const size_t mw8 = nbt * (size_t)32 * 128 * slot;
+    for (int cc = 16; cc >= 13 && !c_row; cc--)
+      if (n_row * ((size_t)1 << (cc - 1)) * slot + mw8 <= budget) c_row = cc;
+    if (c_row) {
+      g->split = nbt;
+      g->c = 8; g->W = 32; g->E = 128;
+      g->narrowed = true;
+    }
+  }
+  if (c_row) {
+    g->n_row = n_row;
+    g->c_row = c_row; g->W_row = row_windows(c_row); g->E_row = 1 << (c_row - 1);
+  }
+  const size_t entries_row = g->n_row * (size_t)g->E_row;
   const size_t n_hi = nbt - g->split;
   const size_t entries = g->split * (size_t)g->W * g->E, entries_hi = n_hi * (size_t)g->W_hi * g->E_hi;
-  const size_t max_entries = entries > entries_hi ? entries : entries_hi;
+  const size_t max_entries = std::max(std::max(entries, entries_hi), entries_row);
   const size_t max_shifts = std::max(g->split * (size_t)g->W, n_hi * (size_t)g->W_hi);
   TraceLap lap(c, "gens_build");
   DevBuf raw(c), b_shifts(c), b_prefix(c);
   if (raw.alloc(nbt * 128) != VPIN_OK || b_shifts.alloc(max_shifts * sizeof(ge_ext)) != VPIN_OK ||
       b_prefix.alloc(max_entries * sizeof(fp)) != VPIN_OK || driver_malloc((void**)&g->table, entries * slot) != hipSuccess ||
-      (n_hi && driver_malloc((void**)&g->table_hi, entries_hi * slot) != hipSuccess)) {
+      (n_hi && driver_malloc((void**)&g->table_hi, entries_hi * slot) != hipSuccess) ||
+      (entries_row && driver_malloc((void**)&g->table_row, entries_row * slot) != hipSuccess)) {
     if (g->table) (void)hipFree(g->table);
     if (g->table_hi) (void)hipFree(g->table_hi);
+    if (g->table_row) (void)hipFree(g->table_row);
     delete g;
     return VPIN_ENOMEM;
   }
@@ -935,6 +1151,9 @@
       hipLaunchKernelGGL(gens_table_kernel, dim3((unsigned)((n_hi * g->W_hi + 63) / 64)), dim3(64), 0, c->stream, shifts, n_hi,
                          g->W_hi, g->E_hi, g->table_hi, g->s32, prefix);
     }
+    if (entries_row)
+      hipLaunchKernelGGL(gens_table_kernel, dim3((unsigned)((g->n_row + 63) / 64)), dim3(64), 0, c->stream, (const ge_ext*)raw.p, g->n_row, 1,
+                         g->E_row, g->table_row, g->s32, prefix);
     e = hipGetLastError();
   }
   if (e == hipSuccess) e = hipStreamSynchronize(c->stream);
@@ -948,6 +1167,7 @@
     set_last_error("vpin_gens_create", e);
     (void)hipFree(g->table);
     if (g->table_hi) (void)hipFree(g->table_hi);
+    if (g->table_row) (void)hipFree(g->table_row);
     delete g;
     return VPIN_EHIP;
   }
@@ -965,7 +1185,7 @@
 }
 
 int vpin_gens_create(vpin_ctx* c, const uint8_t* gens_xyzt, size_t nb, vpin_gens** out) {
-  return gens_build(c, gens_xyzt, nb, default_budget(), out);
+  return gens_build(c, gens_xyzt, nb, default_budget(), false, out);
 }
 
 int vpin_gens_map_stream(vpin_ctx* c, const uint8_t* stream64, size_t nb, uint8_t* out_xyzt) {
@@ -982,21 +1202,21 @@
 }
 
 namespace {
-struct RegEntry { int device; std::string label; vpin_gens* g; };
-struct Building { int device; std::string label; size_t nb; };
+struct RegEntry { int device; std::string label; vpin_gens* g; bool rows; };
+struct Building { int device; std::string label; size_t nb; bool rows; };
 std::mutex g_reg_mu;
 std::condition_variable g_reg_cv;
 std::vector<RegEntry> g_reg;
 std::vector<Building> g_building;
 }
 
-int vpin_gens_shared(vpin_ctx* c, const char* label, const uint8_t* gens_xyzt, size_t nb, size_t budget_gb,
-                     const vpin_gens** out) {
+static int gens_shared_impl(vpin_ctx* c, const char* label, const uint8_t* gens_xyzt, size_t nb, size_t budget_gb, bool rows,
+                            const vpin_gens** out) {
   if (!c || !label || !out || nb == 0) return VPIN_EINVAL;
   auto lookup = [&]() -> const vpin_gens* {
     const vpin_gens* best = nullptr;
     for (auto& e : g_reg)
-      if (e.device == c->device && e.label == label && e.g->nb >= nb && (!best || e.g->nb < best->nb)) best = e.g;
+      if (e.device == c->device && e.label == label && (rows || !e.g->narrowed) && e.g->nb >= nb && (!best || e.g->nb < best->nb)) best = e.g;
     return best;
   };
   {
@@ -1004,7 +1224,7 @@
     for (;;) {
       if (const vpin_gens* best = lookup()) { *out = best; return VPIN_OK; }
       bool covered = false;
-      for (auto& b : g_building) covered = covered || (b.device == c->device && b.label == label && b.nb >= nb);
+      for (auto& b : g_building) covered = covered || (b.device == c->device && b.label == label && (rows || !b.rows) && b.nb >= nb);
       if (!covered) break;
       g_reg_cv.wait(lock);
     }
@@ -1014,19 +1234,24 @@
       if (e.device == c->device && e.label == label && !said.exchange(true))
         fprintf(stderr, "vpin_gens_shared: a table of \"%s\" for %zu generators is built beside the one for %zu (both stay allocated): "
                         "call vpin_spark_prepare / vpin_sat_prepare with the largest shape first\n", label, nb, e.g->nb);
-    g_building.push_back(Building{c->device, label, nb});
+    g_building.push_back(Building{c->device, label, nb, rows});
   }
   vpin_gens* g = nullptr;
-  const int rc = gens_build(c, gens_xyzt, nb, budget_gb ? (budget_gb << 30) : default_budget(), &g);
+  const int rc = gens_build(c, gens_xyzt, nb, budget_gb ? (budget_gb << 30) : default_budget(), rows, &g);
   std::lock_guard<std::mutex> lock(g_reg_mu);
   for (size_t i = 0; i < g_building.size(); i++)
-    if (g_building[i].device == c->device && g_building[i].label == label && g_building[i].nb == nb) { g_building.erase(g_building.begin() + (long)i); break; }
+    if (g_building[i].device == c->device && g_building[i].label == label && g_building[i].nb == nb && g_building[i].rows == rows) { g_building.erase(g_building.begin() + (long)i); break; }
   if (!rc) {
-    g_reg.push_back(RegEntry{c->device, label, g});
+    g_reg.push_back(RegEntry{c->device, label, g, rows});
     *out = g;
   }
   g_reg_cv.notify_all();
   return rc;
+}
+
+int vpin_gens_shared(vpin_ctx* c, const char* label, const uint8_t* gens_xyzt, size_t nb, size_t budget_gb,
+                     const vpin_gens** out) {
+  return gens_shared_impl(c, label, gens_xyzt, nb, budget_gb, false, out);
 }
 
 size_t vpin_gens_shared_bytes(int device) {
@@ -1035,7 +1260,8 @@
   for (auto& e : g_reg)
     if (e.device == device)
       total += (size_t)32 * (size_t)e.g->s32 * ((size_t)e.g->W * e.g->split * (size_t)e.g->E +
-                                     (e.g->split < e.g->nbt ? (size_t)e.g->W_hi * (e.g->nbt - e.g->split) * (size_t)e.g->E_hi : 0));
+                                     (e.g->split < e.g->nbt ? (size_t)e.g->W_hi * (e.g->nbt - e.g->split) * (size_t)e.g->E_hi : 0) +
+                                     e.g->n_row * (size_t)e.g->E_row);
   return total;
 }
 
@@ -1046,6 +1272,7 @@
     (void)hipDeviceSynchronize();
     if (e.g->table) (void)hipFree(e.g->table);
     if (e.g->table_hi) (void)hipFree(e.g->table_hi);
+    if (e.g->table_row) (void)hipFree(e.g->table_row);
     delete e.g;
   }
   g_reg.clear();
@@ -1056,6 +1283,7 @@
   if (c) { (void)hipSetDevice(c->device); (void)hipStreamSynchronize(c->stream); }
   if (g->table) (void)hipFree(g->table);
   if (g->table_hi) (void)hipFree(g->table_hi);
+  if (g->table_row) (void)hipFree(g->table_row);
   delete g;
 }
 
@@ -1064,6 +1292,11 @@
   if (!g || !out) return VPIN_EINVAL;
   out[0] = (size_t)g->c; out[1] = (size_t)g->W; out[2] = g->split;
   out[3] = g->split < g->nbt ? (size_t)g->c_hi : 0; out[4] = g->split < g->nbt ? (size_t)g->W_hi : 0; out[5] = g->nbt;
+  return VPIN_OK;
+}
+int vpin_gens_row_layout(const vpin_gens* g, size_t out[4]) {
+  if (!g || !out) return VPIN_EINVAL;
+  out[0] = (size_t)g->c_row; out[1] = (size_t)g->W_row; out[2] = g->n_row; out[3] = g->c_row ? (size_t)row_segment(g->W_row) : 0;
   return VPIN_OK;
 }
 size_t vpin_gens_entry_bytes(void) { return table_slot_bytes(); }
@@ -1093,8 +1326,46 @@
   return env_pad >= 0 ? (unsigned)env_pad : (c->shared_device ? kSharedPad : 0u);
 }
 
+static inline RowTable row_view(const vpin_gens* g) {
+  return RowTable{g->table_row, g->n_row, g->c_row, g->W_row, g->E_row, g->s32};
+}
+
+static size_t row_table_min_scalars() {
+  const char* e = getenv("VPIN_MSM_ROW_MIN");
+  return e ? (size_t)atoll(e) : (size_t)1 << 24;
+}
+static bool row_table_use(const vpin_ctx* c, const vpin_gens* g, size_t rows, size_t ncols, int n_extra, size_t extra_base0) {
+  if (!g->table_row || c->comm != nullptr) return false;
+  const char* e = getenv("VPIN_MSM_ROW_TABLE");
+  if (e && atoi(e) == 0) return false;
+  if (ncols > g->n_row || (n_extra && extra_base0 + (size_t)n_extra > g->n_row)) return false;
+  return rows * (ncols + (size_t)n_extra) >= row_table_min_scalars();
+}
+
+static int msm_rows_win(vpin_ctx* c, const vpin_gens* g, const fq* dZ, size_t rows, size_t stride, size_t ncols, const fq* d_extra,
+                        int n_extra, size_t extra_base0, const HotRows& hr, size_t row_base, size_t row_step, int z_compact,
+                        ge_ext* d_points) {
+  const RowTable rt = row_view(g);
+  const int segn = row_segment(rt.W);
+  c->row_table_rows += rows;
+  const size_t total = ncols + (size_t)n_extra;
+  const size_t most = std::max<size_t>(1, total / ((size_t)segn * 2));
+  size_t want = rows >= 768 ? 1 : (768 + rows - 1) / rows;
+  if (rows >= 768 && total > (size_t)kSeg) want = std::min<size_t>(8, (total + kSeg - 1) / kSeg);
+  const char* ec = getenv("VPIN_MSM_ROW_WIN_CHUNKS");
+  const int chunks = ec && atoi(ec) > 0 ? std::min(atoi(ec), 64) : (int)std::max<size_t>(1, std::min<size_t>(64, std::min(want, most)));
+  DevBuf parts(c);
+  if (parts.alloc(rows * (size_t)chunks * (size_t)rt.W * sizeof(ge_ext))) return VPIN_ENOMEM;
+  hipLaunchKernelGGL(msm_rows_win_kernel, dim3((unsigned)rows, (unsigned)chunks), dim3(kMsmBlock), msm_lds_pad(c), c->stream, dZ, stride,
+                     ncols, d_extra, n_extra, extra_base0, view(g), rt, hr, segn, (ge_ext*)parts.p, row_base, row_step, z_compact);
+  hipLaunchKernelGGL(msm_rows_finish_kernel, dim3((unsigned)((rows + 63) / 64)), dim3(64), 0, c->stream, (ge_ext*)parts.p, rows, chunks,
+                     rt.W, rt.c, d_points);
+  VPIN_HIP_TRY(hipGetLastError());
+  return VPIN_OK;
+}
+
 static int msm_rows(vpin_ctx* c, const vpin_gens* g, const fq* dZ, size_t rows, size_t stride, size_t ncols,
-                    const fq* d_extra, int n_extra, size_t extra_base0, ge_ext* d_points) {
+                    const fq* d_extra, int n_extra, size_t extra_base0, ge_ext* d_points, bool walk_only = false) {
   if (const int pm = pip_mode())
     if (n_extra <= 1 && ncols + (size_t)n_extra <= 32768)
       return msm_rows_pip(c, g, dZ, rows, stride, ncols, d_extra, n_extra, extra_base0, pm < 0 ? 0 : pm, d_points);
@@ -1112,15 +1383,21 @@
     chunks = (int)(want < most ? want : most);
     if (chunks < 1) chunks = 1;
   }
+  const bool use_row = !walk_only && row_table_use(c, g, rows, ncols, n_extra, extra_base0);
   DevBuf parts(c);
   ge_ext* dst = d_points;
-  if (chunks > 1) {
+  if (chunks > 1 && !use_row) {
     if (parts.alloc(rows * (size_t)chunks * sizeof(ge_ext))) return VPIN_ENOMEM;
     dst = (ge_ext*)parts.p;
   }
   if (c->prof_count_adds && c->d_add_count && rows >= 128)
     hipLaunchKernelGGL(msm_count_adds_kernel, dim3((unsigned)rows), dim3(kMsmBlock), 0, c->stream, dZ, stride, ncols, d_extra,
-                       n_extra, extra_base0, view(g), c->d_add_count);
+                       n_extra, extra_base0, view(g), c->d_add_count, HotRows{}, (size_t)0, (size_t)1, 0, use_row ? g->c_row : 0,
+                       use_row ? g->W_row : 0);
+  if (use_row) {
+    ProfScope ps(c, VPIN_K_MSM, 32.0 * nz_est, rows >= 128 ? VPIN_K_MSM_ROWS : -1);
+    return msm_rows_win(c, g, dZ, rows, stride, ncols, d_extra, n_extra, extra_base0, HotRows{}, 0, 1, 0, d_points);
+  }
   {
     ProfScope ps(c, VPIN_K_MSM, 32.0 * nz_est, rows >= 128 ? VPIN_K_MSM_ROWS : -1);
     hipLaunchKernelGGL(msm_rows_kernel, dim3((unsigned)rows, (unsigned)chunks), dim3(kMsmBlock), msm_lds_pad(c), c->stream, dZ, stride, ncols,
@@ -1146,14 +1423,14 @@
 }
 
 static int commit_rows(vpin_ctx* c, const vpin_gens* g, const fq* z, size_t rows, size_t stride, size_t R, const uint8_t* blinds,
-                       size_t blind_base, bool buckets, int c_bits, uint8_t* out_compressed) {
+                       size_t blind_base, bool buckets, int c_bits, uint8_t* out_compressed, bool walk_only = false) {
   (void)hipSetDevice(c->device);
   const int n_extra = blinds ? 1 : 0;
   DevBuf dbl(c), dpts(c);
   if ((blinds && dbl.alloc(rows * 32)) || dpts.alloc(rows * sizeof(ge_ext))) return VPIN_ENOMEM;
   if (blinds) VPIN_HIP_TRY(hipMemcpyAsync(dbl.p, blinds, rows * 32, hipMemcpyHostToDevice, c->stream));
   const int rc = buckets ? msm_rows_pip(c, g, z, rows, stride, R, (const fq*)dbl.p, n_extra, blind_base, c_bits, (ge_ext*)dpts.p)
-                         : msm_rows(c, g, z, rows, stride, R, (const fq*)dbl.p, n_extra, blind_base, (ge_ext*)dpts.p);
+                         : msm_rows(c, g, z, rows, stride, R, (const fq*)dbl.p, n_extra, blind_base, (ge_ext*)dpts.p, walk_only);
   if (rc) return rc;
   return compress_to_host(c, (const ge_ext*)dpts.p, rows, out_compressed);
 }
@@ -1246,15 +1523,23 @@
     for (int m = 0; m < 3; m++)
       if (hot[m] == distinct[k]) hr.T[m] = Tk;
   }
+  const char* es = getenv("VPIN_MSM_STRIP");
+  const char* em = getenv("VPIN_MSM_STRIP_MIN");
+  const bool use_row = !es && !em && row_table_use(c, g, nrows, R, 0, 0);
   if (c->prof_count_adds && c->d_add_count)
     hipLaunchKernelGGL(msm_count_adds_kernel, dim3((unsigned)nrows), dim3(kMsmBlock), 0, c->stream, zbase, R, R, (const fq*)nullptr, 0,
-                       (size_t)0, view(g), c->d_add_count, hr, row0, row_step, z_compact);
+                       (size_t)0, view(g), c->d_add_count, hr, row0, row_step, z_compact, use_row ? g->c_row : 0, use_row ? g->W_row : 0);
+  if (use_row) {
+    {
+      ProfScope ps(c, VPIN_K_MSM, 32.0 * (double)(nrows * R), VPIN_K_MSM_ROWS);
+      if (const int rc = msm_rows_win(c, g, zbase, nrows, R, R, nullptr, 0, 0, hr, row0, row_step, z_compact, (ge_ext*)dpts.p)) return rc;
+    }
+    return compress_to_host(c, (const ge_ext*)dpts.p, nrows, out_compressed);
+  }
   static const int env_chunks = [] { const char* e = getenv("VPIN_MSM_HOT_CHUNKS"); return e ? atoi(e) : 0; }();
   const int chunks = env_chunks > 0 ? env_chunks : (int)std::max<size_t>(1, std::min<size_t>(8, R / kSeg));
   DevBuf dparts(c);
   if (chunks > 1 && dparts.alloc(nrows * (size_t)chunks * sizeof(ge_ext))) return VPIN_ENOMEM;
-  const char* es = getenv("VPIN_MSM_STRIP");
-  const char* em = getenv("VPIN_MSM_STRIP_MIN");
   const int env_strip = es ? atoi(es) : -1;
   const size_t min_rows = em ? (size_t)atol(em) : 8192, min_list = em ? (size_t)1 : 4096, min_R = em ? (size_t)64 : 4096;
   int S = env_strip > 0 ? env_strip : 16;
@@ -1319,6 +1604,19 @@
   return compress_to_host(c, (const ge_ext*)dpts.p, nrows, out_compressed);
 }
 
+int hyrax_commit_walk(vpin_ctx* c, const vpin_gens* g, const vpin_table* Z, const uint8_t* blinds, size_t L, size_t blind_base,
+                      uint8_t* out_compressed) {
+  if (!c || !g || !Z || !Z->d || !blinds || !out_compressed || L == 0) return VPIN_EINVAL;
+  if (Z->len % L != 0) return VPIN_ESHAPE;
+  const size_t R = Z->len / L;
+  if (R > g->nb || blind_base >= g->nb) return VPIN_ESHAPE;
+  return commit_rows(c, g, Z->d, L, R, R, blinds, blind_base, false, 0, out_compressed, true);
+}
+
+int gens_shared_rows(vpin_ctx* c, const char* label, const uint8_t* gens_xyzt, size_t nb, size_t budget_gb, const vpin_gens** out) {
+  return gens_shared_impl(c, label, gens_xyzt, nb, budget_gb, true, out);
+}
+
 int hyrax_commit_rows_strided(vpin_ctx* c, const vpin_gens* g, const vpin_table* Z, size_t L, size_t row0, size_t nrows, size_t row_step,
                               uint8_t* out_compressed, const fq* z_rows) {
   if (!c || !g || !Z || (!Z->d && !z_rows) || !out_compressed || L == 0 || row_step == 0) return VPIN_EINVAL;
@@ -1333,6 +1631,21 @@
 }
 
 extern "C" {
+
+int vpin_hyrax_commit_derefs(vpin_ctx* c, const vpin_gens* g, const vpin_table* Z, size_t L, size_t N, const uint32_t* col_idx,
+                             const uint32_t hot[3], const vpin_table* e_ry, uint8_t* out_compressed) {
+  if (!c || !g || !Z || !Z->d || !col_idx || !hot || !e_ry || !e_ry->d || !out_compressed || L == 0 || N == 0) return VPIN_EINVAL;
+  for (size_t i = 0; i < 3 * N; i++)
+    if (col_idx[i] >= e_ry->len) return VPIN_ESHAPE;
+  for (int m = 0; m < 3; m++)
+    if (hot[m] != 0xffffffffu && hot[m] >= e_ry->len) return VPIN_ESHAPE;
+  (void)hipSetDevice(c->device);
+  DevBuf didx(c);
+  if (didx.alloc(3 * N * sizeof(uint32_t))) return VPIN_ENOMEM;
+  VPIN_HIP_TRY(hipMemcpyAsync(didx.p, col_idx, 3 * N * sizeof(uint32_t), hipMemcpyHostToDevice, c->stream));
+  const uint32_t* const idx[3] = {(const uint32_t*)didx.p, (const uint32_t*)didx.p + N, (const uint32_t*)didx.p + 2 * N};
+  return vpin::hyrax_commit_derefs_hot(c, g, Z, L, N, idx, hot, (const fq*)e_ry->d, out_compressed);
+}
 
 int vpin_hyrax_commit_pair(vpin_ctx* c, const vpin_gens* g, const vpin_table* Za, const vpin_table* Zb,
                            const uint8_t* blinds_a, const uint8_t* blinds_b, size_t L, size_t blind_base,
diff --git a/vpin_amd/csrc/prover.cpp b/vpin_amd/csrc/prover.cpp
--- a/vpin_amd/csrc/prover.cpp
+++ b/vpin_amd/csrc/prover.cpp
@@ -51,12 +51,12 @@
   sg->gens_1 = sg->pc.gens_1;
   sg->gens_3 = Mcg{3, {&sg->fb[0], &sg->fb[1], &sg->fb[2], nullptr}, &sg->fb[3]};
   sg->gens_4 = Mcg{4, {&sg->fb[0], &sg->fb[1], &sg->fb[2], &sg->fb[3]}, &sg->fb[4]};
-  int rc = vpin_gens_shared(c, "gens_r1cs_sat", nullptr, sg->nb, 0, &sg->dev);
+  int rc = vpin::gens_shared_rows(c, "gens_r1cs_sat", nullptr, sg->nb, 0, &sg->dev);
   if (rc == VPIN_EINVAL) {
     std::vector<uint8_t> xyzt(128 * sg->nb);
     for (size_t i = 0; i < sg->nb; i++) sg->g[i].to_xyzt(xyzt.data() + 128 * i);
     c->gens_scalars_per_proof = (double)num_vars;
-    rc = vpin_gens_shared(c, "gens_r1cs_sat", xyzt.data(), sg->nb, 0, &sg->dev);
+    rc = vpin::gens_shared_rows(c, "gens_r1cs_sat", xyzt.data(), sg->nb, 0, &sg->dev);
   }
   if (rc) return rc;
   lap("fixed bases + table");
diff --git a/vpin_amd/csrc/spark.cpp b/vpin_amd/csrc/spark.cpp
--- a/vpin_amd/csrc/spark.cpp
+++ b/vpin_amd/csrc/spark.cpp
@@ -53,13 +53,13 @@
     lap("derive_gens (host)");
     std::unique_ptr<PcGens> v(new PcGens());
     v->ell = ell; v->L = (size_t)1 << left; v->R = R;
-    int rc = vpin_gens_shared(c, "gens_r1cs_eval", nullptr, nb, 0, &v->dev);
+    int rc = vpin::gens_shared_rows(c, "gens_r1cs_eval", nullptr, nb, 0, &v->dev);
     if (rc == VPIN_EINVAL) {
       std::vector<uint8_t> xyzt(128 * nb);
 #pragma omp parallel for schedule(static) num_threads(host_threads())
       for (long i = 0; i < (long)nb; i++) sg->g[i].to_xyzt(xyzt.data() + 128 * (size_t)i);
       c->gens_scalars_per_proof = (double)((size_t)1 << ell) * 0.375;
-      rc = vpin_gens_shared(c, "gens_r1cs_eval", xyzt.data(), nb, spark_budget_gb(c), &v->dev);
+      rc = vpin::gens_shared_rows(c, "gens_r1cs_eval", xyzt.data(), nb, spark_budget_gb(c), &v->dev);
     }
     if (rc) return rc;
     lap("device table");
@@ -93,9 +93,10 @@
   return s;
 }
 
-static int commit_noblind(vpin_ctx* c, const PcGens* pc, const vpin_table* Z, std::vector<CG>& out) {
+static int commit_noblind(vpin_ctx* c, const PcGens* pc, const vpin_table* Z, std::vector<CG>& out, bool short_scalars = false) {
   std::vector<uint8_t> zeros(pc->L * 32, 0);
   out.resize(pc->L);
+  if (short_scalars) return vpin::hyrax_commit_walk(c, pc->dev, Z, zeros.data(), pc->L, pc->R + 1, out[0].b);
   return vpin_hyrax_commit(c, pc->dev, Z, zeros.data(), pc->L, pc->R + 1, out[0].b);
 }
 
@@ -1110,9 +1111,9 @@
   std::vector<CG> c_ops, c_mem;
   if ((rc = vpin::spark_comb_tables(c, d.get()))) return fail(rc);
   lap("comb tables");
-  if ((rc = commit_noblind(c, g_ops, d->comb_ops, c_ops))) return fail(rc);
+  if ((rc = commit_noblind(c, g_ops, d->comb_ops, c_ops, true))) return fail(rc);
   lap("commit ops");
-  if ((rc = commit_noblind(c, g_mem, d->comb_mem, c_mem))) return fail(rc);
+  if ((rc = commit_noblind(c, g_mem, d->comb_mem, c_mem, true))) return fail(rc);
   lap("commit mem");
   vpin::spark_comb_release(c, d.get(), false);
   lap("comb release");
diff --git a/vpin_amd/csrc/verify.cpp b/vpin_amd/csrc/verify.cpp
--- a/vpin_amd/csrc/verify.cpp
+++ b/vpin_amd/csrc/verify.cpp
@@ -401,7 +401,8 @@
 static int make_pc(vpin_ctx* c, const char* label, const std::vector<Point>& g, size_t ell, size_t budget_gb, PcGens& pc) {
   const size_t left = ell / 2, R = (size_t)1 << (ell - left), nb = R + 2;
   pc.ell = ell; pc.L = (size_t)1 << left; pc.R = R;
-  int rc = vpin_gens_shared(c, label, nullptr, nb, 0, &pc.dev);
+  int rc = vpin::gens_shared_rows(c, label, nullptr, nb, 0, &pc.dev);
+  if (rc == VPIN_EINVAL) rc = vpin_gens_shared(c, label, nullptr, nb, 0, &pc.dev);
   if (rc == VPIN_EINVAL) {
     std::vector<uint8_t> xyzt(128 * nb);
     for (size_t i = 0; i < nb; i++) g[i].to_xyzt(xyzt.data() + 128 * i);
```

After: 74.75 million constraints/s (median of 6 runs). 4.4% higher.
